# adammoss/nnest

Measured on AMD Instinct MI355X. Metric: live-point evals/sec (flow-transform + loglike) + log-Z error, x_dim=50, higher is better.
Workload: dtype f32

## Files before the change

nnest_amd/csrc/flow_tile.h:

```cpp
#pragma once
#include <hip/hip_runtime.h>
#include <stdint.h>
#include "slice_walk.h"

namespace nnest {

typedef float f32x4 __attribute__((ext_vector_type(4)));
enum { FLOW_KIND_NVP = 0, FLOW_KIND_MAF = 1 };

struct FlowShape {
    int D, H, B, L;
    int NT;
    int NH;
    int net_floats;
    int image_floats;
    int net_params;
    int scale_mode;
    float base_beta, base_const;
    int kind, G;
    __host__ __device__ int nets_params() const { return B * 2 * net_params; }
    __host__ __device__ int num_params() const { return B * 2 * net_params + (scale_mode == 2 ? B : 0); }
    __host__ __device__ int image_total() const { return image_floats + (scale_mode == 2 ? B : 0); }
};

__host__ __device__ inline int frag_off_L1() { return 0; }
__host__ __device__ inline int frag_off_L2(int NT, int NH) { return NH * NT * 4 * 64; }
__host__ __device__ inline int frag_off_L3(int NT, int NH, int L) { return frag_off_L2(NT, NH) + L * NH * NH * 4 * 64; }
__host__ __device__ inline int frag_off_b1(int NT, int NH, int L) { return frag_off_L3(NT, NH, L) + NT * NH * 4 * 64; }
__host__ __device__ inline int frag_off_b2(int NT, int NH, int L) { return frag_off_b1(NT, NH, L) + 16 * NH; }
__host__ __device__ inline int frag_off_b3(int NT, int NH, int L) { return frag_off_b2(NT, NH, L) + L * 16 * NH; }
__host__ __device__ inline int frag_net_floats(int NT, int NH, int L) { return frag_off_b3(NT, NH, L) + 16 * NT; }

__device__ __forceinline__ float fast_tanh(float x) {
    float e = __builtin_amdgcn_exp2f(x * 2.8853900817779268f);
    return 1.0f - 2.0f * __builtin_amdgcn_rcpf(e + 1.0f);
}

template <int ACT>
__device__ __forceinline__ f32x4 activate(f32x4 v) {
    f32x4 o;
    if (ACT == 0) {
        o.x = fast_tanh(v.x); o.y = fast_tanh(v.y); o.z = fast_tanh(v.z); o.w = fast_tanh(v.w);
    } else {
        o.x = fmaxf(v.x, 0.f); o.y = fmaxf(v.y, 0.f); o.z = fmaxf(v.z, 0.f); o.w = fmaxf(v.w, 0.f);
    }
    return o;
}

__device__ __forceinline__ float base_pow(float a, float beta) { return __builtin_amdgcn_exp2f(beta * __builtin_amdgcn_logf(a)); }
__device__ __forceinline__ float base_E(float u, float beta) { return beta == 0.f ? 0.5f * u * u : base_pow(fabsf(u), beta); }
__device__ __forceinline__ float base_dE(float u, float beta) {
    if (beta == 0.f) return u;
    return u == 0.f ? 0.f : beta * base_pow(fabsf(u), beta) / u;
}
__device__ __forceinline__ float base_E4(f32x4 v, float beta) { return (base_E(v.x, beta) + base_E(v.y, beta)) + (base_E(v.z, beta) + base_E(v.w, beta)); }
__device__ __forceinline__ f32x4 base_dE4(f32x4 v, float beta) { return (f32x4){base_dE(v.x, beta), base_dE(v.y, beta), base_dE(v.z, beta), base_dE(v.w, beta)}; }

__device__ __forceinline__ f32x4 mfma4(float a, float b, f32x4 c) {
    return __builtin_amdgcn_mfma_f32_16x16x4f32(a, b, c, 0, 0, 0);
}

__host__ __device__ inline int frag_elem(int idx, int lane) { return (((idx >> 2) * 64 + lane) << 2) + (idx & 3); }
__device__ __forceinline__ f32x4 frag_quad(const float *__restrict__ region_lane , int q) {
    return *reinterpret_cast<const f32x4 *>(region_lane + q * 256);
}

template <int NT, int NH, int ACT>
__device__ __forceinline__ void mlp_tile(const float *__restrict__ wn, int L, int lane, const f32x4 (&in)[NT],
                                         f32x4 (&out)[NT]) {
    const int g4 = (lane >> 4) * 4;
    const float *fL1 = wn + frag_off_L1() + 4 * lane;
    const float *fL2 = wn + frag_off_L2(NT, NH) + 4 * lane;
    const float *fL3 = wn + frag_off_L3(NT, NH, L) + 4 * lane;
    const float *b1 = wn + frag_off_b1(NT, NH, L) + g4;
    const float *b2 = wn + frag_off_b2(NT, NH, L) + g4;
    const float *b3 = wn + frag_off_b3(NT, NH, L) + g4;
    f32x4 h[NH];
#pragma unroll
    for (int ht = 0; ht < NH; ++ht) {
        f32x4 acc = *reinterpret_cast<const f32x4 *>(b1 + 16 * ht);
#pragma unroll
        for (int tau = 0; tau < NT; ++tau) {
            const f32x4 f = frag_quad(fL1, ht * NT + tau);
            acc = mfma4(f.x, in[tau].x, acc);
            acc = mfma4(f.y, in[tau].y, acc);
            acc = mfma4(f.z, in[tau].z, acc);
            acc = mfma4(f.w, in[tau].w, acc);
        }
        h[ht] = activate<ACT>(acc);
    }
    for (int l = 0; l < L; ++l) {
        f32x4 h2[NH];
#pragma unroll
        for (int hto = 0; hto < NH; ++hto) {
            f32x4 acc = *reinterpret_cast<const f32x4 *>(b2 + (l * NH + hto) * 16);
#pragma unroll
            for (int hti = 0; hti < NH; ++hti) {
                const f32x4 f = frag_quad(fL2, (l * NH + hto) * NH + hti);
                acc = mfma4(f.x, h[hti].x, acc);
                acc = mfma4(f.y, h[hti].y, acc);
                acc = mfma4(f.z, h[hti].z, acc);
                acc = mfma4(f.w, h[hti].w, acc);
            }
            h2[hto] = activate<ACT>(acc);
        }
#pragma unroll
        for (int ht = 0; ht < NH; ++ht) h[ht] = h2[ht];
    }
#pragma unroll
    for (int tau = 0; tau < NT; ++tau) {
        f32x4 acc = *reinterpret_cast<const f32x4 *>(b3 + 16 * tau);
#pragma unroll
        for (int ht = 0; ht < NH; ++ht) {
            const f32x4 f = frag_quad(fL3, tau * NH + ht);
            acc = mfma4(f.x, h[ht].x, acc);
            acc = mfma4(f.y, h[ht].y, acc);
            acc = mfma4(f.z, h[ht].z, acc);
            acc = mfma4(f.w, h[ht].w, acc);
        }
        out[tau] = acc;
    }
}

template <int NT, int NH, bool INVERSE>
__device__ __forceinline__ float coupling_tile(const float *__restrict__ wblk, int net_floats, int L, int lane,
                                               const f32x4 (&cond)[NT], f32x4 (&trans)[NT]) {
    f32x4 ls[NT], t[NT];
    mlp_tile<NT, NH, 0>(wblk, L, lane, cond, ls);
    mlp_tile<NT, NH, 1>(wblk + net_floats, L, lane, cond, t);
    float ld = 0.f;
#pragma unroll
    for (int tau = 0; tau < NT; ++tau) {
        if (!INVERSE) {
            trans[tau].x = trans[tau].x * __expf(ls[tau].x) + t[tau].x;
            trans[tau].y = trans[tau].y * __expf(ls[tau].y) + t[tau].y;
            trans[tau].z = trans[tau].z * __expf(ls[tau].z) + t[tau].z;
            trans[tau].w = trans[tau].w * __expf(ls[tau].w) + t[tau].w;
            ld += (ls[tau].x + ls[tau].y) + (ls[tau].z + ls[tau].w);
        } else {
            trans[tau].x = (trans[tau].x - t[tau].x) * __expf(-ls[tau].x);
            trans[tau].y = (trans[tau].y - t[tau].y) * __expf(-ls[tau].y);
            trans[tau].z = (trans[tau].z - t[tau].z) * __expf(-ls[tau].z);
            trans[tau].w = (trans[tau].w - t[tau].w) * __expf(-ls[tau].w);
            ld -= (ls[tau].x + ls[tau].y) + (ls[tau].z + ls[tau].w);
        }
    }
    return ld;
}

struct ImageFrags {
    const float *p;
    __device__ __forceinline__ float operator()(int idx) const {
        return static_cast<const float *>(__builtin_assume_aligned(p, 16))[(idx >> 2) * 256 + (idx & 3)];
    }
};
template <int N> struct RegFrags {
    float v[N];
    __device__ __forceinline__ float operator()(int idx) const { return v[idx]; }
};
template <int NT, int NH, int L> struct FragCount {
    static constexpr int F1 = NH * NT * 4, F2 = L * NH * NH * 4, F3 = NT * NH * 4, N = F1 + F2 + F3;
};

template <int NT, int NH, int L, bool INVERSE, class FS, class FT>
__device__ __forceinline__ float coupling_core(const FS &fs, const FT &ft, const float *__restrict__ bias_s,
                                               const float *__restrict__ bias_t, int lane, const f32x4 (&cond)[NT],
                                               f32x4 (&trans)[NT]) {
    typedef FragCount<NT, NH, L> FC;
    const int g4 = (lane >> 4) * 4;
    const f32x4 zero4 = {0.f, 0.f, 0.f, 0.f};
    f32x4 hs[NH], ht[NH];
    {
        const float *bs = bias_s + g4, *bt = bias_t + g4;
#pragma unroll
        for (int o = 0; o < NH; ++o) {
// ... 585 lines not shown
```

nnest_amd/csrc/nnest_abi.hip:

```cpp
#include <math.h>
#include <stdio.h>
#include <string.h>
#include <stdarg.h>

#include "nnest_internal.h"
#include "mh_common.h"
#include "ensemble_common.h"
#include "mcmc_walk.h"
#include "importance_walk.h"

using namespace nnest;

struct nnest_nvp {
    FlowShape s;
    int device;
    int num_cu;
    int num_params;
    float *w;
    float *adam_m;
    float *adam_v;
    float *best_w;
    float *img;
    int *adam_step;
    float *train_ws;
    int *fwd_pos;
    int *bwd_pos;
    size_t train_ws_floats;
    float *img_bwd;
    int *gpos;
    unsigned int *ticket;
};

static thread_local char g_err[512] = "";

static int fail(int code, const char *fmt, ...) {
    va_list ap;
    va_start(ap, fmt);
    vsnprintf(g_err, sizeof(g_err), fmt, ap);
    va_end(ap);
    return code;
}

namespace nnest {
void set_last_error(const char *msg) { snprintf(g_err, sizeof(g_err), "%s", msg); }
}

#define HIP_TRY(expr)                                                                                   \
    do {                                                                                                \
        hipError_t e__ = (expr);                                                                        \
        if (e__ != hipSuccess) return fail(NNEST_E_HIP, "%s: %s", #expr, hipGetErrorString(e__));       \
    } while (0)

static hipError_t refresh_images(nnest_nvp *h, hipStream_t st) {
    if (h->s.kind == FLOW_KIND_MAF) return launch_maf_repack(h->w, h->img, h->img_bwd, h->s, st);
    if (h->s.scale_mode != NNEST_SCALE_AFFINE) {
        hipError_t e = launch_zero_scale_nets(h->w, h->s, st);
        if (e != hipSuccess) return e;
    }
    return launch_repack(h->w, h->img, h->s, st);
}

extern "C" {

int nnest_hip_version(void) { return NNEST_HIP_ABI_VERSION; }

const char *nnest_hip_last_error(void) { return g_err; }

int nnest_hip_device_info(int *num_cu, int *clock_khz, char *name, int name_len) {
    int dev = 0;
    HIP_TRY(hipGetDevice(&dev));
    hipDeviceProp_t p;
    HIP_TRY(hipGetDeviceProperties(&p, dev));
    if (num_cu) *num_cu = p.multiProcessorCount;
    if (clock_khz) *clock_khz = p.clockRate;
    if (name && name_len > 0) {
        snprintf(name, name_len, "%s (%s)", p.name, p.gcnArchName);
    }
    return NNEST_OK;
}

int nnest_nvp_create(int D, int H, int B, int L, nnest_nvp_t **out) {
    return nnest_nvp_create_scaled(D, H, B, L, NNEST_SCALE_AFFINE, out);
}

int nnest_nvp_create_scaled(int D, int H, int B, int L, int scale_mode, nnest_nvp_t **out) {
    if (!out) return fail(NNEST_E_ARG, "out is NULL");
    *out = nullptr;
    if (D < 1 || H < 1 || B < 1 || L < 0) return fail(NNEST_E_ARG, "bad shape D=%d H=%d B=%d L=%d", D, H, B, L);
    if (scale_mode < NNEST_SCALE_AFFINE || scale_mode > NNEST_SCALE_CONSTANT)
        return fail(NNEST_E_ARG, "scale_mode=%d (0 '', 1 'translate', 2 'constant')", scale_mode);
    if (scale_mode == NNEST_SCALE_CONSTANT && B > 8)
        return fail(NNEST_E_UNSUPPORTED, "scale='constant' with num_blocks=%d > 8", B);
    if (H % 16 != 0)
        return fail(NNEST_E_UNSUPPORTED, "hidden_dim=%d: the gfx950 kernels tile the hidden layer by 16 (MFMA 16x16x4)", H);
    FlowShape s;
    s.D = D; s.H = H; s.B = B; s.L = L;
    s.NT = ((D + 1) / 2 + 15) / 16;
    s.NH = H / 16;
    s.net_floats = frag_net_floats(s.NT, s.NH, L);
    s.image_floats = B * 2 * s.net_floats;
    s.net_params = H * D + H + L * (H * H + H) + D * H + D;
    s.scale_mode = scale_mode;
    s.kind = FLOW_KIND_NVP;
    s.G = 0;
    s.base_beta = 0.f;
    s.base_const = -0.91893853320467274f;
    if (!shape_supported(s))
        return fail(NNEST_E_UNSUPPORTED, "x_dim=%d hidden_dim=%d not instantiated (x_dim<=128 at H=16, <=64 at H=32, <=32 at H=64)", D, H);
    nnest_nvp *h = new nnest_nvp();
    memset(h, 0, sizeof(*h));
    h->s = s;
    h->num_params = s.num_params();
    if (hipGetDevice(&h->device) != hipSuccess) { delete h; return fail(NNEST_E_HIP, "hipGetDevice failed (no GPU?)"); }
    hipDeviceProp_t p;
    if (hipGetDeviceProperties(&p, h->device) != hipSuccess) { delete h; return fail(NNEST_E_HIP, "hipGetDeviceProperties failed"); }
    h->num_cu = p.multiProcessorCount;
    size_t nb = (size_t)h->num_params * sizeof(float);
    h->train_ws_floats = train_workspace_floats(s, 128);
    hipError_t e = hipSuccess;
    if (e == hipSuccess) e = hipMalloc((void **)&h->w, nb);
    if (e == hipSuccess) e = hipMalloc((void **)&h->adam_m, nb);
    if (e == hipSuccess) e = hipMalloc((void **)&h->adam_v, nb);
    if (e == hipSuccess) e = hipMalloc((void **)&h->best_w, nb);
    if (e == hipSuccess) e = hipMalloc((void **)&h->img, (size_t)s.image_total() * sizeof(float));
    if (e == hipSuccess) e = hipMalloc((void **)&h->adam_step, sizeof(int));
    if (e == hipSuccess) e = hipMalloc((void **)&h->train_ws, h->train_ws_floats * sizeof(float));
    if (e == hipSuccess) e = hipMalloc((void **)&h->fwd_pos, nb);
    if (e == hipSuccess) e = hipMalloc((void **)&h->bwd_pos, nb);
    if (e == hipSuccess) e = launch_build_pos(h->fwd_pos, h->bwd_pos, s, 0);
    if (e == hipSuccess) e = hipStreamSynchronize(0);
    if (e == hipSuccess) e = hipMemset(h->w, 0, nb);
    if (e == hipSuccess) e = hipMemset(h->adam_m, 0, nb);
    if (e == hipSuccess) e = hipMemset(h->adam_v, 0, nb);
    if (e == hipSuccess) e = hipMemset(h->adam_step, 0, sizeof(int));
    if (e == hipSuccess) e = hipMemset(h->img, 0, (size_t)s.image_total() * sizeof(float));
    if (e != hipSuccess) {
        nnest_nvp_destroy(h);
        return fail(NNEST_E_HIP, "device allocation failed: %s", hipGetErrorString(e));
    }
    *out = h;
    return NNEST_OK;
}

int nnest_maf_create(int D, int H, int B, int L, nnest_nvp_t **out) {
    if (!out) return fail(NNEST_E_ARG, "out is NULL");
    *out = nullptr;
    if (D < 2 || H < 1 || B < 1 || L < 0) return fail(NNEST_E_ARG, "bad shape D=%d H=%d B=%d L=%d (a MAF needs x_dim >= 2)", D, H, B, L);
    if (H != 16) return fail(NNEST_E_UNSUPPORTED, "maf: hidden_dim=%d, the kernels are instantiated for 16", H);
    FlowShape s;
    s.D = D; s.H = H; s.B = B; s.L = L;
    s.NT = ((D + 1) / 2 + 15) / 16;
    s.NH = H / 16;
    s.net_floats = frag_net_floats(2 * s.NT, s.NH, L);
    s.image_floats = B * 2 * s.net_floats + B * 16 * 2 * s.NT;
    s.net_params = H * D + H + L * (H * H + H) + D * H + D;
    s.scale_mode = NNEST_SCALE_AFFINE;
    s.kind = FLOW_KIND_MAF;
    s.G = maf_num_groups(D, H);
    s.base_beta = 0.f;
    s.base_const = -0.91893853320467274f;
    if (s.NT > 4 || !maf_shape_supported(s))
        return fail(NNEST_E_UNSUPPORTED, "maf: x_dim=%d num_blocks=%d num_layers=%d: the fragment image (%d floats) has to fit one CU's LDS and x_dim <= 128", D, B, L, s.image_floats);
    nnest_nvp *h = new nnest_nvp();
    memset(h, 0, sizeof(*h));
    h->s = s;
    h->num_params = s.num_params();
    if (hipGetDevice(&h->device) != hipSuccess) { delete h; return fail(NNEST_E_HIP, "hipGetDevice failed (no GPU?)"); }
    hipDeviceProp_t p;
    if (hipGetDeviceProperties(&p, h->device) != hipSuccess) { delete h; return fail(NNEST_E_HIP, "hipGetDeviceProperties failed"); }
    h->num_cu = p.multiProcessorCount;
    const size_t nb = (size_t)h->num_params * sizeof(float), ib = (size_t)s.image_floats * sizeof(float);
    h->train_ws_floats = maf_workspace_floats(s);
    hipError_t e = hipSuccess;
    if (e == hipSuccess) e = hipMalloc((void **)&h->w, nb);
    if (e == hipSuccess) e = hipMalloc((void **)&h->adam_m, nb);
    if (e == hipSuccess) e = hipMalloc((void **)&h->adam_v, nb);
    if (e == hipSuccess) e = hipMalloc((void **)&h->best_w, nb);
    if (e == hipSuccess) e = hipMalloc((void **)&h->img, ib);
    if (e == hipSuccess) e = hipMalloc((void **)&h->img_bwd, ib);
    if (e == hipSuccess) e = hipMalloc((void **)&h->adam_step, sizeof(int));
    if (e == hipSuccess) e = hipMalloc((void **)&h->train_ws, h->train_ws_floats * sizeof(float));
    if (e == hipSuccess) e = hipMalloc((void **)&h->gpos, nb);
    if (e == hipSuccess) e = launch_maf_build_gpos(h->gpos, s, 0);
    if (e == hipSuccess) e = hipMalloc((void **)&h->fwd_pos, nb);
    if (e == hipSuccess) e = hipMalloc((void **)&h->bwd_pos, nb);
    if (e == hipSuccess) e = launch_maf_build_pos(h->fwd_pos, h->bwd_pos, s, 0);
    if (e == hipSuccess) e = hipMalloc((void **)&h->ticket, sizeof(unsigned int));
    if (e == hipSuccess) e = hipMemset(h->ticket, 0, sizeof(unsigned int));
    if (e == hipSuccess) e = hipMemset(h->w, 0, nb);
    if (e == hipSuccess) e = hipMemset(h->adam_m, 0, nb);
    if (e == hipSuccess) e = hipMemset(h->adam_v, 0, nb);
    if (e == hipSuccess) e = hipMemset(h->adam_step, 0, sizeof(int));
    if (e == hipSuccess) e = refresh_images(h, 0);
    if (e == hipSuccess) e = hipStreamSynchronize(0);
    if (e != hipSuccess) {
        nnest_nvp_destroy(h);
        return fail(NNEST_E_HIP, "device allocation failed: %s", hipGetErrorString(e));
    }
    *out = h;
    return NNEST_OK;
}

int nnest_maf_num_groups(const nnest_nvp_t *h) { return (h && h->s.kind == FLOW_KIND_MAF) ? h->s.G : -1; }

int nnest_nvp_destroy(nnest_nvp_t *h) {
    if (!h) return NNEST_OK;
    (void)hipFree(h->w); (void)hipFree(h->adam_m); (void)hipFree(h->adam_v); (void)hipFree(h->best_w); (void)hipFree(h->img);
    (void)hipFree(h->adam_step); (void)hipFree(h->train_ws); (void)hipFree(h->fwd_pos); (void)hipFree(h->bwd_pos);
    (void)hipFree(h->img_bwd); (void)hipFree(h->gpos); (void)hipFree(h->ticket);
    delete h;
    return NNEST_OK;
}

int nnest_nvp_num_params(const nnest_nvp_t *h) { return h ? h->num_params : -1; }

int nnest_nvp_set_base(nnest_nvp_t *h, float beta) {
    if (!h) return fail(NNEST_E_ARG, "NULL handle");
    if (!(beta >= 0.f)) return fail(NNEST_E_ARG, "beta=%g: 0 selects N(0, I), beta > 0 GeneralisedNormal(0, 1, beta)", (double)beta);
    h->s.base_beta = beta;
    h->s.base_const = beta == 0.f ? -0.91893853320467274f : (float)(log((double)beta) - log(2.0) - lgamma(1.0 / (double)beta));
    return NNEST_OK;
}

int nnest_nvp_load_weights(nnest_nvp_t *h, const float *packed_host, void *stream) {
    if (!h || !packed_host) return fail(NNEST_E_ARG, "NULL argument");
    hipStream_t st = (hipStream_t)stream;
    HIP_TRY(hipMemcpyAsync(h->w, packed_host, (size_t)h->num_params * sizeof(float), hipMemcpyHostToDevice, st));
    HIP_TRY(refresh_images(h, st));
    HIP_TRY(hipStreamSynchronize(st));
    return NNEST_OK;
}

int nnest_nvp_store_weights(nnest_nvp_t *h, float *packed_host, void *stream) {
    if (!h || !packed_host) return fail(NNEST_E_ARG, "NULL argument");
    hipStream_t st = (hipStream_t)stream;
    HIP_TRY(hipMemcpyAsync(packed_host, h->w, (size_t)h->num_params * sizeof(float), hipMemcpyDeviceToHost, st));
    HIP_TRY(hipStreamSynchronize(st));
    return NNEST_OK;
}

int nnest_nvp_device_ptrs(nnest_nvp_t *h, float **w_dev, float **m_dev, float **v_dev) {
    if (!h) return fail(NNEST_E_ARG, "NULL handle");
    if (w_dev) *w_dev = h->w;
    if (m_dev) *m_dev = h->adam_m;
    if (v_dev) *v_dev = h->adam_v;
    return NNEST_OK;
}

int nnest_nvp_store_adam(nnest_nvp_t *h, float *exp_avg_host, float *exp_avg_sq_host, void *stream) {
    if (!h || !exp_avg_host || !exp_avg_sq_host) return fail(NNEST_E_ARG, "NULL argument");
    hipStream_t st = (hipStream_t)stream;
    size_t nb = (size_t)h->num_params * sizeof(float);
    HIP_TRY(hipMemcpyAsync(exp_avg_host, h->adam_m, nb, hipMemcpyDeviceToHost, st));
    HIP_TRY(hipMemcpyAsync(exp_avg_sq_host, h->adam_v, nb, hipMemcpyDeviceToHost, st));
    HIP_TRY(hipStreamSynchronize(st));
    return NNEST_OK;
}

int nnest_nvp_load_adam(nnest_nvp_t *h, const float *exp_avg_host, const float *exp_avg_sq_host, void *stream) {
    if (!h || !exp_avg_host || !exp_avg_sq_host) return fail(NNEST_E_ARG, "NULL argument");
    hipStream_t st = (hipStream_t)stream;
    size_t nb = (size_t)h->num_params * sizeof(float);
    HIP_TRY(hipMemcpyAsync(h->adam_m, exp_avg_host, nb, hipMemcpyHostToDevice, st));
    HIP_TRY(hipMemcpyAsync(h->adam_v, exp_avg_sq_host, nb, hipMemcpyHostToDevice, st));
    HIP_TRY(hipStreamSynchronize(st));
    return NNEST_OK;
}

int nnest_nvp_adam_state(nnest_nvp_t *h, int *step_count, int set_step, int reset_moments, void *stream) {
    if (!h) return fail(NNEST_E_ARG, "NULL handle");
    hipStream_t st = (hipStream_t)stream;
    if (reset_moments) {
        HIP_TRY(hipMemsetAsync(h->adam_m, 0, (size_t)h->num_params * sizeof(float), st));
        HIP_TRY(hipMemsetAsync(h->adam_v, 0, (size_t)h->num_params * sizeof(float), st));
    }
    if (set_step >= 0) HIP_TRY(hipMemcpyAsync(h->adam_step, &set_step, sizeof(int), hipMemcpyHostToDevice, st));
    HIP_TRY(hipStreamSynchronize(st));
    if (step_count) {
        HIP_TRY(hipMemcpyAsync(step_count, h->adam_step, sizeof(int), hipMemcpyDeviceToHost, st));
        HIP_TRY(hipStreamSynchronize(st));
    }
    return NNEST_OK;
}

static int check_rows(const nnest_nvp_t *h, const void *a, const void *b, int N) {
    if (!h) return fail(NNEST_E_ARG, "NULL handle");
    if (N < 0) return fail(NNEST_E_ARG, "N=%d < 0", N);
    if (N > 0 && (!a || !b)) return fail(NNEST_E_ARG, "NULL device buffer");
    return NNEST_OK;
}

int nnest_nvp_forward(nnest_nvp_t *h, const float *x_dev, float *z_dev, float *logdet_dev, int N, void *stream) {
    int rc = check_rows(h, x_dev, z_dev, N);
    if (rc) return rc;
    HIP_TRY(launch_pass(h->img, h->s, PASS_FORWARD, x_dev, z_dev, logdet_dev, nullptr, nullptr, N, LikeSpec(), h->num_cu,
                        (hipStream_t)stream));
    return NNEST_OK;
}

int nnest_nvp_inverse(nnest_nvp_t *h, const float *z_dev, float *x_dev, float *logdet_dev, int N, void *stream) {
    int rc = check_rows(h, z_dev, x_dev, N);
    if (rc) return rc;
    HIP_TRY(launch_pass(h->img, h->s, PASS_INVERSE, z_dev, x_dev, logdet_dev, nullptr, nullptr, N, LikeSpec(), h->num_cu,
                        (hipStream_t)stream));
    return NNEST_OK;
}

int nnest_nvp_log_probs(nnest_nvp_t *h, const float *x_dev, float *logp_dev, int N, void *stream) {
    int rc = check_rows(h, x_dev, logp_dev, N);
    if (rc) return rc;
    HIP_TRY(launch_pass(h->img, h->s, PASS_LOGPROB, x_dev, logp_dev, nullptr, nullptr, nullptr, N, LikeSpec(), h->num_cu,
                        (hipStream_t)stream));
    return NNEST_OK;
}

static int check_like(const nnest_like_t *like, int D, LikeSpec *out) {
    if (!like) return fail(NNEST_E_ARG, "like is NULL");
    if (like->id < 0 || like->id >= NNEST_LIKE_COUNT) return fail(NNEST_E_ARG, "unknown likelihood id %d", like->id);
    if (like->id == NNEST_LIKE_EGGBOX && D != 2) return fail(NNEST_E_ARG, "Eggbox is defined for x_dim = 2 (likelihoods.py:97-102)");
    if (like->id == NNEST_LIKE_GAUSSMIX && D < 2) return fail(NNEST_E_ARG, "GaussianMix needs x_dim >= 2");
    out->id = like->id;
    out->scale = like->scale;
    for (int i = 0; i < 6; ++i) out->p[i] = like->params[i];
    return NNEST_OK;
}

int nnest_nvp_inverse_loglike(nnest_nvp_t *h, const nnest_like_t *like, const float *z_dev, float *x_dev,
                              float *logdet_dev, double *logl_dev, int *inbox_dev, int N, void *stream) {
    int rc = check_rows(h, z_dev, logl_dev, N);
    if (rc) return rc;
    LikeSpec lk;
    if ((rc = check_like(like, h->s.D, &lk))) return rc;
    HIP_TRY(launch_pass(h->img, h->s, PASS_INVERSE_LOGLIKE, z_dev, x_dev, logdet_dev, logl_dev, inbox_dev, N, lk,
                        h->num_cu, (hipStream_t)stream));
    return NNEST_OK;
}

int nnest_loglike(const nnest_like_t *like, const float *x_unit_dev, double *logl_dev, int N, int D, void *stream) {
    if (N < 0 || D < 1) return fail(NNEST_E_ARG, "bad N=%d D=%d", N, D);
    LikeSpec lk;
    int rc = check_like(like, D, &lk);
    if (rc) return rc;
    if (D > 128) return fail(NNEST_E_UNSUPPORTED, "x_dim=%d > 128", D);
    if (N > 0 && (!x_unit_dev || !logl_dev)) return fail(NNEST_E_ARG, "NULL device buffer");
    int dev = 0, num_cu = 256;
    HIP_TRY(hipGetDevice(&dev));
    HIP_TRY(hipDeviceGetAttribute(&num_cu, hipDeviceAttributeMultiprocessorCount, dev));
    HIP_TRY(launch_loglike(lk, x_unit_dev, logl_dev, N, D, num_cu, (hipStream_t)stream));
    return NNEST_OK;
}

int nnest_mh_constrained_steps(nnest_nvp_t *h, const nnest_like_t *like, float *z_dev, float *x_dev,
                               double *logl_dev, double loglstar, float step_size, int steps, int C, int flags,
                               const float *noise_dz_dev, const float *noise_u_dev, uint64_t seed,
                               uint64_t walker_offset, float *hist_x_dev, double *hist_logl_dev, int *n_accept_dev,
                               int *n_call_dev, float *scale_out_dev, void *sync_dev, void *stream) {
    int rc = check_rows(h, z_dev, logl_dev, C);
    if (rc) return rc;
    LikeSpec lk;
    if ((rc = check_like(like, h->s.D, &lk))) return rc;
    if (steps < 0) return fail(NNEST_E_ARG, "steps=%d < 0", steps);
    if ((noise_dz_dev == nullptr) != (noise_u_dev == nullptr))
        return fail(NNEST_E_ARG, "noise_dz_dev and noise_u_dev must both be given or both be NULL");
    if ((flags & NNEST_MH_DYNAMIC_BATCH) && !sync_dev) return fail(NNEST_E_ARG, "NNEST_MH_DYNAMIC_BATCH needs sync_dev");
    hipError_t e = launch_mh(h->img, h->s, lk, z_dev, x_dev, logl_dev, loglstar, step_size, steps, C, flags,
                             noise_dz_dev, noise_u_dev, seed, walker_offset, hist_x_dev, hist_logl_dev, n_accept_dev, n_call_dev,
                             scale_out_dev, h->w, (unsigned long long *)sync_dev, h->num_cu, (hipStream_t)stream);
    if (e == hipErrorInvalidConfiguration)
        return fail(NNEST_E_UNSUPPORTED, "no kernel form for C=%d walkers with flags 0x%x (pinned form not applicable to this "
                                         "shape / population, or the batch-wide step rule on a grid that may not be resident)", C, flags);
    if (e != hipSuccess) return fail(NNEST_E_HIP, "launch_mh: %s", hipGetErrorString(e));
    return NNEST_OK;
}

int nnest_slice_steps(nnest_nvp_t *h, const nnest_like_t *like, float *z_dev, float *x_dev, double *logl_dev, double loglstar,
                      float width, int steps, int C, int max_stepout, int max_shrink, const float *noise_dz_dev, uint64_t seed,
                      uint64_t walker_offset, float *hist_x_dev, int *n_call_dev, int *n_move_dev, int *n_eval_dev, void *stream) {
    int rc = check_rows(h, z_dev, logl_dev, C);
    if (rc) return rc;
    LikeSpec lk;
    if ((rc = check_like(like, h->s.D, &lk))) return rc;
    if (!slice_params_ok(steps, max_stepout, max_shrink, width))
        return fail(NNEST_E_ARG, "steps=%d max_stepout=%d (0..2^24) max_shrink=%d (1..60) width=%g", steps, max_stepout, max_shrink, (double)width);
    if (!slice_form_eligible(h->s))
        return fail(NNEST_E_UNSUPPORTED, "slice proposal: hidden 16, 3 blocks, 1 layer, scale '' (the one-walker-per-wave layout), x_dim <= 128");
    const SliceArgs a = {z_dev, x_dev, logl_dev, loglstar, width, steps, C, max_stepout, max_shrink, lk, seed, walker_offset, noise_dz_dev,
                         hist_x_dev, nullptr, n_call_dev, n_move_dev, n_eval_dev};
    hipError_t e = launch_slice_solo(h->s, h->w, a, (hipStream_t)stream);
    if (e != hipSuccess) return fail(NNEST_E_HIP, "launch_slice_solo: %s", hipGetErrorString(e));
    return NNEST_OK;
}

int nnest_slice_fill_noise(float *dz_dev, int steps, int C, int D, uint64_t seed, uint64_t walker_offset, void *stream) {
    if (!dz_dev || steps < 0 || C < 0 || D < 1) return fail(NNEST_E_ARG, "bad argument");
    HIP_TRY(launch_slice_fill_noise(dz_dev, steps, C, D, seed, walker_offset, (hipStream_t)stream));
    return NNEST_OK;
}

int nnest_ensemble_work_words(int C, int steps) {
    if (C < 0 || steps < 0) return -1;
    const size_t w = ensemble_work_words(C, steps);
    return w > (size_t)0x7fffffff ? -1 : (int)w;
}

}
int nnest::mcmc_args(McmcArgs *a, const float *t_std, const float *t_mean, const float *lo, const float *hi, const float *z_in,
                     const double *lp_in, const double *logl_in, float *z_out, float *x_out, double *lp_out, double *logl_out,
                     float *hist_z, float *hist_x, double *hist_logl, int *n_accept, int C, int steps, float step_size, uint64_t step0,
                     uint64_t seed, uint64_t walker_offset) {
    if (C < 1 || steps < 0) return fail(NNEST_E_ARG, "mcmc: C=%d (>= 1 walkers) steps=%d (>= 0)", C, steps);
    if (!isfinite(step_size) || step_size < 0.f) return fail(NNEST_E_ARG, "mcmc: step_size=%g (finite, >= 0)", (double)step_size);
    if (!z_in || !x_out || !lp_out || !logl_out || (steps > 0 && !z_out)) return fail(NNEST_E_ARG, "NULL device buffer");
    if (!t_std != !t_mean) return fail(NNEST_E_ARG, "t_std_dev and t_mean_dev: both or neither");
    if (!lo != !hi) return fail(NNEST_E_ARG, "lo_dev and hi_dev: both or neither");
    if (!lp_in != !logl_in) return fail(NNEST_E_ARG, "lp_in_dev and logl_in_dev: both or neither");
    if ((!hist_z != !hist_x) || (!hist_z != !hist_logl)) return fail(NNEST_E_ARG, "hist_z_dev, hist_x_dev and hist_logl_dev: all or none");
    a->t_std = t_std; a->t_mean = t_mean; a->lo = lo; a->hi = hi;
    a->z_in = z_in; a->lp_in = lp_in; a->logl_in = logl_in;
    a->z_out = z_out; a->x_out = x_out; a->lp_out = lp_out; a->logl_out = logl_out;
    a->hist_z = hist_z; a->hist_x = hist_x; a->hist_logl = hist_logl; a->n_accept = n_accept;
    a->C = C; a->S = steps; a->step = step_size; a->step0 = (uint32_t)step0; a->seed = seed; a->walker_offset = walker_offset;
    return NNEST_OK;
}
int nnest::mcmc_beta_ok(double beta) {
    if (!isfinite(beta) || beta < 0.0) return fail(NNEST_E_ARG, "mcmc: beta=%g (the likelihood's power: finite, >= 0)", beta);
    return NNEST_OK;
}
int nnest::importance_args(ImpArgs *a, const float *t_std, const float *t_mean, const float *lo, const float *hi, float *z_out, float *x_out,
                           double *logl_out, double *logw_out, double *partials, double *sums, int M, uint64_t seed, uint64_t sample_offset) {
    if (M < 0 || M > (1 << 30)) return fail(NNEST_E_ARG, "importance: M=%d (0 .. 2^30 samples a launch)", M);
    if (!sums || (M > 0 && !partials)) return fail(NNEST_E_ARG, "importance: NULL sums_dev or partials_dev");
    if (!t_std != !t_mean) return fail(NNEST_E_ARG, "t_std_dev and t_mean_dev: both or neither");
    if (!lo != !hi) return fail(NNEST_E_ARG, "lo_dev and hi_dev: both or neither");
    if ((!z_out != !x_out) || (!z_out != !logl_out) || (!z_out != !logw_out))
        return fail(NNEST_E_ARG, "z_out_dev, x_out_dev, logl_out_dev and logw_out_dev: all or none");
    a->t_std = t_std; a->t_mean = t_mean; a->lo = lo; a->hi = hi;
    a->z_out = z_out; a->x_out = x_out; a->logl_out = logl_out; a->logw_out = logw_out;
    a->partials = partials; a->sums = sums; a->M = M; a->seed = seed; a->sample_offset = sample_offset;
    return NNEST_OK;
}
int nnest::ensemble_sizes(int C, int steps) {
    if (C < 2 || C > (1 << 16) || steps < 0) return fail(NNEST_E_ARG, "ensemble: C=%d (2..65536 walkers) steps=%d", C, steps);
    if (nnest_ensemble_work_words(C, steps) < 0) return fail(NNEST_E_ARG, "ensemble: C=%d x steps=%d: the work buffer exceeds 2^31 words", C, steps);
    return NNEST_OK;
}
static int ens_resolve_moves(const nnest_ens_moves_t *m, int C, int D, EnsMoves *out) {
    out->thr = ENS_THR_ALWAYS;
    out->g0 = out->sigma = 0.f;
    if (!m) return NNEST_OK;
    const double ws = (double)m->w_stretch, wd = (double)m->w_de;
    if (!(isfinite(ws) && isfinite(wd)) || ws < 0.0 || wd < 0.0 || ws + wd <= 0.0)
        return fail(NNEST_E_ARG, "ensemble moves: weights stretch=%g de=%g (finite, >= 0, not both 0)", ws, wd);
    if (!(isfinite(m->de_gamma0) && isfinite(m->de_sigma)) || m->de_gamma0 < 0.f || m->de_sigma < 0.f)
        return fail(NNEST_E_ARG, "ensemble moves: de_gamma0=%g de_sigma=%g (finite, >= 0; 0: emcee's default)", (double)m->de_gamma0, (double)m->de_sigma);
    if (wd > 0.0 && C < 4) return fail(NNEST_E_ARG, "ensemble moves: C=%d walkers: the DE move needs two partners in either set (C >= 4)", C);
    if (D < 1) return fail(NNEST_E_ARG, "ensemble moves: D=%d", D);
    out->thr = (uint32_t)floor(ws / (ws + wd) * 16777216.0);
    out->g0 = m->de_gamma0 != 0.f ? m->de_gamma0 : (float)(2.38 / sqrt(2.0 * (double)D));
    out->sigma = m->de_sigma != 0.f ? m->de_sigma : 1e-5f;
    return NNEST_OK;
}

extern "C" {

int nnest_ensemble_moves_threshold(const nnest_ens_moves_t *moves) {
    EnsMoves mv;
    if (ens_resolve_moves(moves, 4, 1, &mv)) return -1;
    return (int)mv.thr;
}

int nnest_ensemble_fill_moves(const int *work_dev, int *move_dev, int *b_dev, float *gamma_dev, int C, int D, int steps, uint64_t step0,
                              uint64_t seed, const nnest_ens_moves_t *moves, void *stream) {
    int rc = ensemble_sizes(C, steps);
    if (rc) return rc;
    if (!work_dev) return fail(NNEST_E_ARG, "NULL work_dev");
    if (C < 4) return fail(NNEST_E_ARG, "ensemble moves: C=%d walkers: the DE move needs two partners in either set (C >= 4)", C);
    EnsMoves mv;
    const nnest_ens_moves_t dflt = {1.f, 0.f, 0.f, 0.f};
    if ((rc = ens_resolve_moves(moves ? moves : &dflt, C, D, &mv))) return rc;
    HIP_TRY(launch_ensemble_fill_moves(work_dev, move_dev, b_dev, gamma_dev, C, steps, (uint32_t)step0, seed, mv, (hipStream_t)stream));
    return NNEST_OK;
}

int nnest_ensemble_fill_noise(int *work_dev, float *u_dev, int C, int steps, uint64_t step0, uint64_t seed, void *stream) {
    int rc = ensemble_sizes(C, steps);
    if (rc) return rc;
    if (!work_dev) return fail(NNEST_E_ARG, "NULL work_dev");
    HIP_TRY(launch_ensemble_split(work_dev, u_dev, C, steps, (uint32_t)step0, seed, (hipStream_t)stream));
    return NNEST_OK;
}

static int mcmc_steps_entry(nnest_nvp_t *h, const nnest_like_t *like, const float *t_std_dev, const float *t_mean_dev, const float *lo_dev,
                            const float *hi_dev, const float *z_in_dev, const double *lp_in_dev, const double *logl_in_dev, float *z_out_dev,
                            float *x_out_dev, double *lp_out_dev, double *logl_out_dev, float *hist_z_dev, float *hist_x_dev,
                            double *hist_logl_dev, int *n_accept_dev, int C, int steps, float step_size, uint64_t step0, uint64_t seed,
                            uint64_t walker_offset, const double *beta, void *stream) {
    if (!like) return fail(NNEST_E_ARG, "like is NULL");
    if (like->id < 0 || like->id >= NNEST_LIKE_COUNT) return fail(NNEST_E_ARG, "unknown likelihood id %d", like->id);
    int rc;
    if (beta && (rc = mcmc_beta_ok(*beta))) return rc;
    McmcTemperedArgs a;
    memset(&a, 0, sizeof(a));
    a.beta = beta ? *beta : 1.0;
    rc = mcmc_args(&a, t_std_dev, t_mean_dev, lo_dev, hi_dev, z_in_dev, lp_in_dev, logl_in_dev, z_out_dev, x_out_dev, lp_out_dev,
                   logl_out_dev, hist_z_dev, hist_x_dev, hist_logl_dev, n_accept_dev, C, steps, step_size, step0, seed, walker_offset);
    if (rc) return rc;
    if (!h) return fail(NNEST_E_ARG, "NULL handle");
    if ((rc = check_like(like, h->s.D, &a.like))) return rc;
    a.like.scale = 1.0f;
    if (!ensemble_form_eligible(h->s))
        return fail(NNEST_E_UNSUPPORTED, "mcmc: hidden 16, 3 blocks, 1 layer, scale '' (the one-walker-per-wave layout), x_dim <= 128");
    hipError_t e = beta ? launch_mcmc_tempered(h->s, h->w, a, (hipStream_t)stream) : launch_mcmc(h->s, h->w, a, (hipStream_t)stream);
    if (e == hipErrorInvalidConfiguration) return fail(NNEST_E_UNSUPPORTED, "mcmc: x_dim=%d not instantiated", h->s.D);
    if (e != hipSuccess) return fail(NNEST_E_HIP, "launch_mcmc: %s", hipGetErrorString(e));
    return NNEST_OK;
}

int nnest_mcmc_steps(nnest_nvp_t *h, const nnest_like_t *like, const float *t_std_dev, const float *t_mean_dev, const float *lo_dev,
                     const float *hi_dev, const float *z_in_dev, const double *lp_in_dev, const double *logl_in_dev, float *z_out_dev,
                     float *x_out_dev, double *lp_out_dev, double *logl_out_dev, float *hist_z_dev, float *hist_x_dev,
                     double *hist_logl_dev, int *n_accept_dev, int C, int steps, float step_size, uint64_t step0, uint64_t seed,
                     uint64_t walker_offset, void *stream) {
    return mcmc_steps_entry(h, like, t_std_dev, t_mean_dev, lo_dev, hi_dev, z_in_dev, lp_in_dev, logl_in_dev, z_out_dev, x_out_dev, lp_out_dev,
                            logl_out_dev, hist_z_dev, hist_x_dev, hist_logl_dev, n_accept_dev, C, steps, step_size, step0, seed,
                            walker_offset, nullptr, stream);
}

int nnest_mcmc_tempered_steps(nnest_nvp_t *h, const nnest_like_t *like, const float *t_std_dev, const float *t_mean_dev, const float *lo_dev,
                              const float *hi_dev, const float *z_in_dev, const double *lp_in_dev, const double *logl_in_dev,
                              float *z_out_dev, float *x_out_dev, double *lp_out_dev, double *logl_out_dev, float *hist_z_dev,
                              float *hist_x_dev, double *hist_logl_dev, int *n_accept_dev, int C, int steps, float step_size,
                              uint64_t step0, uint64_t seed, uint64_t walker_offset, double beta, void *stream) {
    return mcmc_steps_entry(h, like, t_std_dev, t_mean_dev, lo_dev, hi_dev, z_in_dev, lp_in_dev, logl_in_dev, z_out_dev, x_out_dev, lp_out_dev,
                            logl_out_dev, hist_z_dev, hist_x_dev, hist_logl_dev, n_accept_dev, C, steps, step_size, step0, seed,
                            walker_offset, &beta, stream);
}

int nnest_mcmc_fill_noise(float *dz_dev, float *u_dev, int steps, int C, int D, uint64_t step0, uint64_t seed, uint64_t walker_offset,
                          void *stream) {
    if (steps < 0 || C < 0 || D < 1) return fail(NNEST_E_ARG, "mcmc_fill_noise: steps=%d C=%d D=%d", steps, C, D);
    HIP_TRY(launch_mcmc_fill_noise(dz_dev, u_dev, steps, C, D, (uint32_t)step0, seed, walker_offset, (hipStream_t)stream));
// ... 307 lines not shown
```

nnest_amd/csrc/nnest_internal.h:

```cpp
#pragma once
#include <hip/hip_runtime.h>
#include <stdint.h>
#include "flow_tile.h"
#include "maf_tile.h"
#include "spline_tile.h"
#include "../../include/nnest_hip.h"

namespace nnest {

enum { PASS_FORWARD = 0, PASS_INVERSE = 1, PASS_LOGPROB = 2, PASS_INVERSE_LOGLIKE = 3 };

void set_last_error(const char *msg);
bool shape_supported(const FlowShape &s);
hipError_t launch_repack(const float *packed, float *img, const FlowShape &s, hipStream_t st);
hipError_t launch_zero_scale_nets(float *packed, const FlowShape &s, hipStream_t st);
hipError_t launch_pass(const float *img, const FlowShape &s, int mode, const float *in, float *out, float *logdet,
                       double *logl, int *inbox, int N, const LikeSpec &like, int num_cu, hipStream_t st);
hipError_t launch_mh(const float *img, const FlowShape &s, const LikeSpec &like, float *z, float *x, double *logl,
                     double loglstar, float step_size, int steps, int C, int flags, const float *noise_dz,
                     const float *noise_u, uint64_t seed, uint64_t walker_offset, float *hist_x, double *hist_logl,
                     int *n_accept, int *n_call, float *scale_out, const float *packed, unsigned long long *sync, int num_cu,
                     hipStream_t st);
struct MhArgs;
struct SliceArgs;
bool quad_form_eligible(const MhArgs &a, int num_cu);
hipError_t launch_mh_quad(const MhArgs &a, int num_cu, hipStream_t st);
bool solo_form_eligible(const MhArgs &a, int num_cu);
hipError_t launch_mh_solo(const MhArgs &a, int num_cu, hipStream_t st);
int mh_form_for(const FlowShape &s, int C, int flags, int num_cu);
bool maf_shape_supported(const FlowShape &s);
hipError_t launch_maf_repack(const float *packed, float *imgf, float *imgb, const FlowShape &s, hipStream_t st);
hipError_t launch_loglike(const LikeSpec &like, const float *x, double *logl, int N, int D, int num_cu, hipStream_t st);
hipError_t launch_fill_noise(float *dz, float *u, int steps, int C, int D, uint64_t seed, uint64_t walker_offset,
                             hipStream_t st);
int mh_num_groups(int C);

struct SplArgs {
    const float *img;
    SplineShape sp;
};
hipError_t launch_spline_mh_pair(const MhArgs &a, const SplArgs &q, bool dbg, hipStream_t st);
hipError_t launch_spline_mh_team(const MhArgs &a, const SplArgs &q, bool dbg, hipStream_t st);
int spline_mh_form(const SplineShape &sp, int C, int flags, int num_cu);
int spline_slice_form(const SplineShape &sp, int C, int flags, int num_cu);
hipError_t launch_spline_slice(const SplArgs &q, const SliceArgs &a, int flags, int num_cu, hipStream_t st);
bool spline_shape_supported(const SplineShape &s);
hipError_t launch_spline_pass(const float *img, const SplineShape &sp, int mode, const float *in, float *out, float *logdet,
                              double *logl, int *inbox, int N, const LikeSpec &like, int num_cu, hipStream_t st);
hipError_t launch_spline_mh(const float *img, const SplineShape &sp, const LikeSpec &like, float *z, float *x, double *logl,
                            double loglstar, float step_size, int steps, int C, int flags, const float *noise_dz,
                            const float *noise_u, uint64_t seed, uint64_t walker_offset, float *hist_x, double *hist_logl,
                            int *n_accept, int *n_call, float *scale_out, unsigned long long *sync, int num_cu, hipStream_t st);

struct TrainArgs;
hipError_t launch_loss_grad(const float *packed, const FlowShape &s, const float *x, int M, float *grad, float *loss,
                            float *workspace, float *img_fwd, const int *fwd_pos, const int *bwd_pos, hipStream_t st);
hipError_t launch_vjp(const float *packed, const FlowShape &s, const float *x, const float *gz, float gld, int M, float *grad, float *gx,
                      float *workspace, float *img_fwd, const int *fwd_pos, const int *bwd_pos, hipStream_t st);
hipError_t launch_adam_packed(float *w, const float *grad, float *m, float *v, int n, int step, float lr, float wd, hipStream_t st);
hipError_t launch_adam_packed_dev(float *w, const float *grad, float *m, float *v, int n, int *step_dev, float lr, float wd, hipStream_t st);
size_t train_workspace_floats(const FlowShape &s, int batch);
hipError_t launch_train(float *packed, float *adam_m, float *adam_v, float *best_w, float *img, int *adam_step_dev,
                        const FlowShape &s, const float *xtrain, int n_train, const float *xvalid, int n_valid,
                        const int *perm, const float *noise, uint64_t seed, float jitter, int batch, int max_epochs,
                        int patience, float lr, float wd, int epoch_offset, int flags, float *losses, nnest_train_result_t *result,
                        float *workspace, const int *fwd_pos, const int *bwd_pos,
                        hipStream_t st);
int train_form_for(const FlowShape &s, int batch, int flags, int *detail);
hipError_t launch_build_pos(int *fwd_pos, int *bwd_pos, const FlowShape &s, hipStream_t st);
size_t maf_workspace_floats(const FlowShape &s);
hipError_t launch_maf_build_gpos(int *gpos, const FlowShape &s, hipStream_t st);
hipError_t launch_maf_build_pos(int *fwd_pos, int *bwd_pos, const FlowShape &s, hipStream_t st);
hipError_t launch_maf_train_minibatch(const FlowShape &s, float *imgf, float *imgb, const int *gpos, const int *fwd_pos, const int *bwd_pos,
                                      const float *x, int M, float *w, float *m, float *v, int *step_dev, float lr, float wd,
                                      float *loss_acc, unsigned int *ticket, float *workspace, hipStream_t st);
hipError_t launch_maf_loss_grad(const FlowShape &s, const float *imgf, const float *imgb, const int *gpos, const float *x, int M,
                                float *grad, float *loss, float *workspace, hipStream_t st);
hipError_t launch_training_jitter(const double *samples, int N, int D, double *out, hipStream_t st);
bool slice_form_eligible(const FlowShape &s);
hipError_t launch_slice_solo(const FlowShape &s, const float *packed, const SliceArgs &a, hipStream_t st);
hipError_t launch_slice_fill_noise(float *dz, int steps, int C, int D, uint64_t seed, uint64_t walker_offset, hipStream_t st);
size_t ensemble_work_words(int C, int S);
bool ensemble_form_eligible(const FlowShape &s);
struct EnsMoves;
hipError_t ensemble_max_walkers(const FlowShape &s, int like_id, const EnsMoves &mv, int num_cu, int *out);
hipError_t ensemble_x_max_walkers(int D, int like_id, const EnsMoves &mv, int num_cu, int *out);
hipError_t launch_ensemble_fill_moves(const int *work, int *move, int *jb, float *gamma, int C, int S, uint32_t step0, uint64_t seed,
                                      const EnsMoves &mv, hipStream_t st);
int launch_ensemble_x(int D, const LikeSpec &like, const float *t_std, const float *t_mean, const float *lo, const float *hi,
                      const float *x_in, const double *lp_in, float *x_out, float *tx_out, double *lp_out, float *hist_x, double *hist_lp,
                      int *n_accept, int *work, int C, int S, uint32_t step0, uint64_t seed, int constrained, double loglstar,
                      const EnsMoves &mv, int num_cu, hipStream_t st, char *msg, size_t msg_len);
hipError_t launch_ensemble_split(int *work, float *u, int C, int S, uint32_t step0, uint64_t seed, hipStream_t st);
int launch_ensemble(const FlowShape &s, const float *packed, const LikeSpec &like, const float *t_std, const float *t_mean, const float *lo,
                    const float *hi, const float *z_in, const double *lp_in, float *z_out, float *x_out, double *lp_out, float *hist_z,
                    float *hist_x, double *hist_lp, int *n_accept, int *work, int C, int S, uint32_t step0, uint64_t seed, int constrained,
                    double loglstar, const EnsMoves &mv, int num_cu, hipStream_t st, char *msg, size_t msg_len);
int ensemble_sizes(int C, int steps);
struct EnsArgs;
hipError_t spline_ensemble_max_walkers(const SplArgs &q, int num_cu, int *out);
int launch_spline_ensemble(const SplArgs &q, const EnsArgs &a, int num_cu, hipStream_t st, char *msg, size_t msg_len);
hipError_t launch_ensemble_propose(const int *work, int C, int S, int D, int i, int half, uint32_t step0, uint64_t seed, const EnsMoves &mv,
                                   const float *z_cur, float *q, int rows, hipStream_t st);
hipError_t launch_ensemble_accept(const int *work, int C, int S, int D, int i, int half, uint32_t step0, uint64_t seed, const EnsMoves &mv,
                                  const float *q, const float *x, const float *ld, const double *logl, const double *lprior, const float *t_std,
                                  const float *t_mean, const float *lo, const float *hi, float *z_cur, float *x_cur, double *lp_cur,
                                  float *hist_z, float *hist_x, double *hist_lp, int *n_accept, int *acc_rows, int constrained,
                                  double loglstar, int rows, hipStream_t st);

}
```

nnest_amd/csrc/nnest_kernels.hip:

```cpp
#include <map>
#include <mutex>
#include <utility>
#include <string.h>

#include "flow_tile.h"
#include "maf_tile.h"
#include "mh_common.h"
#include "nnest_internal.h"
#include "spline_train_tile.h"

namespace nnest {

__global__ void repack_fragments_kernel(const float *__restrict__ packed, float *__restrict__ img, FlowShape s) {
    const int NT = s.NT, NH = s.NH, L = s.L, D = s.D, H = s.H;
    const int total = s.image_floats;
    for (int idx = blockIdx.x * blockDim.x + threadIdx.x; idx < total; idx += gridDim.x * blockDim.x) {
        int bn = idx / s.net_floats, o = idx - bn * s.net_floats;
        int b = bn >> 1, net = bn & 1;
        const float *p = packed + ((size_t)b * 2 + net) * s.net_params;
        const int pc = (b + 1) & 1, pt = b & 1;
        const int pW0 = 0, pb0 = H * D, phid = H * D + H, pWo = H * D + H + L * (H * H + H), pbo = pWo + D * H;
        float v = 0.f;
        if (o < frag_off_L2(NT, NH)) {
            int r = o & 3, lane = (o >> 2) & 63, q = (o >> 8) << 2, tau = (q >> 2) % NT, ht = (q >> 2) / NT;
// ... 499 lines not shown
        if (b.p) (void)hipFree(b.p);
        b.p = nullptr; b.cap = 0;
        const size_t want = floats + floats / 2 + 4096;
        if (hipMalloc((void **)&b.p, want * sizeof(float)) != hipSuccess) { b.p = nullptr; return nullptr; }
        b.cap = want;
    }
    return b.p;
}
hipError_t launch_mh_zero_other_sync(const MhArgs &a, hipStream_t st) {
    if (!a.sync || !(a.flags & (NNEST_MH_SYNC_ZERO_NEXT | NNEST_MH_SYNC_ZERO_PREV))) return hipSuccess;
    const size_t W = mh_sync_words(a.steps) + 1;
    unsigned long long *other = (a.flags & NNEST_MH_SYNC_ZERO_NEXT) ? a.sync + W : a.sync - W;
    return hipMemsetAsync(other, 0, W * sizeof(unsigned long long), st);
}
hipError_t launch_mh_all_moved(const MhArgs &a, hipStream_t st) {
    if (!a.x0 || !a.x || !a.n_accept) return hipSuccess;
    const int grid = min((a.C + 3) / 4, 2048);
    hipLaunchKernelGGL(mh_all_moved_kernel, dim3(grid), dim3(256), 0, st, a.x0, a.x, a.n_accept, a.C, a.s.D);
    return hipGetLastError();
}

template <int NT, int NH, int LT>
static hipError_t launch_mh_tiles_t(const MhArgs &a, int form, int num_cu, hipStream_t st);
template <int NT, int NH, int LT>
static hipError_t launch_mh_t(const MhArgs &a_in, int num_cu, hipStream_t st) {
    const bool batch = (a_in.flags & NNEST_MH_DYNAMIC_BATCH) != 0;
    if (batch && !a_in.sync) return hipErrorInvalidValue;
    const int form = pick_mh_form<NT, NH, LT>(a_in, num_cu);
    if (form < 0) return hipErrorInvalidConfiguration;
    if (form == MH_FORM_SOLO) return launch_mh_solo(a_in, num_cu, st);
    if (form == MH_FORM_QUAD || form == MH_FORM_QUAD1) {
        hipError_t e = launch_mh_quad(a_in, num_cu, st);
        return e != hipSuccess ? e : launch_mh_zero_other_sync(a_in, st);
    }
    MhArgs a = a_in;
    if (a.x && a.n_accept && !(a.x0 = mh_first_x_buffer((size_t)a.C * a.s.D, st))) return hipErrorOutOfMemory;
    hipError_t e = launch_mh_tiles_t<NT, NH, LT>(a, form, num_cu, st);
    if (e != hipSuccess) return e;
    e = launch_mh_zero_other_sync(a, st);
    if (e != hipSuccess) return e;
    return launch_mh_all_moved(a, st);
}
template <int NT, int NH, int LT>
static hipError_t launch_mh_tiles_t(const MhArgs &a, int form, int num_cu, hipStream_t st) {
    const int ntiles = (a.C + 15) / 16;
    const bool batch = (a.flags & NNEST_MH_DYNAMIC_BATCH) != 0;
    if constexpr (LT == 1 && NH == 1) {
        if (form == MH_FORM_TEAM) {
            const size_t timg = NT <= 2 ? 0 : (size_t)a.s.image_floats * 4;
            const int grid = ntiles + ((batch && mh_flag_lag(a.flags) >= 2) ? 1 : 0);
            if (a.hist_x || a.hist_logl) {
                hipError_t e = allow_lds(mh_kernel_team<NT, 1, 3, true>, timg + 48 * 1024);
                if (e != hipSuccess) return e;
                hipLaunchKernelGGL((mh_kernel_team<NT, 1, 3, true>), dim3(grid), dim3(192), timg, st, a);
            } else {
                hipError_t e = allow_lds(mh_kernel_team<NT, 1, 3, false>, timg + 48 * 1024);
                if (e != hipSuccess) return e;
                hipLaunchKernelGGL((mh_kernel_team<NT, 1, 3, false>), dim3(grid), dim3(192), timg, st, a);
            }
            return hipGetLastError();
        }
    }
    if constexpr (LT == 1 && NH == 1 && NT <= 2) {
        if (form == MH_FORM_REG) {
            if (a.noise_dz || a.hist_x || a.hist_logl)
                hipLaunchKernelGGL((mh_kernel_reg<NT, 1, 1, 3, true>), dim3(ntiles), dim3(64), 0, st, a);
            else
                hipLaunchKernelGGL((mh_kernel_reg<NT, 1, 1, 3, false>), dim3(ntiles), dim3(64), 0, st, a);
            return hipGetLastError();
        }
    }
    const size_t img_bytes = (size_t)a.s.image_floats * 4;
    const bool dbg = a.noise_dz || a.hist_x || a.hist_logl;
    const ImageGeom geo = image_geometry<NT>(ntiles, num_cu, img_bytes, batch, dbg);
    const int block = geo.block, grid = geo.grid;
    if constexpr (NT >= 3) {
        if (geo.occ == 1) {
            hipError_t e = allow_lds(mh_kernel<NT, NH, LT, true, false, 1>, img_bytes);
            if (e != hipSuccess) return e;
            hipLaunchKernelGGL((mh_kernel<NT, NH, LT, true, false, 1>), dim3(grid), dim3(block), img_bytes, st, a);
            return hipGetLastError();
        }
    }
    if (geo.occ == 2) {
        hipError_t e = allow_lds(mh_kernel<NT, NH, LT, true, false, 2>, img_bytes);
        if (e != hipSuccess) return e;
        hipLaunchKernelGGL((mh_kernel<NT, NH, LT, true, false, 2>), dim3(grid), dim3(block), img_bytes, st, a);
        return hipGetLastError();
    }
    if (img_bytes <= (size_t)LDS_IMAGE_LIMIT) {
        if (dbg) {
            hipError_t e = allow_lds(mh_kernel<NT, NH, LT, true, true>, img_bytes);
            if (e != hipSuccess) return e;
            hipLaunchKernelGGL((mh_kernel<NT, NH, LT, true, true>), dim3(grid), dim3(block), img_bytes, st, a);
        } else {
            hipError_t e = allow_lds(mh_kernel<NT, NH, LT, true, false>, img_bytes);
            if (e != hipSuccess) return e;
            hipLaunchKernelGGL((mh_kernel<NT, NH, LT, true, false>), dim3(grid), dim3(block), img_bytes, st, a);
        }
    } else {
        if (dbg) hipLaunchKernelGGL((mh_kernel<NT, NH, LT, false, true>), dim3(grid), dim3(block), 0, st, a);
        else hipLaunchKernelGGL((mh_kernel<NT, NH, LT, false, false>), dim3(grid), dim3(block), 0, st, a);
    }
    return hipGetLastError();
}

template <int NT, int NH, int LT>
static int mh_form_t(const MhArgs &a, int num_cu) { return pick_mh_form<NT, NH, LT>(a, num_cu); }

#define DISPATCH_NTNH(FN, s, LT, ...)                                \
    do {                                                             \
        if ((s).NH == 1) {                                           \
            switch ((s).NT) {                                        \
                case 1: return FN<1, 1, LT>(__VA_ARGS__);            \
                case 2: return FN<2, 1, LT>(__VA_ARGS__);            \
                case 3: return FN<3, 1, LT>(__VA_ARGS__);            \
                case 4: return FN<4, 1, LT>(__VA_ARGS__);            \
            }                                                        \
        } else if ((s).NH == 2) {                                    \
            switch ((s).NT) {                                        \
                case 1: return FN<1, 2, LT>(__VA_ARGS__);            \
                case 2: return FN<2, 2, LT>(__VA_ARGS__);            \
            }                                                        \
        } else if ((s).NH == 4) {                                    \
            switch ((s).NT) {                                        \
                case 1: return FN<1, 4, LT>(__VA_ARGS__);            \
            }                                                        \
        }                                                            \
        return hipErrorInvalidConfiguration;                         \
    } while (0)

#define DISPATCH_SHAPE(FN, s, ...)                                   \
    do {                                                             \
        if ((s).L == 1) DISPATCH_NTNH(FN, s, 1, __VA_ARGS__);        \
        DISPATCH_NTNH(FN, s, -1, __VA_ARGS__);                       \
    } while (0)

bool shape_supported(const FlowShape &s) {
    if (s.NH == 1) return s.NT >= 1 && s.NT <= 4;
    if (s.NH == 2) return s.NT >= 1 && s.NT <= 2;
    if (s.NH == 4) return s.NT == 1;
    return false;
}

hipError_t launch_zero_scale_nets(float *packed, const FlowShape &s, hipStream_t st) {
    hipLaunchKernelGGL(zero_scale_nets_kernel, dim3(64), dim3(256), 0, st, packed, s);
    return hipGetLastError();
}

hipError_t launch_repack(const float *packed, float *img, const FlowShape &s, hipStream_t st) {
    int block = 256, grid = (s.image_floats + block - 1) / block;
    if (grid > 1024) grid = 1024;
    hipLaunchKernelGGL(repack_fragments_kernel, dim3(grid), dim3(block), 0, st, packed, img, s);
    return hipGetLastError();
}

static hipError_t launch_maf_pass(const PassArgs &a, int num_cu, hipStream_t st);
static hipError_t launch_maf_mh(const MhArgs &a, int num_cu, hipStream_t st);

hipError_t launch_pass(const float *img, const FlowShape &s, int mode, const float *in, float *out, float *logdet,
                       double *logl, int *inbox, int N, const LikeSpec &like, int num_cu, hipStream_t st) {
    if (N <= 0) return hipSuccess;
    PassArgs a;
    a.img = img; a.s = s; a.mode = mode; a.in = in; a.out = out; a.logdet = logdet; a.logl = logl; a.inbox = inbox;
    a.N = N; a.like = like;
    if (s.kind == FLOW_KIND_MAF) return launch_maf_pass(a, num_cu, st);
    DISPATCH_SHAPE(launch_pass_t, s, a, num_cu, st);
}

hipError_t launch_mh(const float *img, const FlowShape &s, const LikeSpec &like, float *z, float *x, double *logl,
                     double loglstar, float step_size, int steps, int C, int flags, const float *noise_dz,
                     const float *noise_u, uint64_t seed, uint64_t walker_offset, float *hist_x, double *hist_logl,
                     int *n_accept, int *n_call, float *scale_out, const float *packed, unsigned long long *sync, int num_cu,
                     hipStream_t st) {
    if (C <= 0) return hipSuccess;
    MhArgs a;
    a.packed = packed;
    a.sync = sync;
    a.sync_err = sync ? reinterpret_cast<int *>(sync + mh_sync_words(steps)) : nullptr;
    a.img = img; a.s = s; a.z = z; a.x = x; a.logl = logl; a.loglstar = loglstar; a.step_size = step_size;
    a.steps = steps; a.C = C; a.flags = flags; a.like = like;
    a.noise_dz = noise_dz; a.noise_u = noise_u; a.seed = seed; a.walker_offset = walker_offset;
    a.hist_x = hist_x; a.hist_logl = hist_logl; a.n_accept = n_accept; a.n_call = n_call; a.scale_out = scale_out;
    a.x0 = nullptr;
    if (s.kind == FLOW_KIND_MAF) {
        if (a.x && a.n_accept && !(a.x0 = mh_first_x_buffer((size_t)C * s.D, st))) return hipErrorOutOfMemory;
        hipError_t e = launch_maf_mh(a, num_cu, st);
        if (e == hipSuccess) e = launch_mh_zero_other_sync(a, st);
        return e != hipSuccess ? e : launch_mh_all_moved(a, st);
    }
    DISPATCH_SHAPE(launch_mh_t, s, a, num_cu, st);
}

hipError_t launch_loglike(const LikeSpec &like, const float *x, double *logl, int N, int D, int num_cu, hipStream_t st) {
    if (N <= 0) return hipSuccess;
    const int NT = ((D + 1) / 2 + 15) / 16;
    const int ntiles = (N + 15) / 16;
    int block = 256, grid = (ntiles + 3) / 4;
    if (grid > 8 * num_cu) grid = 8 * num_cu;
    switch (NT) {
        case 1: hipLaunchKernelGGL((loglike_kernel<1>), dim3(grid), dim3(block), 0, st, x, logl, N, D, like); break;
        case 2: hipLaunchKernelGGL((loglike_kernel<2>), dim3(grid), dim3(block), 0, st, x, logl, N, D, like); break;
        case 3: hipLaunchKernelGGL((loglike_kernel<3>), dim3(grid), dim3(block), 0, st, x, logl, N, D, like); break;
        case 4: hipLaunchKernelGGL((loglike_kernel<4>), dim3(grid), dim3(block), 0, st, x, logl, N, D, like); break;
        default: return hipErrorInvalidConfiguration;
    }
    return hipGetLastError();
}

hipError_t launch_fill_noise(float *dz, float *u, int steps, int C, int D, uint64_t seed, uint64_t walker_offset,
                             hipStream_t st) {
    if (steps <= 0 || C <= 0) return hipSuccess;
    int block = 256;
    int grid = (C * 4 + block - 1) / block;
    hipLaunchKernelGGL(fill_noise_kernel, dim3(grid), dim3(block), 0, st, dz, u, steps, C, D, seed, walker_offset);
    return hipGetLastError();
}

int mh_num_groups(int C) { return (C + 15) / 16; }

int mh_form_for(const FlowShape &s, int C, int flags, int num_cu) {
    MhArgs a = MhArgs();
    a.s = s; a.C = C; a.flags = flags;
    if (s.kind == FLOW_KIND_MAF) {
        const int form = mh_flag_form(flags);
        if (form != MH_FORM_AUTO && form != MH_FORM_IMAGE) return -1;
        if ((flags & NNEST_MH_DYNAMIC_BATCH) && mh_flag_lag(flags) > 0 && mh_flag_warm(flags) > 0) return -1;
        int block, grid;
        pick_geometry((C + 15) / 16, num_cu, 4, &block, &grid);
        return ((flags & NNEST_MH_DYNAMIC_BATCH) && grid > num_cu) ? -1 : MH_FORM_IMAGE;
    }
    DISPATCH_SHAPE(mh_form_t, s, a, num_cu);
}

#include "maf_kernels.h"
#include "spline_kernels.h"

}
```

nnest_amd/csrc/nnest_solo.hip:

```cpp
#include <string.h>
#include "mh_common.h"
#include "nnest_internal.h"
#include "solo_loglike.h"
#include "solo_tile.h"

namespace nnest {

static constexpr int SOLO_ETAB = 1024;

template <int U, int WPG> constexpr bool solo_lds_weights() { return U >= 3 || WPG > 4; }
template <int U, int WPG> constexpr int solo_reg_blocks() { return !solo_lds_weights<U, WPG>() ? 3 : (WPG == 4 ? 1 : (U <= 2 && WPG == 8 ? 1 : 0)); }

enum { MH_SOLO_LAG_INTERNAL = 8 };
template <int U, bool DBG, int LK, int WPG>
__global__ void __launch_bounds__(64 * (WPG + 2)) mh_kernel_solo(MhArgs a) {
    extern __shared__ __attribute__((aligned(16))) float wlds[];
    __shared__ __attribute__((aligned(16))) float nbuf[2][WPG][16][2 * U];
    __shared__ float ubuf[2][WPG];
    __shared__ __attribute__((aligned(16))) uint32_t rawbuf[4 * WPG * 8 * U];
    __shared__ int acc_lds[2][WPG];
    __shared__ float fsbuf[2];
    __shared__ float fs_exact;
    __shared__ float fs_cand[2];
    __shared__ int vote_sel;
    __shared__ double etab[SOLO_ETAB];

    const int lane = threadIdx.x & 63, wave = __builtin_amdgcn_readfirstlane(threadIdx.x >> 6);
    const int tile = blockIdx.x;
    const int D = a.s.D, S = a.steps, C = a.C;
    const bool recorded = DBG && a.noise_dz;
    const bool dynamic = (a.flags & NNEST_MH_DYNAMIC_BATCH) != 0;
    const bool use_tab = S + 2 <= SOLO_ETAB;
    const bool exact_all = dynamic && mh_flag_lag(a.flags) == 0;
    const bool direct_votes = (a.flags & NNEST_MH_WINDOW_VOTES_ONLY) == 0;
    const int lag = exact_all ? MH_SOLO_LAG_INTERNAL : mh_flag_lag(a.flags);
    const int warm = dynamic ? min(exact_all ? S : mh_flag_warm(a.flags), S - 1) : 0;
    constexpr bool LDSW = solo_lds_weights<U, WPG>();
    constexpr int RB = solo_reg_blocks<U, WPG>();
    const int ntiles = (C + WPG - 1) / WPG;
    if (tile >= ntiles) {
        if (dynamic && wave == 0) mh_sync_publisher(a.sync, S, exact_all ? S : max(S - lag, warm), ntiles, C, lane, a.sync_err);
        else if (dynamic && (a.flags & (NNEST_MH_SYNC_ZERO_NEXT | NNEST_MH_SYNC_ZERO_PREV))) {
            const size_t W = (size_t)mh_sync_words(S) + 1;
            unsigned long long *other = (a.flags & NNEST_MH_SYNC_ZERO_NEXT) ? a.sync + W : a.sync - W;
            const int nthr = (int)blockDim.x - 64;
            for (size_t i = threadIdx.x - 64; i < W; i += nthr) other[i] = 0ull;
        }
        return;
    }
    {
        if constexpr (!LDSW) {
            const int n = a.s.nets_params();
            for (int i = threadIdx.x; i < n; i += blockDim.x) wlds[i] = a.packed[i];
        } else {
            if (wave < 3) {
                SoloNet<U> nb;
                solo_gather<U>(nb, a.packed + (size_t)(wave * 2 + (lane >= 32 ? 1 : 0)) * a.s.net_params, D, (wave + 1) & 1, wave & 1, lane);
                solo4_store<U>(wlds, wave, nb, lane);
            }
        }
        if (dynamic && use_tab)
            for (int k = threadIdx.x; k < S + 2; k += blockDim.x) etab[k] = exp(1.0 / (double)(1 + k));
    }
    __syncthreads();

    if (wave == WPG) {
        const int g = lane & 3, j = min(lane >> 2, WPG - 1);
        const bool gen = lane < 4 * WPG;
        Xoshiro128 rn = xoshiro_seed(a.seed, a.walker_offset + (uint64_t)(tile * WPG + j), (uint32_t)g, NOISE_STREAM_DZ);
        Xoshiro128 ru = xoshiro_seed(a.seed, a.walker_offset + (uint64_t)(tile * WPG + j), 0xffffffffu, NOISE_STREAM_U);
        constexpr int NQ = 8 * WPG * U;
        unsigned long long n0 = 0, n1 = 0, n2 = 0, n_gen = 0, n_all = 0;
        (void)n0; (void)n1; (void)n2; (void)n_gen; (void)n_all;
        auto draw = [&](int k) {
            if (k > S) return;
            STAMP(n0);
            if (!recorded) {
                if (gen) {
#pragma unroll
                    for (int t = 0; t < 2 * U; ++t) {
                        u32x4 r;
                        r.x = xoshiro_next(rn); r.y = xoshiro_next(rn); r.z = xoshiro_next(rn); r.w = xoshiro_next(rn);
                        *reinterpret_cast<u32x4 *>(&rawbuf[lane * 8 * U + 4 * t]) = r;
                    }
                    const float u = xoshiro_uniform(ru);
                    if (g == 0) ubuf[k & 1][j] = u;
                }
                float *nb = &nbuf[k & 1][0][0][0];
#pragma unroll
                for (int i = 0; i < (NQ + 63) / 64; ++i) {
                    const int q = lane + 64 * i;
                    if (NQ % 64 == 0 || q < NQ) {
                        const u32x4 r = *reinterpret_cast<const u32x4 *>(&rawbuf[4 * q]);
                        const int sl = q / (2 * U), qq = q % (2 * U);
                        const int d0 = 32 * (qq >> 1) + 8 * (sl & 3) + 4 * (qq & 1);
                        float o0, o1, o2, o3;
                        box_muller(r.x, r.y, o0, o1);
                        box_muller(r.z, r.w, o2, o3);
                        const f32x4 o = {d0 < D ? o0 : 0.f, d0 + 1 < D ? o1 : 0.f, d0 + 2 < D ? o2 : 0.f, d0 + 3 < D ? o3 : 0.f};
                        *reinterpret_cast<f32x4 *>(nb + (sl >> 2) * 32 * U + d0) = o;
                    }
                }
            }
            if (!dynamic && lane == 0) fsbuf[k & 1] = a.step_size;
            STAMP(n1);
#ifdef NNEST_STAMP
            n_gen += n1 - n0;
#endif
        };
        STAMP(n2);
        draw(0);
        solo_barrier();
        if (S >= 1) {
            draw(1);
            solo_barrier();
            draw(2);
            for (int k = 1; k <= warm; ++k) {
                solo_barrier();
                solo_barrier();
                draw(k + 2);
                solo_barrier();
            }
            for (int k = warm > 0 ? warm + 2 : 2; k <= S; ++k) {
                solo_barrier();
                draw(k + 1);
            }
        }
#ifdef NNEST_STAMP
        { unsigned long long n3 = 0; STAMP(n3); n_all = n3 - n2; }
#endif
#ifdef NNEST_STAMP
        if (a.scale_out && lane == 0 && tile == 0) { a.scale_out[4] = (float)n_gen; a.scale_out[5] = (float)n_all; }
#endif
#ifndef NNEST_STAMP
        if (!dynamic && a.scale_out && lane == 0) {
            const int g0 = (tile * WPG + 15) >> 4;
            if (16 * g0 < (tile + 1) * WPG && 16 * g0 < C) a.scale_out[g0] = a.step_size;
        }
#endif
        return;
    }
    if (wave == WPG + 1) {
        if (!dynamic) return;
        double scale = (double)a.step_size;
        int accept = 0, reject = 0;
        const int last = S - lag;
        const unsigned long long *wbase = a.sync + 2 * mh_sync_counter_words(S) + (size_t)(tile & (MH_SYNC_SHARDS - 1)) * MH_SYNC_STRIDE;
#define SOLO_RELAY_ITERATION(k_, q_)                                                                                        \
        {                                                                                                                   \
            const int k = (k_), want = k - lag;                                                                             \
              \
              \
              \
              \
              \
            asm volatile("s_waitcnt vmcnt(2)" : "+v"(q_) : : "memory");                                                     \
            if (want > warm) {                                                                                              \
                const bool up = mh_window_vote(a.sync, S, want, tile, q_, a.sync_err);                                      \
                if (up) accept += 1; else reject += 1;                                                                      \
                if (accept > reject) scale *= use_tab ? etab[accept] : exp(1.0 / (1 + accept));                             \
                if (accept < reject) scale /= use_tab ? etab[reject] : exp(1.0 / (1 + reject));                             \
            }                                                                                                               \
                   \
             \
            if (lane == 0) {                                                                                                \
                const int *ac = acc_lds[k & 1];                                                                             \
                const bool mine = k - 2 > warm;                                 \
                int acs = 0;                                                                                                \
                _Pragma("unroll") for (int w_ = 0; w_ < WPG; ++w_) acs += ac[w_];                                           \
                mh_sync_post(a.sync, mine ? k - 2 : 0, tile, mine ? acs : 0);                                               \
            }                                                                                                               \
            const int ask = min(max(want + 2, 1), max(last, 1));         \
            const unsigned long long *wp = wbase + (size_t)((ask - 1) >> 5) * MH_SYNC_SHARDS * MH_SYNC_STRIDE;              \
            asm volatile("global_load_dwordx2 %0, %1, off sc1" : "=v"(q_) : "v"(wp) : "memory");                            \
              \
            if (lane == 0) fsbuf[k & 1] = (float)scale;                                                                     \
            solo_barrier();                                                                           \
        }
        unsigned long long qa = 0, qb = 0;
        int k0 = 0;
        if (warm > 0) {
            auto E = [&](int n) { return use_tab ? etab[n] : exp(1.0 / (1 + n)); };
            auto next_scale = [&](int acc, int rej, double sc) {
                if (acc > rej) sc *= E(acc);
                if (acc < rej) sc /= E(rej);
                return sc;
            };
            if (lane == 0) {
                fsbuf[0] = (float)scale;
                fs_cand[0] = (float)next_scale(accept + 1, reject, scale);
                fs_cand[1] = (float)next_scale(accept, reject + 1, scale);
            }
            solo_barrier();
            if (lane == 0) fsbuf[1] = (float)scale;
            solo_barrier();
            for (int k = 1; k <= warm; ++k) {
                solo_barrier();
                if (lane == 0) {
                    const int *ac = acc_lds[k & 1];
                    int acs = 0;
#pragma unroll
                    for (int w_ = 0; w_ < WPG; ++w_) acs += ac[w_];
                    mh_sync_post(a.sync, k, tile, acs);
                    fsbuf[(k + 1) & 1] = (float)scale;
                }
                solo_barrier();
                const bool up = direct_votes ? 2 * mh_sync_total(a.sync, k, ntiles, 0ull, a.sync_err) > C
                                             : mh_window_vote(a.sync, S, k, tile, 0ull, a.sync_err);
                if (up) accept += 1; else reject += 1;
                scale = next_scale(accept, reject, scale);
                if (lane == 0) {
                    vote_sel = up ? 0 : 1;
                    fs_exact = (float)scale;
                    fs_cand[0] = (float)next_scale(accept + 1, reject, scale);
                    fs_cand[1] = (float)next_scale(accept, reject + 1, scale);
                }
                solo_barrier();
            }
            k0 = warm + 2;
        }
        for (int k2 = k0; k2 <= S; k2 += 2) {
            SOLO_RELAY_ITERATION(k2, qa)
            if (k2 + 1 <= S) SOLO_RELAY_ITERATION(k2 + 1, qb)
        }
#undef SOLO_RELAY_ITERATION
        asm volatile("s_waitcnt vmcnt(0)" : "+v"(qa), "+v"(qb) : : "memory");
        if (exact_all) {
            solo_barrier();
            if (lane == 0) {
                const int *ac = acc_lds[S & 1];
                int acs = 0;
#pragma unroll
                for (int w_ = 0; w_ < WPG; ++w_) acs += ac[w_];
                mh_sync_post(a.sync, S, tile, acs);
            }
            const bool up = direct_votes ? 2 * mh_sync_total(a.sync, S, ntiles, 0ull, a.sync_err) > C : mh_window_vote(a.sync, S, S, tile, 0ull, a.sync_err);
            if (up) accept += 1; else reject += 1;
            if (accept > reject) scale *= use_tab ? etab[accept] : exp(1.0 / (1 + accept));
            if (accept < reject) scale /= use_tab ? etab[reject] : exp(1.0 / (1 + reject));
        }
#ifndef NNEST_STAMP
        if (a.scale_out && lane == 0) {
            const int g0 = (tile * WPG + 15) >> 4;
            if (16 * g0 < (tile + 1) * WPG && 16 * g0 < C) a.scale_out[g0] = (float)scale;
        }
#endif
        return;
    }

    const int j = wave;
    const int pos = lane & 15;
    const bool translate_half = lane >= 32;
    const bool writer_lane = lane < 16;
    const int row = tile * WPG + j;
    const bool ok = row < C;
    const LikeSpec like = a.like;
    const double loglstar = a.loglstar;
    const bool free_mode = (a.flags & NNEST_MH_UNCONSTRAINED) != 0;

    SoloNet<U> net[RB > 0 ? RB : 1];
    if constexpr (LDSW) {
        if constexpr (RB == 1)
            solo_gather<U>(net[0], a.packed + (size_t)(1 * 2 + (translate_half ? 1 : 0)) * a.s.net_params, D, (1 + 1) & 1, 1 & 1, lane);
    } else {
#pragma unroll
        for (int b = 0; b < 3; ++b)
            solo_gather<U>(net[b], wlds + (size_t)(b * 2 + (translate_half ? 1 : 0)) * a.s.net_params, D, (b + 1) & 1, b & 1, lane);
    }
    const unsigned sel = translate_half ? 0xffffffffu : 0u;
    const bool h1 = (lane & 16) != 0;
    auto inverse = [&](float (&xs)[2][U]) {
        if constexpr (LDSW) {
            float ld = solo_coupling_inverse4<U>(Solo4Lds{wlds + (size_t)2 * SOLO4_NF * 64, lane}, sel, h1, xs[1], xs[0]);
            if constexpr (RB == 1) ld += solo_coupling_inverse4<U>(Solo4Reg<U>{net[0]}, sel, h1, xs[0], xs[1]);
            else ld += solo_coupling_inverse4<U>(Solo4Lds{wlds + (size_t)1 * SOLO4_NF * 64, lane}, sel, h1, xs[0], xs[1]);
            ld += solo_coupling_inverse4<U>(Solo4Lds{wlds, lane}, sel, h1, xs[1], xs[0]);
            return ld;
        } else {
            float ld;
            solo_coupling_inverse<U, true>(net[2], sel, h1, xs[1], xs[0], ld);
            solo_coupling_inverse<U, false>(net[1], sel, h1, xs[0], xs[1], ld);
            solo_coupling_inverse<U, false>(net[0], sel, h1, xs[1], xs[0], ld);
            return ld;
        }
    };

    float z[2][U], x[2][U];
#pragma unroll
    for (int u = 0; u < U; ++u)
#pragma unroll
        for (int c = 0; c < 2; ++c) {
            const int d = 2 * U * pos + 2 * u + c;
            z[c][u] = (ok && d < D) ? a.z[(size_t)row * D + d] : 0.f;
            x[c][u] = z[c][u];
        }
    float ld = solo_logdet_total(inverse(x));
    double logl = ok ? a.logl[row] : 0.0;
    int n_acc = 0, n_call = 0;

    auto store_row = [&](float *base, size_t r, const float (&v)[2][U]) {
#pragma unroll
        for (int u = 0; u < U; ++u)
#pragma unroll
            for (int c = 0; c < 2; ++c) {
                const int d = 2 * U * pos + 2 * u + c;
                if (d < D) base[r * D + d] = v[c][u];
            }
    };
    if (writer_lane && ok && a.x) store_row(a.x, (size_t)row, x);
    if (DBG && writer_lane && ok) {
        if (a.hist_x) store_row(a.hist_x, (size_t)row * (S + 1), x);
        if (a.hist_logl && pos == 0) a.hist_logl[(size_t)row * (S + 1)] = logl;
    }

    float nz[2 * U], u_next = 0.f, fs_next = a.step_size;
    int kbuf = 0;
    auto fetch_noise = [&]() {
        solo_barrier();
        if (!recorded) {
#pragma unroll
            for (int k = 0; k < 2 * U; ++k) nz[k] = nbuf[kbuf & 1][j][pos][k];
            u_next = ubuf[kbuf & 1][j];
        }
        fs_next = fsbuf[kbuf & 1];
        ++kbuf;
    };
    fetch_noise();

    unsigned long long st0 = 0, st1 = 0, st2 = 0, st3 = 0, a_prop = 0, a_inv = 0, a_post = 0, a_tot = 0;
    (void)st0; (void)st1; (void)st2; (void)st3; (void)a_prop; (void)a_inv; (void)a_post; (void)a_tot;
    struct Prop { float zp[2][U], xp[2][U]; float ldp; double lp; bool pre, acc; };
    auto propose = [&](int it, float fs, float (&zp)[2][U], float &u) {
        if (recorded) {
#pragma unroll
            for (int uu = 0; uu < U; ++uu)
#pragma unroll
                for (int c = 0; c < 2; ++c) {
                    const int d = 2 * U * pos + 2 * uu + c;
                    const float dz = (ok && d < D) ? a.noise_dz[((size_t)(it - 1) * C + row) * D + d] : 0.f;
                    zp[c][uu] = __builtin_fmaf(dz, fs, z[c][uu]);
                }
            u = ok ? a.noise_u[(size_t)(it - 1) * C + row] : 1.f;
        } else {
#pragma unroll
            for (int uu = 0; uu < U; ++uu) {
                zp[0][uu] = __builtin_fmaf(nz[2 * uu], fs, z[0][uu]);
                zp[1][uu] = __builtin_fmaf(nz[2 * uu + 1], fs, z[1][uu]);
            }
            u = u_next;
        }
    };
    auto finish = [&](Prop &r, float u) {
#pragma unroll
        for (int c = 0; c < 2; ++c)
#pragma unroll
            for (int uu = 0; uu < U; ++uu) r.xp[c][uu] = r.zp[c][uu];
        STAMP(st1);
        constexpr bool RIDE = LK == NNEST_LIKE_ROSENBROCK;
        r.ldp = RIDE ? inverse(r.xp) : solo_logdet_total(inverse(r.xp));
        STAMP(st2);
        if constexpr (RIDE) r.lp = solo_loglike<U, LK>(like, D, lane, r.xp, &r.ldp);
        int okl = 1;
#pragma unroll
        for (int c = 0; c < 2; ++c)
#pragma unroll
            for (int uu = 0; uu < U; ++uu) okl &= !(r.xp[c][uu] < -1.f || r.xp[c][uu] > 1.f);
        const bool inb = __ballot(okl != 0) == ~0ull;
        float log_ratio = inb ? (r.ldp - ld) : -INFINITY;
        float ratio = fminf(__expf(log_ratio), 1.0f);
        if (log_ratio != log_ratio) ratio = log_ratio;
        r.pre = ok && (u < ratio);
        if constexpr (!RIDE) r.lp = solo_loglike<U, LK>(like, D, lane, r.xp);
        r.acc = r.pre && (r.lp > loglstar);
        if (free_mode) {
            const double lr = inb ? (double)(r.ldp - ld) + (r.lp - logl) : -INFINITY;
            const double rt = fmin(exp(lr), 1.0);
            r.acc = ok && ((double)u < rt);
        }
    };
    auto apply = [&](int it, const Prop &r) {
        n_call += (free_mode ? ok : r.pre) ? 1 : 0;
        n_acc += r.acc ? 1 : 0;
#pragma unroll
        for (int c = 0; c < 2; ++c)
#pragma unroll
            for (int uu = 0; uu < U; ++uu) {
                z[c][uu] = r.acc ? r.zp[c][uu] : z[c][uu];
                x[c][uu] = r.acc ? r.xp[c][uu] : x[c][uu];
            }
        ld = r.acc ? r.ldp : ld;
        logl = r.acc ? r.lp : logl;
        if (dynamic && lane == 0) acc_lds[it & 1][j] = r.acc ? 1 : 0;
        if (DBG && writer_lane && ok) {
            if (a.hist_x) store_row(a.hist_x, (size_t)row * (S + 1) + it, x);
            if (a.hist_logl && pos == 0) a.hist_logl[(size_t)row * (S + 1) + it] = logl;
        }
    };
    Prop cur;
    bool have = false;
    for (int it = 1; it <= S; ++it) {
        STAMP(st0);
        if (!have) {
            float u;
            propose(it, fs_next, cur.zp, u);
            fetch_noise();
            finish(cur, u);
        }
        apply(it, cur);
        have = false;
        if (it <= warm) {
            solo_barrier();
            const float f0 = fs_cand[0], f1 = fs_cand[1];
            Prop c1;
            float u;
            propose(it + 1, f0, cur.zp, u);
            propose(it + 1, f1, c1.zp, u);
            fetch_noise();
            finish(cur, u);
            finish(c1, u);
            solo_barrier();
            if (vote_sel != 0) cur = c1;
            have = true;
            fs_next = fs_exact;
        }
        STAMP(st3);
#ifdef NNEST_STAMP
        a_prop += st1 - st0; a_inv += st2 - st1; a_post += st3 - st2; a_tot += st3 - st0;
#endif
    }
    if (exact_all) solo_barrier();
#ifdef NNEST_STAMP
    if (a.scale_out && lane == 0 && tile == 0) {
        float *o = a.scale_out;
        if (j == 0) { o[0] = (float)a_tot; o[1] = (float)a_prop; o[2] = (float)a_inv; o[3] = (float)a_post; }
        if (j < 4) { o[8 + 2 * j] = (float)a_inv; o[9 + 2 * j] = (float)a_post; }
    }
#endif
    bool all_moved = n_acc > 0;
    if (a.x) {
        bool mine = true;
        if (writer_lane) {
#pragma unroll
            for (int u = 0; u < U; ++u)
#pragma unroll
                for (int c = 0; c < 2; ++c) {
                    const int d = 2 * U * pos + 2 * u + c;
                    const float x0 = (ok && d < D) ? a.x[(size_t)row * D + d] : 0.f;
                    mine = mine && (d >= D || x[c][u] != x0);
                }
        }
        all_moved = (__ballot(mine) & 0xffffull) == 0xffffull;
    }
    if (writer_lane && ok) {
        store_row(a.z, (size_t)row, z);
        if (a.x) store_row(a.x, (size_t)row, x);
        if (pos == 0) {
            a.logl[row] = logl;
            if (a.n_accept) a.n_accept[row] = n_acc | (all_moved ? NNEST_MH_ALL_MOVED : 0);
            if (a.n_call) a.n_call[row] = n_call;
        }
    }
}

template <int U>
static __device__ __forceinline__ void slice_normals(uint64_t seed, uint64_t walker, uint32_t step, int pos, int D, float (&e)[2][U]) {
    const int d0 = 2 * U * pos;
    f32x4 q[(2 * U + 3) / 4 + 1];
    const int q0 = d0 >> 2;
#pragma unroll
    for (int k = 0; k < (2 * U + 3) / 4 + 1; ++k) q[k] = noise_normal4(seed, walker, step, (uint32_t)(q0 + k), NOISE_STREAM_DZ);
#pragma unroll
    for (int u = 0; u < U; ++u)
#pragma unroll
        for (int c = 0; c < 2; ++c) {
            const int d = d0 + 2 * u + c, k = (d >> 2) - q0, r = d & 3;
            float v = 0.f;
#pragma unroll
            for (int kk = 0; kk < (2 * U + 3) / 4 + 1; ++kk)
                if (kk == k) v = r == 0 ? q[kk].x : (r == 1 ? q[kk].y : (r == 2 ? q[kk].z : q[kk].w));
            e[c][u] = d < D ? v : 0.f;
        }
}

template <int U, int LK>
__global__ void __launch_bounds__(256) slice_kernel_solo(SliceArgs a, FlowShape s, const float *packed) {
    extern __shared__ __attribute__((aligned(16))) float wlds[];
    const int lane = threadIdx.x & 63, wave = __builtin_amdgcn_readfirstlane(threadIdx.x >> 6);
    const int D = s.D, S = a.steps, C = a.C;
    constexpr bool LDSW = solo_lds_weights<U, 4>();
    {
        if constexpr (!LDSW) {
            const int n = s.nets_params();
            for (int i = threadIdx.x; i < n; i += blockDim.x) wlds[i] = packed[i];
        } else if (wave < 3) {
            SoloNet<U> nb;
            solo_gather<U>(nb, packed + (size_t)(wave * 2 + (lane >= 32 ? 1 : 0)) * s.net_params, D, (wave + 1) & 1, wave & 1, lane);
            solo4_store<U>(wlds, wave, nb, lane);
        }
    }
    __syncthreads();
    const int pos = lane & 15;
    const bool translate_half = lane >= 32, writer_lane = lane < 16;
    const int row = blockIdx.x * 4 + wave;
    const bool ok = row < C;
    if (!ok) return;
    const LikeSpec like = a.like;
    const double loglstar = a.loglstar;
    SoloNet<U> net[LDSW ? 1 : 3];
    if constexpr (!LDSW) {
#pragma unroll
        for (int b = 0; b < 3; ++b)
            solo_gather<U>(net[b], wlds + (size_t)(b * 2 + (translate_half ? 1 : 0)) * s.net_params, D, (b + 1) & 1, b & 1, lane);
    }
    const unsigned sel = translate_half ? 0xffffffffu : 0u;
    const bool h1 = (lane & 16) != 0;
    auto inverse = [&](float (&xs)[2][U]) {
        if constexpr (LDSW) {
            float ld = solo_coupling_inverse4<U>(Solo4Lds{wlds + (size_t)2 * SOLO4_NF * 64, lane}, sel, h1, xs[1], xs[0]);
            ld += solo_coupling_inverse4<U>(Solo4Lds{wlds + (size_t)1 * SOLO4_NF * 64, lane}, sel, h1, xs[0], xs[1]);
            ld += solo_coupling_inverse4<U>(Solo4Lds{wlds, lane}, sel, h1, xs[1], xs[0]);
            return ld;
        } else {
            float ld;
            solo_coupling_inverse<U, true>(net[2], sel, h1, xs[1], xs[0], ld);
            solo_coupling_inverse<U, false>(net[1], sel, h1, xs[0], xs[1], ld);
            solo_coupling_inverse<U, false>(net[0], sel, h1, xs[1], xs[0], ld);
            return ld;
        }
    };
    auto store_row = [&](float *base, size_t r, const float (&v)[2][U]) {
#pragma unroll
        for (int u = 0; u < U; ++u)
#pragma unroll
            for (int c = 0; c < 2; ++c) {
                const int d = 2 * U * pos + 2 * u + c;
                if (d < D) base[r * D + d] = v[c][u];
            }
    };
    float z[2][U], x[2][U];
#pragma unroll
    for (int u = 0; u < U; ++u)
#pragma unroll
        for (int c = 0; c < 2; ++c) {
            const int d = 2 * U * pos + 2 * u + c;
            z[c][u] = d < D ? a.z[(size_t)row * D + d] : 0.f;
            x[c][u] = z[c][u];
        }
    float ld = solo_logdet_total(inverse(x));
    double logl = a.logl[row];
    if (writer_lane && a.x) store_row(a.x, (size_t)row, x);
    if (writer_lane && a.hist_x) store_row(a.hist_x, (size_t)row * (S + 1), x);
    const uint64_t walker = a.walker_offset + (uint64_t)row;
    int n_call = 0, n_move = 0, n_eval = 0;
    float zc[2][U], xc[2][U], ldc = 0.f;
    double lc = 0.0;
    for (int it = 1; it <= S; ++it) {
        float e[2][U];
        if (a.noise_dz) {
#pragma unroll
            for (int u = 0; u < U; ++u)
#pragma unroll
                for (int c = 0; c < 2; ++c) {
                    const int d = 2 * U * pos + 2 * u + c;
                    e[c][u] = d < D ? a.noise_dz[((size_t)(it - 1) * C + row) * D + d] : 0.f;
                }
        } else {
            slice_normals<U>(a.seed, walker, (uint32_t)it, pos, D, e);
        }
        const float u0 = noise_uniform(a.seed, walker, 64u * (uint32_t)it + 0u), u1 = noise_uniform(a.seed, walker, 64u * (uint32_t)it + 1u);
        const float logy = ld + __logf(u1);
        auto inside = [&](float t) -> bool {
            const float tw = t * a.width;
#pragma unroll
            for (int u = 0; u < U; ++u)
#pragma unroll
                for (int c = 0; c < 2; ++c) { zc[c][u] = __builtin_fmaf(e[c][u], tw, z[c][u]); xc[c][u] = zc[c][u]; }
            ldc = solo_logdet_total(inverse(xc));
            int okl = 1;
#pragma unroll
            for (int c = 0; c < 2; ++c)
#pragma unroll
                for (int u = 0; u < U; ++u) okl &= !(xc[c][u] < -1.f || xc[c][u] > 1.f);
            const bool inb = __ballot(okl != 0) == ~0ull;
            const bool pre = inb && (ldc > logy);
            lc = solo_loglike<U, LK>(like, D, lane, xc);
            n_eval += 1;
            n_call += pre ? 1 : 0;
            return pre && (lc > loglstar);
        };
        float tl = -u0, tr = 1.0f - u0;
        if (a.max_out > 0) {
            const int B = 2 * a.max_out;
            int n = 0;
            while (n <= B && inside(tl)) { tl -= 1.0f; n += 1; }
            while (n <= B && inside(tr)) { tr += 1.0f; n += 1; }
            if (n > B) {
                tl = -u0;
                tr = 1.0f - u0;
                const int nl = slice_stepout_left(a.seed, walker, (uint32_t)it, a.max_out);
                for (int j = 0; j < nl; ++j) { if (!inside(tl)) break; tl -= 1.0f; }
                for (int j = 0; j < B - nl; ++j) { if (!inside(tr)) break; tr += 1.0f; }
            }
        }
        bool moved = false;
        for (int k = 0; k < a.max_shrink; ++k) {
            const float uk = noise_uniform(a.seed, walker, 64u * (uint32_t)it + 2u + (uint32_t)k);
            const float t = __builtin_fmaf(tr - tl, uk, tl);
            if (inside(t)) { moved = true; break; }
            if (t < 0.f) tl = t; else tr = t;
        }
        if (moved) {
#pragma unroll
            for (int c = 0; c < 2; ++c)
#pragma unroll
                for (int u = 0; u < U; ++u) { z[c][u] = zc[c][u]; x[c][u] = xc[c][u]; }
            ld = ldc; logl = lc; n_move += 1;
        }
        if (writer_lane && a.hist_x) store_row(a.hist_x, (size_t)row * (S + 1) + it, x);
    }
    bool all_moved = n_move > 0;
    if (a.x) {
        bool mine = true;
        if (writer_lane) {
#pragma unroll
            for (int u = 0; u < U; ++u)
#pragma unroll
                for (int c = 0; c < 2; ++c) {
                    const int d = 2 * U * pos + 2 * u + c;
                    const float x0 = d < D ? a.x[(size_t)row * D + d] : 0.f;
                    mine = mine && (d >= D || x[c][u] != x0);
                }
        }
        all_moved = (__ballot(mine) & 0xffffull) == 0xffffull;
    }
    if (writer_lane) {
        store_row(a.z, (size_t)row, z);
        if (a.x) store_row(a.x, (size_t)row, x);
        if (pos == 0) {
            a.logl[row] = logl;
            if (a.n_call) a.n_call[row] = n_call;
            if (a.n_move) a.n_move[row] = n_move | (all_moved ? NNEST_MH_ALL_MOVED : 0);
            if (a.n_eval) a.n_eval[row] = n_eval;
        }
    }
}

__global__ void slice_fill_noise_kernel(float *__restrict__ dz, int steps, int C, int D, uint64_t seed, uint64_t walker_offset) {
    const long nq = (long)steps * C * ((D + 3) / 4);
    for (long i = (long)blockIdx.x * blockDim.x + threadIdx.x; i < nq; i += (long)gridDim.x * blockDim.x) {
        const int Q = (D + 3) / 4, q = (int)(i % Q), c = (int)((i / Q) % C), it = (int)(i / ((long)Q * C)) + 1;
        const f32x4 n = noise_normal4(seed, walker_offset + (uint64_t)c, (uint32_t)it, (uint32_t)q, NOISE_STREAM_DZ);
        float *o = dz + ((size_t)(it - 1) * C + c) * D + 4 * q;
        if (4 * q + 0 < D) o[0] = n.x;
        if (4 * q + 1 < D) o[1] = n.y;
        if (4 * q + 2 < D) o[2] = n.z;
        if (4 * q + 3 < D) o[3] = n.w;
    }
}

template <int U, int LK>
static hipError_t launch_slice_k(const FlowShape &s, const float *packed, const SliceArgs &a, hipStream_t st) {
    const size_t lds = solo_lds_weights<U, 4>() ? (size_t)3 * SOLO4_NF * 64 * sizeof(float) : (size_t)s.nets_params() * sizeof(float);
    hipError_t e = hipFuncSetAttribute(reinterpret_cast<const void *>(slice_kernel_solo<U, LK>), hipFuncAttributeMaxDynamicSharedMemorySize, (int)lds);
    if (e != hipSuccess) return e;
    hipLaunchKernelGGL((slice_kernel_solo<U, LK>), dim3((a.C + 3) / 4), dim3(256), lds, st, a, s, packed);
    return hipGetLastError();
}

bool slice_form_eligible(const FlowShape &s) {
    return s.kind == FLOW_KIND_NVP && s.H == 16 && s.B == 3 && s.L == 1 && s.scale_mode == 0 && s.NT >= 1 && s.NT <= 4;
}

hipError_t launch_slice_solo(const FlowShape &s, const float *packed, const SliceArgs &a, hipStream_t st) {
    if (a.C <= 0) return hipSuccess;
    if (!slice_form_eligible(s)) return hipErrorInvalidConfiguration;
    const bool rosen = a.like.id == NNEST_LIKE_ROSENBROCK;
    switch (s.NT) {
        case 1: return rosen ? launch_slice_k<1, NNEST_LIKE_ROSENBROCK>(s, packed, a, st) : launch_slice_k<1, -1>(s, packed, a, st);
        case 2: return rosen ? launch_slice_k<2, NNEST_LIKE_ROSENBROCK>(s, packed, a, st) : launch_slice_k<2, -1>(s, packed, a, st);
        case 3: return rosen ? launch_slice_k<3, NNEST_LIKE_ROSENBROCK>(s, packed, a, st) : launch_slice_k<3, -1>(s, packed, a, st);
        case 4: return rosen ? launch_slice_k<4, NNEST_LIKE_ROSENBROCK>(s, packed, a, st) : launch_slice_k<4, -1>(s, packed, a, st);
    }
    return hipErrorInvalidConfiguration;
}

hipError_t launch_slice_fill_noise(float *dz, int steps, int C, int D, uint64_t seed, uint64_t walker_offset, hipStream_t st) {
    hipLaunchKernelGGL(slice_fill_noise_kernel, dim3(256), dim3(256), 0, st, dz, steps, C, D, seed, walker_offset);
    return hipGetLastError();
}

int solo_walkers_per_group(int C, int num_cu) {
    static const int pinned = [] { const char *e = getenv("NNEST_SOLO_WPG"); return e ? atoi(e) : 0; }();
    for (int wpg = 4; wpg <= 12; wpg += 4) {
        if (pinned && wpg != pinned) continue;
        if ((C + wpg - 1) / wpg + 1 <= num_cu) return wpg;
    }
    return 0;
}

bool solo_form_eligible(const MhArgs &a, int num_cu) {
    const FlowShape &s = a.s;
    if (s.H != 16 || s.B != 3 || s.L != 1 || s.scale_mode != 0 || s.NT < 1 || s.NT > 4) return false;
    if (a.flags & NNEST_MH_DYNAMIC_STEP) return false;
    if ((a.flags & NNEST_MH_DYNAMIC_BATCH) && (mh_flag_lag(a.flags) == 1 || mh_flag_lag(a.flags) == 2)) return false;
    const int wpg = solo_walkers_per_group(a.C, num_cu);
    if (wpg != 4 && (a.noise_dz || a.hist_x || a.hist_logl)) return false;
    return wpg != 0;
}

template <int U, bool DBG, int LK, int WPG>
static hipError_t launch_solo_k(const MhArgs &a, hipStream_t st) {
    const int batch = (a.flags & NNEST_MH_DYNAMIC_BATCH) ? 1 : 0;
    const int grid = (a.C + WPG - 1) / WPG + batch;
    const size_t lds = solo_lds_weights<U, WPG>() ? (size_t)3 * SOLO4_NF * 64 * sizeof(float) : (size_t)a.s.nets_params() * sizeof(float);
    hipError_t e = hipFuncSetAttribute(reinterpret_cast<const void *>(mh_kernel_solo<U, DBG, LK, WPG>),
                                       hipFuncAttributeMaxDynamicSharedMemorySize, (int)lds);
    if (e != hipSuccess) return e;
    hipLaunchKernelGGL((mh_kernel_solo<U, DBG, LK, WPG>), dim3(grid), dim3(64 * (WPG + 2)), lds, st, a);
    return hipGetLastError();
}
template <int U, bool DBG, int LK>
static hipError_t launch_solo_w(const MhArgs &a, int wpg, hipStream_t st) {
    if (wpg == 4) return launch_solo_k<U, DBG, LK, 4>(a, st);
    if constexpr (!DBG) {
        if (wpg == 8) return launch_solo_k<U, DBG, LK, 8>(a, st);
        if (wpg == 12) return launch_solo_k<U, DBG, LK, 12>(a, st);
    }
    return hipErrorInvalidConfiguration;
}

hipError_t launch_mh_solo(const MhArgs &a_in, int num_cu, hipStream_t st) {
    MhArgs a = a_in;
    static const bool window_votes = [] { const char *e = getenv("NNEST_SOLO_VOTE"); return e && !strcmp(e, "window"); }();
    if (window_votes) a.flags |= NNEST_MH_WINDOW_VOTES_ONLY;
    const bool dbg = a.noise_dz || a.hist_x || a.hist_logl;
    const int wpg = solo_walkers_per_group(a.C, num_cu);
    if (!dbg && a.like.id == NNEST_LIKE_ROSENBROCK) {
        if (a.s.NT == 1) return launch_solo_w<1, false, NNEST_LIKE_ROSENBROCK>(a, wpg, st);
        if (a.s.NT == 2) return launch_solo_w<2, false, NNEST_LIKE_ROSENBROCK>(a, wpg, st);
        if (a.s.NT == 3) return launch_solo_w<3, false, NNEST_LIKE_ROSENBROCK>(a, wpg, st);
        if (a.s.NT == 4) return launch_solo_w<4, false, NNEST_LIKE_ROSENBROCK>(a, wpg, st);
    }
    switch (a.s.NT) {
        case 1: return dbg ? launch_solo_w<1, true, -1>(a, wpg, st) : launch_solo_w<1, false, -1>(a, wpg, st);
        case 2: return dbg ? launch_solo_w<2, true, -1>(a, wpg, st) : launch_solo_w<2, false, -1>(a, wpg, st);
        case 3: return dbg ? launch_solo_w<3, true, -1>(a, wpg, st) : launch_solo_w<3, false, -1>(a, wpg, st);
        case 4: return dbg ? launch_solo_w<4, true, -1>(a, wpg, st) : launch_solo_w<4, false, -1>(a, wpg, st);
    }
    return hipErrorInvalidConfiguration;
}

}
```

nnest_amd/csrc/nnest_train.hip:

```cpp
#include <string.h>
#include "nnest_internal.h"
#include "solo_tile.h"

namespace nnest {

#ifdef NNEST_STAMP
#define TSTAMP(v) do { __builtin_amdgcn_sched_barrier(0); v = __builtin_amdgcn_s_memtime(); __builtin_amdgcn_s_waitcnt(0xC07F); __builtin_amdgcn_sched_barrier(0); } while (0)
#define TACC(acc, t1, t0) acc += (t1) - (t0)
#else
#define TSTAMP(v) do { } while (0)
#define TACC(acc, t1, t0) do { } while (0)
#endif

enum { TRAIN_MODE_EPOCHS = 0, TRAIN_MODE_GRAD_ONLY = 1, TRAIN_MODE_VJP = 2 };
static const int TRAIN_THREADS = 512;
static const int TRAIN_WAVES = 8;
static const int TRAIN_MAX_ROWS = 128;

struct TrainArgs {
    float *w, *m, *v, *best_w, *img_fwd, *img_bwd, *grad;
    float *stash;
    const int *fwd_pos, *bwd_pos;
    int *adam_step;
    FlowShape s;
// ... 870 lines not shown
    switch (train_imglds<NT, NH, L>(a.s, min(a.batch, a.n_train), lds)) {
        case 2: return launch_train_tt<NT, NH, L, 2>(a, lds, st);
        case 1: return launch_train_tt<NT, NH, L, 1>(a, lds, st);
    }
    return launch_train_tt<NT, NH, L, 0>(a, lds, st);
}

#define TRAIN_SHAPES(X) \
    X(1, 1, 0) X(2, 1, 0) X(3, 1, 0) X(4, 1, 0) X(1, 1, 1) X(2, 1, 1) X(3, 1, 1) X(4, 1, 1) X(1, 1, 2) X(2, 1, 2) X(3, 1, 2) X(4, 1, 2) \
    X(1, 2, 1) X(2, 2, 1) X(1, 2, 2) X(2, 2, 2) X(1, 4, 1) \
    X(1, 1, 3) X(2, 1, 3) X(3, 1, 3) X(4, 1, 3) X(1, 2, 0) X(2, 2, 0) X(1, 2, 3) X(2, 2, 3) X(1, 4, 0) X(1, 4, 2) X(1, 4, 3)

static hipError_t dispatch_train(const TrainArgs &a, hipStream_t st) {
    const FlowShape &s = a.s;
#define TRY_SHAPE(nt, nh, l) if (s.NT == nt && s.NH == nh && s.L == l) return launch_train_t<nt, nh, l>(a, st);
    TRAIN_SHAPES(TRY_SHAPE)
#undef TRY_SHAPE
    return hipErrorInvalidConfiguration;
}

static int train_imglds_for(const FlowShape &s) {
    size_t lds;
#define TRY_SHAPE(nt, nh, l) if (s.NT == nt && s.NH == nh && s.L == l) return train_imglds<nt, nh, l>(s, TRAIN_MAX_ROWS, lds);
    TRAIN_SHAPES(TRY_SHAPE)
#undef TRY_SHAPE
    return -1;
}

#include "nnest_train_grid.h"
#include "nnest_train_rows.h"
#pragma clang fp contract(off)
__device__ __forceinline__ float adam_elem(float wi, float g, float &mref, float &vref, float step_size, float inv_bc2s, float wd) {
    const float b1 = 0.9f, b2 = 0.999f, eps = 1e-8f;
    const float gi = g + wd * wi;
    const float mi = mref + (gi - mref) * (1.0f - b1);
    const float vi = vref * b2 + ((1.0f - b2) * gi) * gi;
    mref = mi; vref = vi;
    return wi - step_size * (mi / (sqrtf(vi) * inv_bc2s + eps));
}
#pragma clang fp contract(fast)

#include "maf_train.h"

hipError_t launch_loss_grad(const float *packed, const FlowShape &s, const float *x, int M, float *grad, float *loss,
                            float *workspace, float *img_fwd, const int *fwd_pos, const int *bwd_pos, hipStream_t st) {
    TrainArgs a;
    memset(&a, 0, sizeof(a));
    a.w = const_cast<float *>(packed);
    a.img_fwd = img_fwd;
    a.img_bwd = workspace;
    a.stash = workspace + s.image_floats + s.num_params() + 64;
    a.fwd_pos = fwd_pos;
    a.bwd_pos = bwd_pos;
    a.grad = grad;
    a.s = s;
    a.xtrain = x;
    a.n_train = M;
    a.batch = M;
    a.loss_out = loss;
    a.mode = TRAIN_MODE_GRAD_ONLY;
    return dispatch_train(a, st);
}

hipError_t launch_vjp(const float *packed, const FlowShape &s, const float *x, const float *gz, float gld, int M, float *grad, float *gx,
                      float *workspace, float *img_fwd, const int *fwd_pos, const int *bwd_pos, hipStream_t st) {
    TrainArgs a;
    memset(&a, 0, sizeof(a));
    a.w = const_cast<float *>(packed);
    a.img_fwd = img_fwd;
    a.img_bwd = workspace;
    a.stash = workspace + s.image_floats + s.num_params() + 64;
    a.fwd_pos = fwd_pos;
    a.bwd_pos = bwd_pos;
    a.grad = grad;
    a.s = s;
    a.xtrain = x;
    a.n_train = M;
    a.batch = M;
    a.gz = gz; a.gx = gx; a.gld_in = gld;
    a.mode = TRAIN_MODE_VJP;
    return dispatch_train(a, st);
}

__global__ void adam_packed_kernel(float *__restrict__ w, const float *__restrict__ grad, float *__restrict__ m, float *__restrict__ v, int n,
                                   float step_size, float inv_bc2s, float wd) {
    const float b1 = 0.9f, b2 = 0.999f, eps = 1e-8f;
    for (int i = blockIdx.x * blockDim.x + threadIdx.x; i < n; i += gridDim.x * blockDim.x) {
        const float gi = grad[i] + wd * w[i];
        const float mi = m[i] + (gi - m[i]) * (1.0f - b1);
        const float vi = v[i] * b2 + (1.0f - b2) * gi * gi;
        m[i] = mi; v[i] = vi;
        w[i] = w[i] - step_size * (mi / (sqrtf(vi) * inv_bc2s + eps));
    }
}

__global__ void adam_packed_dev_kernel(float *__restrict__ w, const float *__restrict__ grad, float *__restrict__ m, float *__restrict__ v, int n,
                                       const int *__restrict__ step_dev, float lr, float wd) {
    const int step = *step_dev + 1;
    const double bc1 = 1.0 - pow(0.9, (double)step), bc2 = 1.0 - pow(0.999, (double)step);
    const float step_size = (float)((double)lr / bc1), inv_bc2s = (float)(1.0 / sqrt(bc2));
    for (int i = blockIdx.x * blockDim.x + threadIdx.x; i < n; i += gridDim.x * blockDim.x) {
        float mi = m[i], vi = v[i];
        w[i] = adam_elem(w[i], grad[i], mi, vi, step_size, inv_bc2s, wd);
        m[i] = mi; v[i] = vi;
    }
}
__global__ void adam_step_advance_kernel(int *step_dev) { *step_dev += 1; }

hipError_t launch_adam_packed_dev(float *w, const float *grad, float *m, float *v, int n, int *step_dev, float lr, float wd, hipStream_t st) {
    hipLaunchKernelGGL(adam_packed_dev_kernel, dim3(64), dim3(256), 0, st, w, grad, m, v, n, step_dev, lr, wd);
    hipLaunchKernelGGL(adam_step_advance_kernel, dim3(1), dim3(1), 0, st, step_dev);
    return hipGetLastError();
}

hipError_t launch_adam_packed(float *w, const float *grad, float *m, float *v, int n, int step, float lr, float wd, hipStream_t st) {
    const double bc1 = 1.0 - pow(0.9, (double)step), bc2 = 1.0 - pow(0.999, (double)step);
    hipLaunchKernelGGL(adam_packed_kernel, dim3(64), dim3(256), 0, st, w, grad, m, v, n, (float)((double)lr / bc1), (float)(1.0 / sqrt(bc2)), wd);
    return hipGetLastError();
}

enum { TRAIN_FORM_SINGLE = 0, TRAIN_FORM_GRID = 1, TRAIN_FORM_ROWS = 2 };
static int epoch_form(const TrainArgs &a) {
    if (!grid_eligible(a)) return TRAIN_FORM_SINGLE;
    return rows_eligible(a) ? TRAIN_FORM_ROWS : TRAIN_FORM_GRID;
}

hipError_t launch_train(float *packed, float *adam_m, float *adam_v, float *best_w, float *img, int *adam_step_dev,
                        const FlowShape &s, const float *xtrain, int n_train, const float *xvalid, int n_valid,
                        const int *perm, const float *noise, uint64_t seed, float jitter, int batch, int max_epochs,
                        int patience, float lr, float wd, int epoch_offset, int flags, float *losses,
                        nnest_train_result_t *result, float *workspace, const int *fwd_pos, const int *bwd_pos,
                        hipStream_t st) {
    TrainArgs a;
    memset(&a, 0, sizeof(a));
    a.w = packed; a.m = adam_m; a.v = adam_v; a.best_w = best_w; a.img_fwd = img;
    a.img_bwd = workspace;
    a.stash = workspace + s.image_floats + s.num_params() + 64;
    a.fwd_pos = fwd_pos;
    a.bwd_pos = bwd_pos;
    a.grad = workspace + s.image_floats;
    a.adam_step = adam_step_dev;
    a.s = s;
    a.xtrain = xtrain; a.n_train = n_train; a.xvalid = xvalid; a.n_valid = n_valid;
    a.perm = perm; a.noise = noise; a.seed = seed; a.jitter = jitter; a.batch = batch;
    a.max_epochs = max_epochs; a.patience = patience; a.lr = lr; a.wd = wd;
    a.losses = losses; a.result = result;
    a.epoch_offset = epoch_offset; a.flags = flags;
    a.mode = TRAIN_MODE_EPOCHS;
    float *gridws = workspace + ((single_workspace_floats(s) + 63) & ~(size_t)63);
    switch (epoch_form(a)) {
        case TRAIN_FORM_ROWS: return dispatch_train_rows(a, gridws, st);
        case TRAIN_FORM_GRID: return dispatch_train_grid(a, gridws, st);
    }
    return dispatch_train(a, st);
}

int train_form_for(const FlowShape &s, int batch, int flags, int *detail) {
    TrainArgs a;
    memset(&a, 0, sizeof(a));
    a.s = s; a.batch = batch; a.flags = flags;
    a.mode = TRAIN_MODE_EPOCHS;
    const int form = epoch_form(a);
    if (detail)
        *detail = form == TRAIN_FORM_ROWS ? s.NT : form == TRAIN_FORM_GRID ? 10 * s.NT + s.L : train_imglds_for(s);
    return form;
}

}
```

nnest_amd/csrc/solo_tile.h:

```cpp
#pragma once
#include "flow_tile.h"

namespace nnest {

static __device__ __forceinline__ void solo_barrier() { asm volatile("s_waitcnt lgkmcnt(0)\n\ts_barrier" ::: "memory"); }

template <int N>
static __device__ __forceinline__ float solo_ror(float v) {
    return __builtin_bit_cast(float, __builtin_amdgcn_update_dpp(0, __builtin_bit_cast(int, v), 0x120 + N, 0xf, 0xf, true));
}
static __device__ __forceinline__ float solo_join(float v) {
    float a = v, b = v;
    asm volatile("s_nop 1\n\tv_permlane16_swap_b32 %0, %1" : "+v"(a), "+v"(b));
    return a + b;
}
static __device__ __forceinline__ float solo_join_rot(float v) {
    float a = v, b;
    asm volatile("s_nop 1\n\tv_mov_b32_dpp %1, %0 row_ror:8 row_mask:0xf bank_mask:0xf\n\ts_nop 1\n\tv_permlane16_swap_b32 %0, %1" : "+v"(a), "=&v"(b));
    return a + b;
}
static __device__ __forceinline__ void solo_nets(float v, float &from_scale, float &from_translate) {
    float a = v, b = v;
    asm volatile("s_nop 1\n\tv_permlane32_swap_b32 %0, %1" : "+v"(a), "+v"(b));
    from_scale = a;
// ... 120 lines not shown
static __device__ __forceinline__ void solo_swap16(float &a, float &b) {
    asm volatile("s_nop 1\n\tv_permlane16_swap_b32 %0, %1\n\ts_nop 0" : "+v"(a), "+v"(b));
}

template <int U>
static __device__ __forceinline__ float solo_coupling_inverse1(const SoloNet<U> &w, unsigned sel, bool h1, const float (&cond)[U],
                                                               float (&trans)[U]) {
    static_assert(U == 1, "the statement-by-statement block: one slot per class");
    float a0, a1;
    solo_chain_1(a0, a1, w.b1, solo_rot8_h1(cond[0]), w.w1[0]);
    float hid = solo_activate(solo_join_rot(a0 + a1), sel);
    solo_chain_1(a0, a1, w.b2, hid, w.w2);
    const float hin = solo_activate(solo_join_rot(a0 + a1), sel);
    float o0, o1;
    solo_chain_1(o0, o1, w.b3[0], hin, w.w3[0]);
    float ls, tt;
    solo_nets(solo_join(o0 + o1), ls, tt);
    trans[0] = (trans[0] - tt) * __expf(-ls);
    return h1 ? 0.f : -ls;
}

#define SOLO_BD(acc, x, w, t) "v_fmac_f32_dpp %[" #acc "], %[" #x "], %[" #w "] row_ror:" #t " row_mask:0xf bank_mask:0xf\n\t"
#define SOLO_BW8(n, a) [n##0] "v"(a[0]), [n##1] "v"(a[1]), [n##2] "v"(a[2]), [n##3] "v"(a[3]), [n##4] "v"(a[4]), [n##5] "v"(a[5]), [n##6] "v"(a[6]), [n##7] "v"(a[7])
#define SOLO_BLOCK2_ACT                                            \
        "v_exp_f32 %[p0], %[a0]\n\t"                                                                                          \
        "v_max_f32 %[p1], 0, %[a0]\n\t"                                                                                       \
        "v_add_f32 %[p0], 1.0, %[p0]\n\t"                                                                                     \
        "v_rcp_f32 %[p0], %[p0]\n\t"                                                                                          \
        "s_nop 0\n\t"                                                                                                         \
        "v_fma_f32 %[p0], %[p0], -2.0, 1.0\n\t"                                                                               \
        "v_bfi_b32 %[a0], %[sel], %[p1], %[p0]\n\t"
#define SOLO_BLOCK2(LD_LINE)                                                                                                  \
        "v_mov_b32 %[p0], %[c0]\n\t"                                                                                          \
        "v_mov_b32 %[p1], %[c1]\n\t"                                                                                          \
        "v_bfi_b32 %[cur], %[h1], %[i1], %[i0]\n\t"                  \
        "v_mov_b32_dpp %[p0], %[c0] row_ror:8 row_mask:0xa bank_mask:0xf\n\t"                                                 \
        "v_mov_b32_dpp %[p1], %[c1] row_ror:8 row_mask:0xa bank_mask:0xf\n\t"                                                 \
        "v_fma_f32 %[a0], %[p0], %[wa0], %[b1]\n\t"                                                                           \
        "v_mul_f32 %[a1], %[p1], %[wb0]\n\t"                                                                                  \
        SOLO_BD(a1, p1, wb1, 1) SOLO_BD(a0, p0, wa1, 1) SOLO_BD(a1, p1, wb2, 2) SOLO_BD(a0, p0, wa2, 2)                       \
        SOLO_BD(a1, p1, wb3, 3) SOLO_BD(a0, p0, wa3, 3) SOLO_BD(a1, p1, wb4, 4) SOLO_BD(a0, p0, wa4, 4)                       \
        SOLO_BD(a1, p1, wb5, 5) SOLO_BD(a0, p0, wa5, 5) SOLO_BD(a1, p1, wb6, 6) SOLO_BD(a0, p0, wa6, 6)                       \
        SOLO_BD(a1, p1, wb7, 7) SOLO_BD(a0, p0, wa7, 7)                                                                       \
        "v_add_f32 %[p1], %[a0], %[a1]\n\t"                                                                                   \
        "v_mov_b32_dpp %[p0], %[a1] row_ror:8 row_mask:0xf bank_mask:0xf\n\t"                                                 \
        "v_add_f32_dpp %[p0], %[a0], %[p0] row_ror:8 row_mask:0xf bank_mask:0xf\n\t"                                          \
        "s_nop 1\n\t"                                                                                                         \
        "v_permlane16_swap_b32 %[p1], %[p0]\n\t"                                                                              \
        "v_add_f32 %[a0], %[p1], %[p0]\n\t"                                                                                   \
        SOLO_BLOCK2_ACT                                                                                                       \
        "v_fma_f32 %[p0], %[a0], %[wc0], %[b2]\n\t"                                                                           \
        "s_nop 0\n\t"                                                                                                         \
        "v_mul_f32_dpp %[p1], %[a0], %[wc1] row_ror:1 row_mask:0xf bank_mask:0xf\n\t"                                         \
        SOLO_BD(p0, a0, wc2, 2) SOLO_BD(p1, a0, wc3, 3) SOLO_BD(p0, a0, wc4, 4) SOLO_BD(p1, a0, wc5, 5)                       \
        SOLO_BD(p0, a0, wc6, 6) SOLO_BD(p1, a0, wc7, 7)                                                                       \
        "v_add_f32 %[a0], %[p0], %[p1]\n\t"                                                                                   \
        "v_add_f32 %[a1], %[p0], %[p1]\n\t"                                                                                   \
        "s_nop 1\n\t"                                                                                                         \
        "v_permlane16_swap_b32 %[a0], %[a1]\n\t"                                                                              \
        "v_add_f32 %[a0], %[a0], %[a1]\n\t"                                                                                   \
        SOLO_BLOCK2_ACT                                                                                                       \
        "v_fma_f32 %[p0], %[a0], %[wd0], %[b3]\n\t"                                                                           \
        "v_mov_b32 %[p1], 0\n\t"                                                                                              \
        SOLO_BD(p1, a0, we0, 8)                                                                                               \
        SOLO_BD(p0, a0, wd1, 1) SOLO_BD(p1, a0, we1, 9) SOLO_BD(p0, a0, wd2, 2) SOLO_BD(p1, a0, we2, 10)                      \
        SOLO_BD(p0, a0, wd3, 3) SOLO_BD(p1, a0, we3, 11) SOLO_BD(p0, a0, wd4, 4) SOLO_BD(p1, a0, we4, 12)                     \
        SOLO_BD(p0, a0, wd5, 5) SOLO_BD(p1, a0, we5, 13) SOLO_BD(p0, a0, wd6, 6) SOLO_BD(p1, a0, we6, 14)                     \
        SOLO_BD(p0, a0, wd7, 7) SOLO_BD(p1, a0, we7, 15)                                                                      \
        "v_add_f32 %[a0], %[p0], %[p1]\n\t"                                                                                   \
        "v_add_f32 %[a1], %[p0], %[p1]\n\t"                                                                                   \
        "s_nop 1\n\t"                                                                                                         \
        "v_permlane32_swap_b32 %[a0], %[a1]\n\t"                                       \
        "v_mul_f32 %[p0], 0xbfb8aa3b, %[a0]\n\t"                                                                              \
        "v_exp_f32 %[p0], %[p0]\n\t"                                                                                          \
        "v_sub_f32 %[p1], %[cur], %[a1]\n\t"                                                                                  \
        "v_mul_f32 %[t0], %[p1], %[p0]\n\t"                                                                                   \
        "v_mul_f32 %[t1], %[p1], %[p0]\n\t"                                                                                   \
        LD_LINE                                                                                                               \
        "s_nop 0\n\t"                                                                                                         \
        "v_permlane16_swap_b32 %[t0], %[t1]\n\t"
#define SOLO_BLOCK2_IN(w)                                                                                                     \
        [c0] "v"(c0), [c1] "v"(c1), [i0] "v"(i0), [i1] "v"(i1), [sel] "v"(sel), [h1] "v"(h1v), [b1] "v"(w.b1), [b2] "v"(w.b2), [b3] "v"(w.b3[0]),          \
        SOLO_BW8(wa, w.w1[0]), SOLO_BW8(wb, w.w1[1]), SOLO_BW8(wc, w.w2), SOLO_BW8(wd, w.w3[0]), SOLO_BW8(we, w.w3[1])
template <bool FIRST>
static __device__ __forceinline__ void solo_block2(const SoloNet<2> &w, unsigned sel, unsigned h1v, float c0, float c1, float i0, float i1,
                                                   float &t0, float &t1, float &ld) {
    float p0, p1, a0, a1, cur;
    if constexpr (FIRST) {
        asm(SOLO_BLOCK2("v_mul_f32 %[ld], -1.0, %[a0]\n\t")
            : [t0] "=&v"(t0), [t1] "=&v"(t1), [ld] "=&v"(ld), [p0] "=&v"(p0), [p1] "=&v"(p1), [a0] "=&v"(a0), [a1] "=&v"(a1), [cur] "=&v"(cur)
            : SOLO_BLOCK2_IN(w));
    } else {
        asm(SOLO_BLOCK2("v_sub_f32 %[ld], %[ld], %[a0]\n\t")
            : [t0] "=&v"(t0), [t1] "=&v"(t1), [ld] "+v"(ld), [p0] "=&v"(p0), [p1] "=&v"(p1), [a0] "=&v"(a0), [a1] "=&v"(a1), [cur] "=&v"(cur)
            : SOLO_BLOCK2_IN(w));
    }
}

template <int U, bool FIRST>
static __device__ __forceinline__ void solo_coupling_inverse(const SoloNet<U> &w, unsigned sel, bool h1, const float (&cond)[U],
                                                              float (&trans)[U], float &ld) {
    if constexpr (U == 2) {
        float t0, t1;
        solo_block2<FIRST>(w, sel, h1 ? 0xffffffffu : 0u, cond[0], cond[1], trans[0], trans[1], t0, t1, ld);
        trans[0] = t0;
        trans[1] = t1;
    } else {
        const float v = solo_coupling_inverse1<U>(w, sel, h1, cond, trans);
        ld = FIRST ? v : ld + v;
    }
}
static __device__ __forceinline__ float solo_logdet_total(float ld) { return solo_join(solo_row_sum(ld)); }
#define SOLO_LADDER(a, t) "v_add_f32_dpp %[" #a "], %[" #a "], %[" #a "] row_ror:" #t " row_mask:0xf bank_mask:0xf bound_ctrl:1\n\t"
static __device__ __forceinline__ void solo_logdet_total_and_row_sum(float &ld, float &v) {
    float l2;
    asm("s_nop 1\n\t"
        SOLO_LADDER(ld, 8) SOLO_LADDER(v, 8) "s_nop 0\n\t"
        SOLO_LADDER(ld, 4) SOLO_LADDER(v, 4) "s_nop 0\n\t"
        SOLO_LADDER(ld, 2) SOLO_LADDER(v, 2) "s_nop 0\n\t"
        "v_add_f32_dpp %[l2], %[ld], %[ld] row_ror:1 row_mask:0xf bank_mask:0xf bound_ctrl:1\n\t"
        SOLO_LADDER(ld, 1) SOLO_LADDER(v, 1)
        "s_nop 0\n\t"
        "v_permlane16_swap_b32 %[ld], %[l2]\n\t"
        "v_add_f32 %[ld], %[ld], %[l2]\n\t"
        : [ld] "+v"(ld), [v] "+v"(v), [l2] "=&v"(l2));
}

constexpr int SOLO4_NF = 80;
template <int U>
static __device__ __forceinline__ void solo4_store(float *base, int b, const SoloNet<U> &n, int lane) {
    float *q = base + (size_t)b * SOLO4_NF * 64;
    auto put = [&](int f, float v) { q[((size_t)(f >> 2) * 64 + lane) * 4 + (f & 3)] = v; };
#pragma unroll
    for (int u = 0; u < U; ++u)
#pragma unroll
        for (int t = 0; t < 8; ++t) { put(8 * u + t, n.w1[u][t]); put(40 + 8 * u + t, n.w3[u][t]); }
#pragma unroll
    for (int t = 0; t < 8; ++t) put(32 + t, n.w2[t]);
    put(72, n.b1); put(73, n.b2);
#pragma unroll
    for (int u = 0; u < 4; ++u) put(74 + u, u < U ? n.b3[u < U ? u : 0] : 0.f);
    put(78, 0.f); put(79, 0.f);
}
static __device__ __forceinline__ void solo4_load8(float (&w)[8], const float *blk, int f0, int lane) {
    const f32x4 a = *reinterpret_cast<const f32x4 *>(blk + ((size_t)(f0 >> 2) * 64 + lane) * 4);
    const f32x4 b = *reinterpret_cast<const f32x4 *>(blk + ((size_t)((f0 >> 2) + 1) * 64 + lane) * 4);
    w[0] = a.x; w[1] = a.y; w[2] = a.z; w[3] = a.w; w[4] = b.x; w[5] = b.y; w[6] = b.z; w[7] = b.w;
}
struct Solo4Lds {
    const float *blk; int lane;
    __device__ __forceinline__ void load8(float (&w)[8], int f0) const { solo4_load8(w, blk, f0, lane); }
    __device__ __forceinline__ f32x4 bias(int c) const { return *reinterpret_cast<const f32x4 *>(blk + ((size_t)(18 + c) * 64 + lane) * 4); }
};
template <int U>
struct Solo4Reg {
    const SoloNet<U> &n;
    __device__ __forceinline__ void load8(float (&w)[8], int f0) const {
#pragma unroll
        for (int t = 0; t < 8; ++t) w[t] = f0 < 32 ? n.w1[(f0 >> 3) < U ? (f0 >> 3) : 0][t] : (f0 < 40 ? n.w2[t] : n.w3[((f0 - 40) >> 3) < U ? ((f0 - 40) >> 3) : 0][t]);
    }
    __device__ __forceinline__ f32x4 bias(int c) const {
        return c == 0 ? (f32x4){n.b1, n.b2, n.b3[0], U > 1 ? n.b3[U > 1 ? 1 : 0] : 0.f}
                      : (f32x4){U > 2 ? n.b3[U > 2 ? 2 : 0] : 0.f, U > 3 ? n.b3[U > 3 ? 3 : 0] : 0.f, 0.f, 0.f};
    }
};
template <int U, class W>
static __device__ __forceinline__ float solo_coupling_inverse4(const W &wsrc, unsigned sel, bool h1, const float (&cond)[U], float (&trans)[U]) {
    const f32x4 bA = wsrc.bias(0);
    const f32x4 bB = wsrc.bias(1);
    float wa[8], wb[8];
    float a0, a1;
    if constexpr (U >= 2) {
        wsrc.load8(wa, 0); wsrc.load8(wb, 8);
        solo_chain_2in(a0, a1, bA.x, solo_rot8_h1(cond[0]), solo_rot8_h1(cond[U >= 2 ? 1 : 0]), wa, wb);
    }
    if constexpr (U == 4) {
        wsrc.load8(wa, 16); wsrc.load8(wb, 24);
        solo_chain_2in_acc(a0, a1, solo_rot8_h1(cond[U == 4 ? 2 : 0]), solo_rot8_h1(cond[U == 4 ? 3 : 0]), wa, wb);
    }
    if constexpr (U == 1) {
        wsrc.load8(wa, 0);
        solo_chain_1(a0, a1, bA.x, solo_rot8_h1(cond[0]), wa);
    }
    if constexpr (U == 3) {
        wsrc.load8(wa, 16);
        solo_chain_1_acc(a0, a1, solo_rot8_h1(cond[U - 1]), wa);
    }
    float hid = solo_activate(solo_join_rot(a0 + a1), sel);
    wsrc.load8(wa, 32);
    solo_chain_1(a0, a1, bA.y, hid, wa);
    constexpr bool FULLK = U == 2;
    const float hin = solo_activate(FULLK ? solo_join(a0 + a1) : solo_join_rot(a0 + a1), sel);
    float ld = 0.f;
#pragma unroll
    for (int k = 0; k < U / 2; ++k) {
        float o0, o1;
        wsrc.load8(wa, 40 + 16 * k); wsrc.load8(wb, 48 + 16 * k);
        if constexpr (FULLK) {
            solo_chain_full(o0, o1, bA.z, hin, wa, wb);
        } else {
            solo_chain_2out(o0, o1, k == 0 ? bA.z : bB.x, k == 0 ? bA.w : bB.y, hin, wa, wb);
            solo_swap16(o0, o1);
        }
        float ls, tt;
        solo_nets(o0 + o1, ls, tt);
        const float cur = h1 ? trans[2 * k + 1] : trans[2 * k];
        float nw = (cur - tt) * __expf(-ls);
        float nb = nw;
        solo_swap16(nw, nb);
        trans[2 * k] = nw;
        trans[2 * k + 1] = nb;
        ld -= ls;
    }
    if constexpr (U & 1) {
        float o0, o1;
        wsrc.load8(wa, 40 + 8 * (U - 1));
        solo_chain_1(o0, o1, U == 1 ? bA.z : bB.x, hin, wa);
        float ls, tt;
        solo_nets(solo_join(o0 + o1), ls, tt);
        trans[U - 1] = (trans[U - 1] - tt) * __expf(-ls);
        ld -= h1 ? 0.f : ls;
    }
    return ld;
}

}
```

Before: 916.9 million.

## Precompute solo weight image at repack and table once per device

New measurement: 938.4 million (median of 6 runs). 1.02x the previous value.

```diff
diff --git a/nnest_amd/csrc/flow_tile.h b/nnest_amd/csrc/flow_tile.h
--- a/nnest_amd/csrc/flow_tile.h
+++ b/nnest_amd/csrc/flow_tile.h
@@ -7,6 +7,7 @@
 
 typedef float f32x4 __attribute__((ext_vector_type(4)));
 enum { FLOW_KIND_NVP = 0, FLOW_KIND_MAF = 1 };
+constexpr int SOLO_IMAGE_FLOATS = 3 * 80 * 64;
 
 struct FlowShape {
     int D, H, B, L;
@@ -21,6 +22,9 @@
     __host__ __device__ int nets_params() const { return B * 2 * net_params; }
     __host__ __device__ int num_params() const { return B * 2 * net_params + (scale_mode == 2 ? B : 0); }
     __host__ __device__ int image_total() const { return image_floats + (scale_mode == 2 ? B : 0); }
+    __host__ __device__ bool has_solo_image() const { return kind == FLOW_KIND_NVP && H == 16 && B == 3 && L == 1 && NT >= 1 && NT <= 4; }
+    __host__ __device__ int solo_image_offset() const { return (image_total() + 3) & ~3; }
+    __host__ __device__ int image_alloc_floats() const { return has_solo_image() ? solo_image_offset() + SOLO_IMAGE_FLOATS : image_total(); }
 };
 
 __host__ __device__ inline int frag_off_L1() { return 0; }
diff --git a/nnest_amd/csrc/nnest_abi.hip b/nnest_amd/csrc/nnest_abi.hip
--- a/nnest_amd/csrc/nnest_abi.hip
+++ b/nnest_amd/csrc/nnest_abi.hip
@@ -122,18 +122,19 @@
     if (e == hipSuccess) e = hipMalloc((void **)&h->adam_m, nb);
     if (e == hipSuccess) e = hipMalloc((void **)&h->adam_v, nb);
     if (e == hipSuccess) e = hipMalloc((void **)&h->best_w, nb);
-    if (e == hipSuccess) e = hipMalloc((void **)&h->img, (size_t)s.image_total() * sizeof(float));
+    if (e == hipSuccess) e = hipMalloc((void **)&h->img, (size_t)s.image_alloc_floats() * sizeof(float));
     if (e == hipSuccess) e = hipMalloc((void **)&h->adam_step, sizeof(int));
     if (e == hipSuccess) e = hipMalloc((void **)&h->train_ws, h->train_ws_floats * sizeof(float));
     if (e == hipSuccess) e = hipMalloc((void **)&h->fwd_pos, nb);
     if (e == hipSuccess) e = hipMalloc((void **)&h->bwd_pos, nb);
     if (e == hipSuccess) e = launch_build_pos(h->fwd_pos, h->bwd_pos, s, 0);
+    if (e == hipSuccess) e = solo_prepare_device(h->device, 0);
     if (e == hipSuccess) e = hipStreamSynchronize(0);
     if (e == hipSuccess) e = hipMemset(h->w, 0, nb);
     if (e == hipSuccess) e = hipMemset(h->adam_m, 0, nb);
     if (e == hipSuccess) e = hipMemset(h->adam_v, 0, nb);
     if (e == hipSuccess) e = hipMemset(h->adam_step, 0, sizeof(int));
-    if (e == hipSuccess) e = hipMemset(h->img, 0, (size_t)s.image_total() * sizeof(float));
+    if (e == hipSuccess) e = hipMemset(h->img, 0, (size_t)s.image_alloc_floats() * sizeof(float));
     if (e != hipSuccess) {
         nnest_nvp_destroy(h);
         return fail(NNEST_E_HIP, "device allocation failed: %s", hipGetErrorString(e));
@@ -386,7 +387,7 @@
         return fail(NNEST_E_UNSUPPORTED, "slice proposal: hidden 16, 3 blocks, 1 layer, scale '' (the one-walker-per-wave layout), x_dim <= 128");
     const SliceArgs a = {z_dev, x_dev, logl_dev, loglstar, width, steps, C, max_stepout, max_shrink, lk, seed, walker_offset, noise_dz_dev,
                          hist_x_dev, nullptr, n_call_dev, n_move_dev, n_eval_dev};
-    hipError_t e = launch_slice_solo(h->s, h->w, a, (hipStream_t)stream);
+    hipError_t e = launch_slice_solo(h->s, h->img + h->s.solo_image_offset(), a, (hipStream_t)stream);
     if (e != hipSuccess) return fail(NNEST_E_HIP, "launch_slice_solo: %s", hipGetErrorString(e));
     return NNEST_OK;
 }
diff --git a/nnest_amd/csrc/nnest_internal.h b/nnest_amd/csrc/nnest_internal.h
--- a/nnest_amd/csrc/nnest_internal.h
+++ b/nnest_amd/csrc/nnest_internal.h
@@ -27,6 +27,8 @@
 hipError_t launch_mh_quad(const MhArgs &a, int num_cu, hipStream_t st);
 bool solo_form_eligible(const MhArgs &a, int num_cu);
 hipError_t launch_mh_solo(const MhArgs &a, int num_cu, hipStream_t st);
+hipError_t launch_solo_image(const float *packed, float *limg, const FlowShape &s, hipStream_t st);
+hipError_t solo_prepare_device(int device, hipStream_t st);
 int mh_form_for(const FlowShape &s, int C, int flags, int num_cu);
 bool maf_shape_supported(const FlowShape &s);
 hipError_t launch_maf_repack(const float *packed, float *imgf, float *imgb, const FlowShape &s, hipStream_t st);
@@ -78,7 +80,7 @@
                                 float *grad, float *loss, float *workspace, hipStream_t st);
 hipError_t launch_training_jitter(const double *samples, int N, int D, double *out, hipStream_t st);
 bool slice_form_eligible(const FlowShape &s);
-hipError_t launch_slice_solo(const FlowShape &s, const float *packed, const SliceArgs &a, hipStream_t st);
+hipError_t launch_slice_solo(const FlowShape &s, const float *limg, const SliceArgs &a, hipStream_t st);
 hipError_t launch_slice_fill_noise(float *dz, int steps, int C, int D, uint64_t seed, uint64_t walker_offset, hipStream_t st);
 size_t ensemble_work_words(int C, int S);
 bool ensemble_form_eligible(const FlowShape &s);
diff --git a/nnest_amd/csrc/nnest_kernels.hip b/nnest_amd/csrc/nnest_kernels.hip
--- a/nnest_amd/csrc/nnest_kernels.hip
+++ b/nnest_amd/csrc/nnest_kernels.hip
@@ -675,7 +675,9 @@
     int block = 256, grid = (s.image_floats + block - 1) / block;
     if (grid > 1024) grid = 1024;
     hipLaunchKernelGGL(repack_fragments_kernel, dim3(grid), dim3(block), 0, st, packed, img, s);
-    return hipGetLastError();
+    hipError_t e = hipGetLastError();
+    if (e == hipSuccess && s.has_solo_image()) e = launch_solo_image(packed, img + s.solo_image_offset(), s, st);
+    return e;
 }
 
 static hipError_t launch_maf_pass(const PassArgs &a, int num_cu, hipStream_t st);
diff --git a/nnest_amd/csrc/nnest_solo.hip b/nnest_amd/csrc/nnest_solo.hip
--- a/nnest_amd/csrc/nnest_solo.hip
+++ b/nnest_amd/csrc/nnest_solo.hip
@@ -1,4 +1,5 @@
 #include <string.h>
+#include <mutex>
 #include "mh_common.h"
 #include "nnest_internal.h"
 #include "solo_loglike.h"
@@ -6,7 +7,54 @@
 
 namespace nnest {
 
+#ifdef NNEST_STAMP
+#define PSTAMP(v) do { __builtin_amdgcn_sched_barrier(0); v = __builtin_amdgcn_s_memtime(); __builtin_amdgcn_s_waitcnt(0xC07F); __builtin_amdgcn_sched_barrier(0); } while (0)
+#define PSTAMP_DRAINED(v) do { __builtin_amdgcn_sched_barrier(0); __builtin_amdgcn_s_waitcnt(0x0070); v = __builtin_amdgcn_s_memtime(); __builtin_amdgcn_s_waitcnt(0xC07F); __builtin_amdgcn_sched_barrier(0); } while (0)
+#ifndef NNEST_STAMP_STEPS
+#undef STAMP
+#define STAMP(v) do { } while (0)
+#endif
+#else
+#define PSTAMP(v) do { } while (0)
+#define PSTAMP_DRAINED(v) do { } while (0)
+#endif
+
 static constexpr int SOLO_ETAB = 1024;
+__device__ double solo_etab_dev[SOLO_ETAB];
+__global__ void solo_etab_kernel() {
+    const int k = blockIdx.x * blockDim.x + threadIdx.x;
+    if (k < SOLO_ETAB) solo_etab_dev[k] = exp(1.0 / (double)(1 + k));
+}
+hipError_t solo_prepare_device(int device, hipStream_t st) {
+    static std::mutex mu;
+    static bool done[64];
+    std::lock_guard<std::mutex> g(mu);
+    if (device < 0 || device >= 64) return hipErrorInvalidDevice;
+    if (done[device]) return hipSuccess;
+    hipLaunchKernelGGL(solo_etab_kernel, dim3(SOLO_ETAB / 256), dim3(256), 0, st);
+    hipError_t e = hipGetLastError();
+    if (e == hipSuccess) e = hipStreamSynchronize(st);
+    done[device] = e == hipSuccess;
+    return e;
+}
+
+template <int U>
+__global__ void __launch_bounds__(192) solo_image_kernel(const float *__restrict__ packed, float *__restrict__ limg, int D, int net_params) {
+    const int lane = threadIdx.x & 63, b = threadIdx.x >> 6;
+    SoloNet<U> nb;
+    solo_gather<U>(nb, packed + (size_t)(b * 2 + (lane >= 32 ? 1 : 0)) * net_params, D, (b + 1) & 1, b & 1, lane);
+    solo4_store<U>(limg, b, nb, lane);
+}
+hipError_t launch_solo_image(const float *packed, float *limg, const FlowShape &s, hipStream_t st) {
+    if (!s.has_solo_image()) return hipErrorInvalidConfiguration;
+    switch (s.NT) {
+        case 1: hipLaunchKernelGGL(solo_image_kernel<1>, dim3(1), dim3(192), 0, st, packed, limg, s.D, s.net_params); break;
+        case 2: hipLaunchKernelGGL(solo_image_kernel<2>, dim3(1), dim3(192), 0, st, packed, limg, s.D, s.net_params); break;
+        case 3: hipLaunchKernelGGL(solo_image_kernel<3>, dim3(1), dim3(192), 0, st, packed, limg, s.D, s.net_params); break;
+        case 4: hipLaunchKernelGGL(solo_image_kernel<4>, dim3(1), dim3(192), 0, st, packed, limg, s.D, s.net_params); break;
+    }
+    return hipGetLastError();
+}
 
 template <int U, int WPG> constexpr bool solo_lds_weights() { return U >= 3 || WPG > 4; }
 template <int U, int WPG> constexpr int solo_reg_blocks() { return !solo_lds_weights<U, WPG>() ? 3 : (WPG == 4 ? 1 : (U <= 2 && WPG == 8 ? 1 : 0)); }
@@ -24,6 +72,7 @@
     __shared__ float fs_cand[2];
     __shared__ int vote_sel;
     __shared__ double etab[SOLO_ETAB];
+    __shared__ __attribute__((aligned(16))) float x0buf[WPG][16][2 * U];
 
     const int lane = threadIdx.x & 63, wave = __builtin_amdgcn_readfirstlane(threadIdx.x >> 6);
     const int tile = blockIdx.x;
@@ -48,21 +97,42 @@
         }
         return;
     }
-    {
-        if constexpr (!LDSW) {
-            const int n = a.s.nets_params();
-            for (int i = threadIdx.x; i < n; i += blockDim.x) wlds[i] = a.packed[i];
+    unsigned long long p0 = 0, p1 = 0, p2 = 0, p3 = 0, p4 = 0, p5 = 0, p6 = 0, p7 = 0, p8 = 0;
+    (void)p0; (void)p1; (void)p2; (void)p3; (void)p4; (void)p5; (void)p6; (void)p7; (void)p8;
+    PSTAMP(p0);
+    const float *limg = a.img + a.s.solo_image_offset();
+    const int j = wave;
+    const int pos = lane & 15;
+    const bool translate_half = lane >= 32;
+    const bool writer_lane = lane < 16;
+    const int row = tile * WPG + j;
+    const bool ok = row < C;
+    SoloNet<U> net[RB > 0 ? RB : 1];
+    float z[2][U];
+    double logl = 0.0;
+    if (wave < WPG) {
+        if constexpr (LDSW) {
+            if constexpr (RB == 1) solo_image_load<U>(net[0], limg + (size_t)1 * SOLO4_NF * 64, lane);
         } else {
-            if (wave < 3) {
-                SoloNet<U> nb;
-                solo_gather<U>(nb, a.packed + (size_t)(wave * 2 + (lane >= 32 ? 1 : 0)) * a.s.net_params, D, (wave + 1) & 1, wave & 1, lane);
-                solo4_store<U>(wlds, wave, nb, lane);
-            }
-        }
-        if (dynamic && use_tab)
-            for (int k = threadIdx.x; k < S + 2; k += blockDim.x) etab[k] = exp(1.0 / (double)(1 + k));
-    }
+#pragma unroll
+            for (int b = 0; b < 3; ++b) solo_image_load<U>(net[b], limg + (size_t)b * SOLO4_NF * 64, lane);
+        }
+#pragma unroll
+        for (int u = 0; u < U; ++u)
+#pragma unroll
+            for (int c = 0; c < 2; ++c) {
+                const int d = 2 * U * pos + 2 * u + c;
+                z[c][u] = (ok && d < D) ? a.z[(size_t)row * D + d] : 0.f;
+            }
+        logl = ok ? a.logl[row] : 0.0;
+    }
+    if constexpr (LDSW) solo_image_to_lds<64 * (WPG + 2)>(wlds, limg);
+    PSTAMP(p1);
+    if (dynamic && use_tab)
+        for (int k = threadIdx.x; k < S + 2; k += blockDim.x) etab[k] = solo_etab_dev[k];
+    PSTAMP(p2);
     __syncthreads();
+    PSTAMP(p3);
 
     if (wave == WPG) {
         const int g = lane & 3, j = min(lane >> 2, WPG - 1);
@@ -110,7 +180,9 @@
         };
         STAMP(n2);
         draw(0);
+        PSTAMP(p4);
         solo_barrier();
+        PSTAMP(p5);
         if (S >= 1) {
             draw(1);
             solo_barrier();
@@ -130,7 +202,13 @@
         { unsigned long long n3 = 0; STAMP(n3); n_all = n3 - n2; }
 #endif
 #ifdef NNEST_STAMP
-        if (a.scale_out && lane == 0 && tile == 0) { a.scale_out[4] = (float)n_gen; a.scale_out[5] = (float)n_all; }
+        PSTAMP(p8);
+        if (a.scale_out && lane == 0 && tile == 0) {
+            float *o = a.scale_out;
+            o[4] = (float)n_gen; o[5] = (float)n_all;
+            o[32] = (float)(p1 - p0); o[33] = (float)(p2 - p1); o[34] = (float)(p3 - p2); o[35] = (float)(p4 - p3); o[36] = (float)(p5 - p4);
+            o[37] = (float)(p8 - p5); o[38] = (float)(p8 - p0);
+        }
 #endif
 #ifndef NNEST_STAMP
         if (!dynamic && a.scale_out && lane == 0) {
@@ -248,25 +326,10 @@
         return;
     }
 
-    const int j = wave;
-    const int pos = lane & 15;
-    const bool translate_half = lane >= 32;
-    const bool writer_lane = lane < 16;
-    const int row = tile * WPG + j;
-    const bool ok = row < C;
     const LikeSpec like = a.like;
     const double loglstar = a.loglstar;
     const bool free_mode = (a.flags & NNEST_MH_UNCONSTRAINED) != 0;
-
-    SoloNet<U> net[RB > 0 ? RB : 1];
-    if constexpr (LDSW) {
-        if constexpr (RB == 1)
-            solo_gather<U>(net[0], a.packed + (size_t)(1 * 2 + (translate_half ? 1 : 0)) * a.s.net_params, D, (1 + 1) & 1, 1 & 1, lane);
-    } else {
-#pragma unroll
-        for (int b = 0; b < 3; ++b)
-            solo_gather<U>(net[b], wlds + (size_t)(b * 2 + (translate_half ? 1 : 0)) * a.s.net_params, D, (b + 1) & 1, b & 1, lane);
-    }
+    PSTAMP(p4);
     const unsigned sel = translate_half ? 0xffffffffu : 0u;
     const bool h1 = (lane & 16) != 0;
     auto inverse = [&](float (&xs)[2][U]) {
@@ -285,17 +348,12 @@
         }
     };
 
-    float z[2][U], x[2][U];
+    float x[2][U];
 #pragma unroll
     for (int u = 0; u < U; ++u)
 #pragma unroll
-        for (int c = 0; c < 2; ++c) {
-            const int d = 2 * U * pos + 2 * u + c;
-            z[c][u] = (ok && d < D) ? a.z[(size_t)row * D + d] : 0.f;
-            x[c][u] = z[c][u];
-        }
+        for (int c = 0; c < 2; ++c) x[c][u] = z[c][u];
     float ld = solo_logdet_total(inverse(x));
-    double logl = ok ? a.logl[row] : 0.0;
     int n_acc = 0, n_call = 0;
 
     auto store_row = [&](float *base, size_t r, const float (&v)[2][U]) {
@@ -307,7 +365,12 @@
                 if (d < D) base[r * D + d] = v[c][u];
             }
     };
-    if (writer_lane && ok && a.x) store_row(a.x, (size_t)row, x);
+    if (writer_lane && a.x) {
+#pragma unroll
+        for (int u = 0; u < U; ++u)
+#pragma unroll
+            for (int c = 0; c < 2; ++c) x0buf[j][pos][2 * u + c] = x[c][u];
+    }
     if (DBG && writer_lane && ok) {
         if (a.hist_x) store_row(a.hist_x, (size_t)row * (S + 1), x);
         if (a.hist_logl && pos == 0) a.hist_logl[(size_t)row * (S + 1)] = logl;
@@ -325,7 +388,9 @@
         fs_next = fsbuf[kbuf & 1];
         ++kbuf;
     };
+    PSTAMP(p5);
     fetch_noise();
+    PSTAMP(p6);
 
     unsigned long long st0 = 0, st1 = 0, st2 = 0, st3 = 0, a_prop = 0, a_inv = 0, a_post = 0, a_tot = 0;
     (void)st0; (void)st1; (void)st2; (void)st3; (void)a_prop; (void)a_inv; (void)a_post; (void)a_tot;
@@ -429,6 +494,7 @@
 #endif
     }
     if (exact_all) solo_barrier();
+    PSTAMP(p7);
 #ifdef NNEST_STAMP
     if (a.scale_out && lane == 0 && tile == 0) {
         float *o = a.scale_out;
@@ -445,7 +511,7 @@
 #pragma unroll
                 for (int c = 0; c < 2; ++c) {
                     const int d = 2 * U * pos + 2 * u + c;
-                    const float x0 = (ok && d < D) ? a.x[(size_t)row * D + d] : 0.f;
+                    const float x0 = x0buf[j][pos][2 * u + c];
                     mine = mine && (d >= D || x[c][u] != x0);
                 }
         }
@@ -460,6 +526,14 @@
             if (a.n_call) a.n_call[row] = n_call;
         }
     }
+#ifdef NNEST_STAMP
+    PSTAMP_DRAINED(p8);
+    if (a.scale_out && lane == 0 && tile == 0 && j == 0) {
+        float *o = a.scale_out;
+        o[16] = (float)(p1 - p0); o[17] = (float)(p2 - p1); o[18] = (float)(p3 - p2); o[19] = (float)(p4 - p3); o[20] = (float)(p5 - p4);
+        o[21] = (float)(p6 - p5); o[22] = (float)(p7 - p6); o[23] = (float)(p8 - p7); o[24] = (float)(p8 - p0);
+    }
+#endif
 }
 
 template <int U>
@@ -483,22 +557,16 @@
 }
 
 template <int U, int LK>
-__global__ void __launch_bounds__(256) slice_kernel_solo(SliceArgs a, FlowShape s, const float *packed) {
+__global__ void __launch_bounds__(256) slice_kernel_solo(SliceArgs a, FlowShape s, const float *limg) {
     extern __shared__ __attribute__((aligned(16))) float wlds[];
+    __shared__ __attribute__((aligned(16))) float x0buf[4][16][2 * U];
     const int lane = threadIdx.x & 63, wave = __builtin_amdgcn_readfirstlane(threadIdx.x >> 6);
     const int D = s.D, S = a.steps, C = a.C;
     constexpr bool LDSW = solo_lds_weights<U, 4>();
-    {
-        if constexpr (!LDSW) {
-            const int n = s.nets_params();
-            for (int i = threadIdx.x; i < n; i += blockDim.x) wlds[i] = packed[i];
-        } else if (wave < 3) {
-            SoloNet<U> nb;
-            solo_gather<U>(nb, packed + (size_t)(wave * 2 + (lane >= 32 ? 1 : 0)) * s.net_params, D, (wave + 1) & 1, wave & 1, lane);
-            solo4_store<U>(wlds, wave, nb, lane);
-        }
-    }
-    __syncthreads();
+    if constexpr (LDSW) {
+        solo_image_to_lds<256>(wlds, limg);
+        __syncthreads();
+    }
     const int pos = lane & 15;
     const bool translate_half = lane >= 32, writer_lane = lane < 16;
     const int row = blockIdx.x * 4 + wave;
@@ -509,8 +577,7 @@
     SoloNet<U> net[LDSW ? 1 : 3];
     if constexpr (!LDSW) {
 #pragma unroll
-        for (int b = 0; b < 3; ++b)
-            solo_gather<U>(net[b], wlds + (size_t)(b * 2 + (translate_half ? 1 : 0)) * s.net_params, D, (b + 1) & 1, b & 1, lane);
+        for (int b = 0; b < 3; ++b) solo_image_load<U>(net[b], limg + (size_t)b * SOLO4_NF * 64, lane);
     }
     const unsigned sel = translate_half ? 0xffffffffu : 0u;
     const bool h1 = (lane & 16) != 0;
@@ -548,7 +615,12 @@
         }
     float ld = solo_logdet_total(inverse(x));
     double logl = a.logl[row];
-    if (writer_lane && a.x) store_row(a.x, (size_t)row, x);
+    if (writer_lane && a.x) {
+#pragma unroll
+        for (int u = 0; u < U; ++u)
+#pragma unroll
+            for (int c = 0; c < 2; ++c) x0buf[wave][pos][2 * u + c] = x[c][u];
+    }
     if (writer_lane && a.hist_x) store_row(a.hist_x, (size_t)row * (S + 1), x);
     const uint64_t walker = a.walker_offset + (uint64_t)row;
     int n_call = 0, n_move = 0, n_eval = 0;
@@ -627,7 +699,7 @@
 #pragma unroll
                 for (int c = 0; c < 2; ++c) {
                     const int d = 2 * U * pos + 2 * u + c;
-                    const float x0 = d < D ? a.x[(size_t)row * D + d] : 0.f;
+                    const float x0 = x0buf[wave][pos][2 * u + c];
                     mine = mine && (d >= D || x[c][u] != x0);
                 }
         }
@@ -659,11 +731,11 @@
 }
 
 template <int U, int LK>
-static hipError_t launch_slice_k(const FlowShape &s, const float *packed, const SliceArgs &a, hipStream_t st) {
-    const size_t lds = solo_lds_weights<U, 4>() ? (size_t)3 * SOLO4_NF * 64 * sizeof(float) : (size_t)s.nets_params() * sizeof(float);
+static hipError_t launch_slice_k(const FlowShape &s, const float *limg, const SliceArgs &a, hipStream_t st) {
+    const size_t lds = solo_lds_weights<U, 4>() ? (size_t)3 * SOLO4_NF * 64 * sizeof(float) : 0;
     hipError_t e = hipFuncSetAttribute(reinterpret_cast<const void *>(slice_kernel_solo<U, LK>), hipFuncAttributeMaxDynamicSharedMemorySize, (int)lds);
     if (e != hipSuccess) return e;
-    hipLaunchKernelGGL((slice_kernel_solo<U, LK>), dim3((a.C + 3) / 4), dim3(256), lds, st, a, s, packed);
+    hipLaunchKernelGGL((slice_kernel_solo<U, LK>), dim3((a.C + 3) / 4), dim3(256), lds, st, a, s, limg);
     return hipGetLastError();
 }
 
@@ -671,15 +743,15 @@
     return s.kind == FLOW_KIND_NVP && s.H == 16 && s.B == 3 && s.L == 1 && s.scale_mode == 0 && s.NT >= 1 && s.NT <= 4;
 }
 
-hipError_t launch_slice_solo(const FlowShape &s, const float *packed, const SliceArgs &a, hipStream_t st) {
+hipError_t launch_slice_solo(const FlowShape &s, const float *limg, const SliceArgs &a, hipStream_t st) {
     if (a.C <= 0) return hipSuccess;
     if (!slice_form_eligible(s)) return hipErrorInvalidConfiguration;
     const bool rosen = a.like.id == NNEST_LIKE_ROSENBROCK;
     switch (s.NT) {
-        case 1: return rosen ? launch_slice_k<1, NNEST_LIKE_ROSENBROCK>(s, packed, a, st) : launch_slice_k<1, -1>(s, packed, a, st);
-        case 2: return rosen ? launch_slice_k<2, NNEST_LIKE_ROSENBROCK>(s, packed, a, st) : launch_slice_k<2, -1>(s, packed, a, st);
-        case 3: return rosen ? launch_slice_k<3, NNEST_LIKE_ROSENBROCK>(s, packed, a, st) : launch_slice_k<3, -1>(s, packed, a, st);
-        case 4: return rosen ? launch_slice_k<4, NNEST_LIKE_ROSENBROCK>(s, packed, a, st) : launch_slice_k<4, -1>(s, packed, a, st);
+        case 1: return rosen ? launch_slice_k<1, NNEST_LIKE_ROSENBROCK>(s, limg, a, st) : launch_slice_k<1, -1>(s, limg, a, st);
+        case 2: return rosen ? launch_slice_k<2, NNEST_LIKE_ROSENBROCK>(s, limg, a, st) : launch_slice_k<2, -1>(s, limg, a, st);
+        case 3: return rosen ? launch_slice_k<3, NNEST_LIKE_ROSENBROCK>(s, limg, a, st) : launch_slice_k<3, -1>(s, limg, a, st);
+        case 4: return rosen ? launch_slice_k<4, NNEST_LIKE_ROSENBROCK>(s, limg, a, st) : launch_slice_k<4, -1>(s, limg, a, st);
     }
     return hipErrorInvalidConfiguration;
 }
@@ -712,7 +784,7 @@
 static hipError_t launch_solo_k(const MhArgs &a, hipStream_t st) {
     const int batch = (a.flags & NNEST_MH_DYNAMIC_BATCH) ? 1 : 0;
     const int grid = (a.C + WPG - 1) / WPG + batch;
-    const size_t lds = solo_lds_weights<U, WPG>() ? (size_t)3 * SOLO4_NF * 64 * sizeof(float) : (size_t)a.s.nets_params() * sizeof(float);
+    const size_t lds = solo_lds_weights<U, WPG>() ? (size_t)3 * SOLO4_NF * 64 * sizeof(float) : 0;
     hipError_t e = hipFuncSetAttribute(reinterpret_cast<const void *>(mh_kernel_solo<U, DBG, LK, WPG>),
                                        hipFuncAttributeMaxDynamicSharedMemorySize, (int)lds);
     if (e != hipSuccess) return e;
diff --git a/nnest_amd/csrc/nnest_train.hip b/nnest_amd/csrc/nnest_train.hip
--- a/nnest_amd/csrc/nnest_train.hip
+++ b/nnest_amd/csrc/nnest_train.hip
@@ -1046,7 +1046,9 @@
         case TRAIN_FORM_ROWS: return dispatch_train_rows(a, gridws, st);
         case TRAIN_FORM_GRID: return dispatch_train_grid(a, gridws, st);
     }
-    return dispatch_train(a, st);
+    hipError_t e = dispatch_train(a, st);
+    if (e == hipSuccess && s.has_solo_image()) e = launch_solo_image(a.w, img + s.solo_image_offset(), s, st);
+    return e;
 }
 
 int train_form_for(const FlowShape &s, int batch, int flags, int *detail) {
diff --git a/nnest_amd/csrc/solo_tile.h b/nnest_amd/csrc/solo_tile.h
--- a/nnest_amd/csrc/solo_tile.h
+++ b/nnest_amd/csrc/solo_tile.h
@@ -296,6 +296,36 @@
     __device__ __forceinline__ void load8(float (&w)[8], int f0) const { solo4_load8(w, blk, f0, lane); }
     __device__ __forceinline__ f32x4 bias(int c) const { return *reinterpret_cast<const f32x4 *>(blk + ((size_t)(18 + c) * 64 + lane) * 4); }
 };
+static_assert(3 * SOLO4_NF * 64 == SOLO_IMAGE_FLOATS, "flow_tile.h sizes the allocation");
+template <int U>
+static __device__ __forceinline__ void solo_image_load(SoloNet<U> &n, const float *blk, int lane) {
+    const Solo4Lds src{blk, lane};
+#pragma unroll
+    for (int u = 0; u < U; ++u) { src.load8(n.w1[u], 8 * u); src.load8(n.w3[u], 40 + 8 * u); }
+    src.load8(n.w2, 32);
+    const f32x4 bA = src.bias(0);
+    n.b1 = bA.x; n.b2 = bA.y; n.b3[0] = bA.z;
+    if constexpr (U >= 2) n.b3[U >= 2 ? 1 : 0] = bA.w;
+    if constexpr (U >= 3) {
+        const f32x4 bB = src.bias(1);
+        n.b3[U >= 3 ? 2 : 0] = bB.x;
+        if constexpr (U >= 4) n.b3[U >= 4 ? 3 : 0] = bB.y;
+    }
+}
+template <int NTHR>
+static __device__ __forceinline__ void solo_image_to_lds(float *wlds, const float *limg) {
+    constexpr int N4 = SOLO_IMAGE_FLOATS / 4, TRIPS = (N4 + NTHR - 1) / NTHR;
+    const f32x4 *src = reinterpret_cast<const f32x4 *>(limg);
+    f32x4 *dst = reinterpret_cast<f32x4 *>(wlds);
+    f32x4 v[TRIPS];
+#pragma unroll
+    for (int i = 0; i < TRIPS; ++i)
+        if (N4 % NTHR == 0 || (int)threadIdx.x + i * NTHR < N4) v[i] = src[threadIdx.x + i * NTHR];
+#pragma unroll
+    for (int i = 0; i < TRIPS; ++i)
+        if (N4 % NTHR == 0 || (int)threadIdx.x + i * NTHR < N4) dst[threadIdx.x + i * NTHR] = v[i];
+}
+
 template <int U>
 struct Solo4Reg {
     const SoloNet<U> &n;
diff --git a/profiles/r08/k4_solo_loop.s b/profiles/r08/k4_solo_loop.s
--- /dev/null
+++ b/profiles/r08/k4_solo_loop.s
@@ -0,0 +1,446 @@
+	v_mov_b32_e32 v183, v177
+	v_mov_b32_e32 v184, v178
+	v_mov_b32_e32 v182, v176
+	v_mov_b32_e32 v210, v207
+	v_mov_b32_e32 v185, v179
+	s_waitcnt lgkmcnt(1)
+	v_mov_b32_e32 v205, v208
+	v_cndmask_b32_e64 v142, v198, v179, s[10:11]
+	v_add_u32_sdwa v45, v45, v142 dst_sel:DWORD dst_unused:UNUSED_PAD src0_sel:DWORD src1_sel:BYTE_0
+	v_add_u32_e32 v195, v195, v209
+	v_cndmask_b32_e64 v134, v134, v177, s[14:15]
+	v_cndmask_b32_e64 v136, v136, v178, s[14:15]
+	v_cndmask_b32_e64 v135, v135, v176, s[14:15]
+	s_cmp_eq_u32 s29, s31
+	v_cndmask_b32_e64 v137, v137, v207, s[14:15]
+	s_cbranch_scc1 1847
+	s_and_b64 vcc, exec, s[72:73]
+	s_cbranch_vccnz 592
+	s_and_b32 s14, s49, 1
+	s_lshl_b32 s15, s14, 4
+	s_waitcnt lgkmcnt(0)
+	v_pk_fma_f32 v[172:173], v[138:139], v[186:187], v[146:147] op_sel_hi:[1,0,1]
+	v_lshl_add_u32 v138, s14, 10, v196
+	s_add_i32 s15, s57, s15
+	s_lshl_b32 s14, s14, 2
+	s_waitcnt lgkmcnt(0)
+	s_barrier
+	v_mov_b32_e32 v142, s15
+	v_mov_b32_e32 v143, s14
+	v_pk_fma_f32 v[174:175], v[140:141], v[186:187], v[150:151] op_sel_hi:[1,0,1]
+	ds_read_b128 v[138:141], v138
+	ds_read_b32 v208, v142
+	ds_read_b32 v186, v143 offset:12352
+	v_mov_b32_e32 v142, v173
+	v_mov_b32_e32 v143, v175
+	v_bfi_b32 v153, v93, v174, v172
+	v_mov_b32_dpp v142, v173 row_ror:8 row_mask:0xa bank_mask:0xf
+	v_mov_b32_dpp v143, v175 row_ror:8 row_mask:0xa bank_mask:0xf
+	v_fma_f32 v144, v142, v94, v74
+	v_mul_f32_e32 v145, v143, v102
+	v_fmac_f32_dpp v145, v143, v103 row_ror:1 row_mask:0xf bank_mask:0xf
+	v_fmac_f32_dpp v144, v142, v95 row_ror:1 row_mask:0xf bank_mask:0xf
+	v_fmac_f32_dpp v145, v143, v104 row_ror:2 row_mask:0xf bank_mask:0xf
+	v_fmac_f32_dpp v144, v142, v96 row_ror:2 row_mask:0xf bank_mask:0xf
+	v_fmac_f32_dpp v145, v143, v105 row_ror:3 row_mask:0xf bank_mask:0xf
+	v_fmac_f32_dpp v144, v142, v97 row_ror:3 row_mask:0xf bank_mask:0xf
+	v_fmac_f32_dpp v145, v143, v106 row_ror:4 row_mask:0xf bank_mask:0xf
+	v_fmac_f32_dpp v144, v142, v98 row_ror:4 row_mask:0xf bank_mask:0xf
+	v_fmac_f32_dpp v145, v143, v107 row_ror:5 row_mask:0xf bank_mask:0xf
+	v_fmac_f32_dpp v144, v142, v99 row_ror:5 row_mask:0xf bank_mask:0xf
+	v_fmac_f32_dpp v145, v143, v108 row_ror:6 row_mask:0xf bank_mask:0xf
+	v_fmac_f32_dpp v144, v142, v100 row_ror:6 row_mask:0xf bank_mask:0xf
+	v_fmac_f32_dpp v145, v143, v109 row_ror:7 row_mask:0xf bank_mask:0xf
+	v_fmac_f32_dpp v144, v142, v101 row_ror:7 row_mask:0xf bank_mask:0xf
+	v_add_f32_e32 v143, v144, v145
+	v_mov_b32_dpp v142, v145 row_ror:8 row_mask:0xf bank_mask:0xf
+	v_add_f32_dpp v142, v144, v142 row_ror:8 row_mask:0xf bank_mask:0xf
+	s_nop 1
+	v_permlane16_swap_b32_e32 v143, v142
+	v_add_f32_e32 v144, v143, v142
+	v_exp_f32_e32 v142, v144
+	v_max_f32_e32 v143, 0, v144
+	v_add_f32_e32 v142, 1.0, v142
+	v_rcp_f32_e32 v142, v142
+	s_nop 0
+	v_fma_f32 v142, v142, -2.0, 1.0
+	v_bfi_b32 v144, v77, v143, v142
+	v_fma_f32 v142, v144, v110, v75
+	s_nop 0
+	v_mul_f32_dpp v143, v144, v111 row_ror:1 row_mask:0xf bank_mask:0xf
+	v_fmac_f32_dpp v142, v144, v112 row_ror:2 row_mask:0xf bank_mask:0xf
+	v_fmac_f32_dpp v143, v144, v113 row_ror:3 row_mask:0xf bank_mask:0xf
+	v_fmac_f32_dpp v142, v144, v114 row_ror:4 row_mask:0xf bank_mask:0xf
+	v_fmac_f32_dpp v143, v144, v115 row_ror:5 row_mask:0xf bank_mask:0xf
+	v_fmac_f32_dpp v142, v144, v116 row_ror:6 row_mask:0xf bank_mask:0xf
+	v_fmac_f32_dpp v143, v144, v117 row_ror:7 row_mask:0xf bank_mask:0xf
+	v_add_f32_e32 v144, v142, v143
+	v_add_f32_e32 v145, v142, v143
+	s_nop 1
+	v_permlane16_swap_b32_e32 v144, v145
+	v_add_f32_e32 v144, v144, v145
+	v_exp_f32_e32 v142, v144
+	v_max_f32_e32 v143, 0, v144
+	v_add_f32_e32 v142, 1.0, v142
+	v_rcp_f32_e32 v142, v142
+	s_nop 0
+	v_fma_f32 v142, v142, -2.0, 1.0
+	v_bfi_b32 v144, v77, v143, v142
+	v_fma_f32 v142, v144, v118, v76
+	v_mov_b32_e32 v143, 0
+	v_fmac_f32_dpp v143, v144, v122 row_ror:8 row_mask:0xf bank_mask:0xf
+	v_fmac_f32_dpp v142, v144, v119 row_ror:1 row_mask:0xf bank_mask:0xf
+	v_fmac_f32_dpp v143, v144, v123 row_ror:9 row_mask:0xf bank_mask:0xf
+	v_fmac_f32_dpp v142, v144, v120 row_ror:2 row_mask:0xf bank_mask:0xf
+	v_fmac_f32_dpp v143, v144, v124 row_ror:10 row_mask:0xf bank_mask:0xf
+	v_fmac_f32_dpp v142, v144, v121 row_ror:3 row_mask:0xf bank_mask:0xf
+	v_fmac_f32_dpp v143, v144, v125 row_ror:11 row_mask:0xf bank_mask:0xf
+	v_fmac_f32_dpp v142, v144, v126 row_ror:4 row_mask:0xf bank_mask:0xf
+	v_fmac_f32_dpp v143, v144, v130 row_ror:12 row_mask:0xf bank_mask:0xf
+	v_fmac_f32_dpp v142, v144, v127 row_ror:5 row_mask:0xf bank_mask:0xf
+	v_fmac_f32_dpp v143, v144, v131 row_ror:13 row_mask:0xf bank_mask:0xf
+	v_fmac_f32_dpp v142, v144, v128 row_ror:6 row_mask:0xf bank_mask:0xf
+	v_fmac_f32_dpp v143, v144, v132 row_ror:14 row_mask:0xf bank_mask:0xf
+	v_fmac_f32_dpp v142, v144, v129 row_ror:7 row_mask:0xf bank_mask:0xf
+	v_fmac_f32_dpp v143, v144, v133 row_ror:15 row_mask:0xf bank_mask:0xf
+	v_add_f32_e32 v144, v142, v143
+	v_add_f32_e32 v145, v142, v143
+	s_nop 1
+	v_permlane32_swap_b32_e32 v144, v145
+	v_mul_f32_e32 v142, 0xbfb8aa3b, v144
+	v_exp_f32_e32 v142, v142
+	v_sub_f32_e32 v143, v153, v145
+	v_mul_f32_e32 v179, v143, v142
+	v_mul_f32_e32 v180, v143, v142
+	v_mul_f32_e32 v206, -1.0, v144
+	s_nop 0
+	v_permlane16_swap_b32_e32 v179, v180
+	s_nop 0
+	v_mov_b32_e32 v142, v179
+	v_mov_b32_e32 v143, v180
+	v_bfi_b32 v153, v93, v175, v173
+	v_mov_b32_dpp v142, v179 row_ror:8 row_mask:0xa bank_mask:0xf
+	v_mov_b32_dpp v143, v180 row_ror:8 row_mask:0xa bank_mask:0xf
+	v_fma_f32 v144, v142, v46, v90
+	v_mul_f32_e32 v145, v143, v54
+	v_fmac_f32_dpp v145, v143, v55 row_ror:1 row_mask:0xf bank_mask:0xf
+	v_fmac_f32_dpp v144, v142, v47 row_ror:1 row_mask:0xf bank_mask:0xf
+	v_fmac_f32_dpp v145, v143, v56 row_ror:2 row_mask:0xf bank_mask:0xf
+	v_fmac_f32_dpp v144, v142, v48 row_ror:2 row_mask:0xf bank_mask:0xf
+	v_fmac_f32_dpp v145, v143, v57 row_ror:3 row_mask:0xf bank_mask:0xf
+	v_fmac_f32_dpp v144, v142, v49 row_ror:3 row_mask:0xf bank_mask:0xf
+	v_fmac_f32_dpp v145, v143, v58 row_ror:4 row_mask:0xf bank_mask:0xf
+	v_fmac_f32_dpp v144, v142, v50 row_ror:4 row_mask:0xf bank_mask:0xf
+	v_fmac_f32_dpp v145, v143, v59 row_ror:5 row_mask:0xf bank_mask:0xf
+	v_fmac_f32_dpp v144, v142, v51 row_ror:5 row_mask:0xf bank_mask:0xf
+	v_fmac_f32_dpp v145, v143, v60 row_ror:6 row_mask:0xf bank_mask:0xf
+	v_fmac_f32_dpp v144, v142, v52 row_ror:6 row_mask:0xf bank_mask:0xf
+	v_fmac_f32_dpp v145, v143, v61 row_ror:7 row_mask:0xf bank_mask:0xf
+	v_fmac_f32_dpp v144, v142, v53 row_ror:7 row_mask:0xf bank_mask:0xf
+	v_add_f32_e32 v143, v144, v145
+	v_mov_b32_dpp v142, v145 row_ror:8 row_mask:0xf bank_mask:0xf
+	v_add_f32_dpp v142, v144, v142 row_ror:8 row_mask:0xf bank_mask:0xf
+	s_nop 1
+	v_permlane16_swap_b32_e32 v143, v142
+	v_add_f32_e32 v144, v143, v142
+	v_exp_f32_e32 v142, v144
+	v_max_f32_e32 v143, 0, v144
+	v_add_f32_e32 v142, 1.0, v142
+	v_rcp_f32_e32 v142, v142
+	s_nop 0
+	v_fma_f32 v142, v142, -2.0, 1.0
+	v_bfi_b32 v144, v77, v143, v142
+	v_fma_f32 v142, v144, v62, v91
+	s_nop 0
+	v_mul_f32_dpp v143, v144, v63 row_ror:1 row_mask:0xf bank_mask:0xf
+	v_fmac_f32_dpp v142, v144, v64 row_ror:2 row_mask:0xf bank_mask:0xf
+	v_fmac_f32_dpp v143, v144, v65 row_ror:3 row_mask:0xf bank_mask:0xf
+	v_fmac_f32_dpp v142, v144, v66 row_ror:4 row_mask:0xf bank_mask:0xf
+	v_fmac_f32_dpp v143, v144, v67 row_ror:5 row_mask:0xf bank_mask:0xf
+	v_fmac_f32_dpp v142, v144, v68 row_ror:6 row_mask:0xf bank_mask:0xf
+	v_fmac_f32_dpp v143, v144, v69 row_ror:7 row_mask:0xf bank_mask:0xf
+	v_add_f32_e32 v144, v142, v143
+	v_add_f32_e32 v145, v142, v143
+	s_nop 1
+	v_permlane16_swap_b32_e32 v144, v145
+	v_add_f32_e32 v144, v144, v145
+	v_exp_f32_e32 v142, v144
+	v_max_f32_e32 v143, 0, v144
+	v_add_f32_e32 v142, 1.0, v142
+	v_rcp_f32_e32 v142, v142
+	s_nop 0
+	v_fma_f32 v142, v142, -2.0, 1.0
+	v_bfi_b32 v144, v77, v143, v142
+	v_fma_f32 v142, v144, v70, v92
+	v_mov_b32_e32 v143, 0
+	v_fmac_f32_dpp v143, v144, v82 row_ror:8 row_mask:0xf bank_mask:0xf
+	v_fmac_f32_dpp v142, v144, v71 row_ror:1 row_mask:0xf bank_mask:0xf
+	v_fmac_f32_dpp v143, v144, v83 row_ror:9 row_mask:0xf bank_mask:0xf
+	v_fmac_f32_dpp v142, v144, v72 row_ror:2 row_mask:0xf bank_mask:0xf
+	v_fmac_f32_dpp v143, v144, v84 row_ror:10 row_mask:0xf bank_mask:0xf
+	v_fmac_f32_dpp v142, v144, v73 row_ror:3 row_mask:0xf bank_mask:0xf
+	v_fmac_f32_dpp v143, v144, v85 row_ror:11 row_mask:0xf bank_mask:0xf
+	v_fmac_f32_dpp v142, v144, v78 row_ror:4 row_mask:0xf bank_mask:0xf
+	v_fmac_f32_dpp v143, v144, v86 row_ror:12 row_mask:0xf bank_mask:0xf
+	v_fmac_f32_dpp v142, v144, v79 row_ror:5 row_mask:0xf bank_mask:0xf
+	v_fmac_f32_dpp v143, v144, v87 row_ror:13 row_mask:0xf bank_mask:0xf
+	v_fmac_f32_dpp v142, v144, v80 row_ror:6 row_mask:0xf bank_mask:0xf
+	v_fmac_f32_dpp v143, v144, v88 row_ror:14 row_mask:0xf bank_mask:0xf
+	v_fmac_f32_dpp v142, v144, v81 row_ror:7 row_mask:0xf bank_mask:0xf
+	v_fmac_f32_dpp v143, v144, v89 row_ror:15 row_mask:0xf bank_mask:0xf
+	v_add_f32_e32 v144, v142, v143
+	v_add_f32_e32 v145, v142, v143
+	s_nop 1
+	v_permlane32_swap_b32_e32 v144, v145
+	v_mul_f32_e32 v142, 0xbfb8aa3b, v144
+	v_exp_f32_e32 v142, v142
+	v_sub_f32_e32 v143, v153, v145
+	v_mul_f32_e32 v176, v143, v142
+	v_mul_f32_e32 v207, v143, v142
+	v_sub_f32_e32 v206, v206, v144
+	s_nop 0
+	v_permlane16_swap_b32_e32 v176, v207
+	s_nop 0
+	v_mov_b32_e32 v142, v176
+	v_mov_b32_e32 v143, v207
+	v_bfi_b32 v153, v93, v180, v179
+	v_mov_b32_dpp v142, v176 row_ror:8 row_mask:0xa bank_mask:0xf
+	v_mov_b32_dpp v143, v207 row_ror:8 row_mask:0xa bank_mask:0xf
+	v_fma_f32 v144, v142, v2, v42
+	v_mul_f32_e32 v145, v143, v10
+	v_fmac_f32_dpp v145, v143, v11 row_ror:1 row_mask:0xf bank_mask:0xf
+	v_fmac_f32_dpp v144, v142, v3 row_ror:1 row_mask:0xf bank_mask:0xf
+	v_fmac_f32_dpp v145, v143, v12 row_ror:2 row_mask:0xf bank_mask:0xf
+	v_fmac_f32_dpp v144, v142, v4 row_ror:2 row_mask:0xf bank_mask:0xf
+	v_fmac_f32_dpp v145, v143, v13 row_ror:3 row_mask:0xf bank_mask:0xf
+	v_fmac_f32_dpp v144, v142, v5 row_ror:3 row_mask:0xf bank_mask:0xf
+	v_fmac_f32_dpp v145, v143, v14 row_ror:4 row_mask:0xf bank_mask:0xf
+	v_fmac_f32_dpp v144, v142, v6 row_ror:4 row_mask:0xf bank_mask:0xf
+	v_fmac_f32_dpp v145, v143, v15 row_ror:5 row_mask:0xf bank_mask:0xf
+	v_fmac_f32_dpp v144, v142, v7 row_ror:5 row_mask:0xf bank_mask:0xf
+	v_fmac_f32_dpp v145, v143, v16 row_ror:6 row_mask:0xf bank_mask:0xf
+	v_fmac_f32_dpp v144, v142, v8 row_ror:6 row_mask:0xf bank_mask:0xf
+	v_fmac_f32_dpp v145, v143, v17 row_ror:7 row_mask:0xf bank_mask:0xf
+	v_fmac_f32_dpp v144, v142, v9 row_ror:7 row_mask:0xf bank_mask:0xf
+	v_add_f32_e32 v143, v144, v145
+	v_mov_b32_dpp v142, v145 row_ror:8 row_mask:0xf bank_mask:0xf
+	v_add_f32_dpp v142, v144, v142 row_ror:8 row_mask:0xf bank_mask:0xf
+	s_nop 1
+	v_permlane16_swap_b32_e32 v143, v142
+	v_add_f32_e32 v144, v143, v142
+	v_exp_f32_e32 v142, v144
+	v_max_f32_e32 v143, 0, v144
+	v_add_f32_e32 v142, 1.0, v142
+	v_rcp_f32_e32 v142, v142
+	s_nop 0
+	v_fma_f32 v142, v142, -2.0, 1.0
+	v_bfi_b32 v144, v77, v143, v142
+	v_fma_f32 v142, v144, v26, v43
+	s_nop 0
+	v_mul_f32_dpp v143, v144, v27 row_ror:1 row_mask:0xf bank_mask:0xf
+	v_fmac_f32_dpp v142, v144, v28 row_ror:2 row_mask:0xf bank_mask:0xf
+	v_fmac_f32_dpp v143, v144, v29 row_ror:3 row_mask:0xf bank_mask:0xf
+	v_fmac_f32_dpp v142, v144, v30 row_ror:4 row_mask:0xf bank_mask:0xf
+	v_fmac_f32_dpp v143, v144, v31 row_ror:5 row_mask:0xf bank_mask:0xf
+	v_fmac_f32_dpp v142, v144, v32 row_ror:6 row_mask:0xf bank_mask:0xf
+	v_fmac_f32_dpp v143, v144, v33 row_ror:7 row_mask:0xf bank_mask:0xf
+	v_add_f32_e32 v144, v142, v143
+	v_add_f32_e32 v145, v142, v143
+	s_nop 1
+	v_permlane16_swap_b32_e32 v144, v145
+	v_add_f32_e32 v144, v144, v145
+	v_exp_f32_e32 v142, v144
+	v_max_f32_e32 v143, 0, v144
+	v_add_f32_e32 v142, 1.0, v142
+	v_rcp_f32_e32 v142, v142
+	s_nop 0
+	v_fma_f32 v142, v142, -2.0, 1.0
+	v_bfi_b32 v144, v77, v143, v142
+	v_fma_f32 v142, v144, v18, v44
+	v_mov_b32_e32 v143, 0
+	v_fmac_f32_dpp v143, v144, v34 row_ror:8 row_mask:0xf bank_mask:0xf
+	v_fmac_f32_dpp v142, v144, v19 row_ror:1 row_mask:0xf bank_mask:0xf
+	v_fmac_f32_dpp v143, v144, v35 row_ror:9 row_mask:0xf bank_mask:0xf
+	v_fmac_f32_dpp v142, v144, v20 row_ror:2 row_mask:0xf bank_mask:0xf
+	v_fmac_f32_dpp v143, v144, v36 row_ror:10 row_mask:0xf bank_mask:0xf
+	v_fmac_f32_dpp v142, v144, v21 row_ror:3 row_mask:0xf bank_mask:0xf
+	v_fmac_f32_dpp v143, v144, v37 row_ror:11 row_mask:0xf bank_mask:0xf
+	v_fmac_f32_dpp v142, v144, v22 row_ror:4 row_mask:0xf bank_mask:0xf
+	v_fmac_f32_dpp v143, v144, v38 row_ror:12 row_mask:0xf bank_mask:0xf
+	v_fmac_f32_dpp v142, v144, v23 row_ror:5 row_mask:0xf bank_mask:0xf
+	v_fmac_f32_dpp v143, v144, v39 row_ror:13 row_mask:0xf bank_mask:0xf
+	v_fmac_f32_dpp v142, v144, v24 row_ror:6 row_mask:0xf bank_mask:0xf
+	v_fmac_f32_dpp v143, v144, v40 row_ror:14 row_mask:0xf bank_mask:0xf
+	v_fmac_f32_dpp v142, v144, v25 row_ror:7 row_mask:0xf bank_mask:0xf
+	v_fmac_f32_dpp v143, v144, v41 row_ror:15 row_mask:0xf bank_mask:0xf
+	v_add_f32_e32 v144, v142, v143
+	v_add_f32_e32 v145, v142, v143
+	s_nop 1
+	v_permlane32_swap_b32_e32 v144, v145
+	v_mul_f32_e32 v142, 0xbfb8aa3b, v144
+	v_exp_f32_e32 v142, v142
+	v_sub_f32_e32 v143, v153, v145
+	v_mul_f32_e32 v177, v143, v142
+	v_mul_f32_e32 v178, v143, v142
+	v_sub_f32_e32 v206, v206, v144
+	s_nop 0
+	v_permlane16_swap_b32_e32 v177, v178
+	v_mov_b32_e32 v179, v176
+	v_pk_mul_f32 v[142:143], s[52:53], v[176:177]
+	v_pk_mul_f32 v[144:145], s[52:53], v[178:179]
+	v_pk_mul_f32 v[182:183], v[142:143], v[142:143] neg_lo:[0,1] neg_hi:[0,1]
+	v_mov_b32_dpp v181, v143 row_ror:15 row_mask:0xf bank_mask:0xf bound_ctrl:1
+	v_pk_add_f32 v[182:183], v[144:145], v[182:183]
+	v_pk_add_f32 v[142:143], v[142:143], 1.0 op_sel_hi:[1,0] neg_lo:[1,0] neg_hi:[1,0]
+	v_pk_mul_f32 v[182:183], v[182:183], v[182:183]
+	v_pk_mul_f32 v[142:143], v[142:143], v[142:143]
+	v_pk_mul_f32 v[182:183], v[182:183], s[56:57] op_sel_hi:[1,0]
+	v_mul_f32_e32 v153, s52, v207
+	v_pk_add_f32 v[142:143], v[142:143], v[182:183]
+	v_mov_b32_e32 v180, v152
+	v_cndmask_b32_e64 v143, 0, v143, s[2:3]
+	v_cndmask_b32_e64 v142, 0, v142, s[4:5]
+	v_add_f32_e32 v179, v142, v143
+	v_pk_mul_f32 v[142:143], v[144:145], v[144:145]
+	s_nop 0
+	v_mov_b32_e32 v145, v142
+	v_pk_add_f32 v[142:143], v[152:153], v[144:145] neg_lo:[0,1] neg_hi:[0,1]
+	s_nop 0
+	v_pk_mul_f32 v[142:143], v[142:143], v[142:143]
+	s_nop 0
+	v_mul_f32_e32 v143, 0x42c80000, v143
+	v_add_f32_e32 v142, v142, v143
+	v_cndmask_b32_e64 v142, 0, v142, s[6:7]
+	v_add_f32_e32 v144, v142, v179
+	v_mul_f32_e32 v143, v153, v153
+	v_mov_b32_e32 v142, v153
+	v_pk_add_f32 v[142:143], v[180:181], v[142:143] neg_lo:[0,1] neg_hi:[0,1]
+	s_nop 0
+	v_pk_mul_f32 v[142:143], v[142:143], v[142:143]
+	s_nop 0
+	v_mul_f32_e32 v143, 0x42c80000, v143
+	v_add_f32_e32 v142, v142, v143
+	v_cndmask_b32_e64 v142, 0, v142, s[8:9]
+	v_add_f32_e32 v142, v142, v144
+	s_nop 1
+	v_add_f32_dpp v206, v206, v206 row_ror:8 row_mask:0xf bank_mask:0xf bound_ctrl:1
+	v_add_f32_dpp v142, v142, v142 row_ror:8 row_mask:0xf bank_mask:0xf bound_ctrl:1
+	s_nop 0
+	v_add_f32_dpp v206, v206, v206 row_ror:4 row_mask:0xf bank_mask:0xf bound_ctrl:1
+	v_add_f32_dpp v142, v142, v142 row_ror:4 row_mask:0xf bank_mask:0xf bound_ctrl:1
+	s_nop 0
+	v_add_f32_dpp v206, v206, v206 row_ror:2 row_mask:0xf bank_mask:0xf bound_ctrl:1
+	v_add_f32_dpp v142, v142, v142 row_ror:2 row_mask:0xf bank_mask:0xf bound_ctrl:1
+	s_nop 0
+	v_add_f32_dpp v143, v206, v206 row_ror:1 row_mask:0xf bank_mask:0xf bound_ctrl:1
+	v_add_f32_dpp v206, v206, v206 row_ror:1 row_mask:0xf bank_mask:0xf bound_ctrl:1
+	v_add_f32_dpp v142, v142, v142 row_ror:1 row_mask:0xf bank_mask:0xf bound_ctrl:1
+	s_nop 0
+	v_permlane16_swap_b32_e32 v206, v143
+	v_add_f32_e32 v206, v206, v143
+	s_nop 0
+	v_cvt_f64_f32_e32 v[144:145], v142
+	v_max3_f32 v142, |v207|, |v176|, |v178|
+	v_max_f32_e64 v143, |v177|, |v177|
+	v_max_f32_e32 v142, v142, v143
+	v_cmp_nlt_f32_e32 vcc, 1.0, v142
+	s_cmp_eq_u64 vcc, -1
+	v_sub_f32_e32 v142, v206, v197
+	s_cselect_b64 s[14:15], -1, 0
+	v_cndmask_b32_e64 v143, v202, v142, s[14:15]
+	v_mul_f32_e32 v153, 0x3fb8aa3b, v143
+	v_exp_f32_e32 v153, v153
+	v_cmp_le_f64_e64 vcc, |v[144:145]|, s[58:59]
+	s_nop 1
+	v_cndmask_b32_e64 v181, v200, -v145, vcc
+	v_cndmask_b32_e32 v180, v201, v144, vcc
+	v_min_f32_e32 v144, 1.0, v153
+	v_cmp_u_f32_e32 vcc, v143, v143
+	v_cmp_lt_f64_e64 s[16:17], s[26:27], v[180:181]
+	s_nop 0
+	v_cndmask_b32_e32 v143, v144, v143, vcc
+	v_cmp_lt_f32_e32 vcc, v205, v143
+	s_and_b64 s[18:19], s[50:51], vcc
+	s_and_b64 vcc, exec, s[12:13]
+	s_cbranch_vccnz 68
+	v_cvt_f64_f32_e32 v[142:143], v142
+	v_add_f64 v[144:145], v[180:181], -v[148:149]
+	v_add_f64 v[142:143], v[144:145], v[142:143]
+	v_cndmask_b32_e64 v143, v203, v143, s[14:15]
+	v_cndmask_b32_e64 v142, 0, v142, s[14:15]
+	v_mul_f64 v[144:145], v[142:143], s[60:61]
+	v_rndne_f64_e32 v[144:145], v[144:145]
+	v_fma_f64 v[182:183], s[62:63], v[144:145], v[142:143]
+	v_fmac_f64_e32 v[182:183], s[64:65], v[144:145]
+	v_mov_b64_e32 v[184:185], v[154:155]
+	v_fmac_f64_e32 v[184:185], s[66:67], v[182:183]
+	v_mov_b64_e32 v[188:189], v[156:157]
+	v_fmac_f64_e32 v[188:189], v[182:183], v[184:185]
+	v_mov_b64_e32 v[184:185], v[158:159]
+	v_fmac_f64_e32 v[184:185], v[182:183], v[188:189]
+	v_mov_b64_e32 v[188:189], v[160:161]
+	v_fmac_f64_e32 v[188:189], v[182:183], v[184:185]
+	v_mov_b64_e32 v[184:185], v[162:163]
+	v_fmac_f64_e32 v[184:185], v[182:183], v[188:189]
+	v_mov_b64_e32 v[188:189], v[164:165]
+	v_fmac_f64_e32 v[188:189], v[182:183], v[184:185]
+	v_mov_b64_e32 v[184:185], v[166:167]
+	v_fmac_f64_e32 v[184:185], v[182:183], v[188:189]
+	v_mov_b64_e32 v[188:189], v[168:169]
+	v_fmac_f64_e32 v[188:189], v[182:183], v[184:185]
+	v_mov_b64_e32 v[184:185], v[170:171]
+	v_fmac_f64_e32 v[184:185], v[182:183], v[188:189]
+	v_fma_f64 v[184:185], v[182:183], v[184:185], 1.0
+	v_fma_f64 v[182:183], v[182:183], v[184:185], 1.0
+	v_cvt_i32_f64_e32 v144, v[144:145]
+	v_ldexp_f64 v[144:145], v[182:183], v144
+	v_min_f64 v[144:145], v[144:145], 1.0
+	v_cmp_nlt_f64_e32 vcc, s[68:69], v[142:143]
+	v_cmp_ngt_f64_e64 s[14:15], s[70:71], v[142:143]
+	s_nop 0
+	v_cndmask_b32_e32 v145, v204, v145, vcc
+	s_and_b64 vcc, s[14:15], vcc
+	v_cndmask_b32_e64 v143, 0, v145, s[14:15]
+	v_cndmask_b32_e32 v142, 0, v144, vcc
+	v_cvt_f64_f32_e32 v[144:145], v205
+	v_cmp_gt_f64_e32 vcc, v[142:143], v[144:145]
+	s_and_b64 s[14:15], s[50:51], vcc
+	s_branch 14
+	s_waitcnt lgkmcnt(1)
+	v_mov_b32_e32 v208, v205
+	v_mov_b32_e32 v179, v185
+	v_mov_b32_e32 v207, v210
+	v_mov_b32_e32 v176, v182
+	v_mov_b32_e32 v178, v184
+	v_mov_b32_e32 v177, v183
+	s_add_i32 s31, s31, 1
+	v_and_b32_e32 v209, 0xff, v153
+	s_and_saveexec_b64 s[14:15], s[54:55]
+	s_cbranch_execnz 11
+	s_branch 16
+	s_and_b64 s[14:15], s[18:19], s[16:17]
+	v_cndmask_b32_e64 v153, 0, 1, s[14:15]
+	s_add_i32 s49, s49, 1
+	v_cndmask_b32_e64 v179, 0, 1, s[18:19]
+	s_add_i32 s31, s31, 1
+	v_and_b32_e32 v209, 0xff, v153
+	s_and_saveexec_b64 s[14:15], s[54:55]
+	s_and_b32 s16, s31, 1
+	s_lshl_b32 s16, s16, 4
+	s_add_i32 s16, s83, s16
+	v_mov_b32_e32 v142, s16
+	ds_write_b32 v142, v209
+	s_or_b64 exec, exec, s[14:15]
+	v_and_b32_e32 v142, 1, v153
+	v_cmp_eq_u32_e64 s[14:15], 1, v142
+	s_cmp_le_i32 s31, s33
+	s_cselect_b64 s[72:73], -1, 0
+	v_cndmask_b32_e64 v147, v147, v173, s[14:15]
+	v_cndmask_b32_e64 v146, v146, v172, s[14:15]
+	v_cndmask_b32_e64 v151, v151, v175, s[14:15]
+	v_cndmask_b32_e64 v150, v150, v174, s[14:15]
+	v_cndmask_b32_e64 v197, v197, v206, s[14:15]
+	v_cndmask_b32_e64 v149, v149, v181, s[14:15]
+	s_cmp_gt_i32 s31, s33
+	v_cndmask_b32_e64 v148, v148, v180, s[14:15]
+	s_cbranch_scc1 64869
```
